# tonyzyl/ladcast

Hardware: AMD Instinct MI355X
Metric: ensemble-member-steps/sec (higher is better)
Workload: dtype f32

## Files before the change

### include/ladcast_hip.h

```cpp
#ifndef LADCAST_HIP_H
#define LADCAST_HIP_H

#ifdef __cplusplus
extern "C" {
#endif

#define LDC_ABI_VERSION 5

#define LDC_OK 0
#define LDC_ERR_ARG (-1)
#define LDC_ERR_ALIGN (-2)
#define LDC_ERR_UNSUPPORTED (-3)

enum ldc_act { LDC_ACT_NONE = 0, LDC_ACT_SILU = 1, LDC_ACT_GELU_TANH = 2, LDC_ACT_RELU = 3 };
#define LDC_ACT_IN_TIMESTEP_SINCOS 16

int ldc_abi_version(void);
const char* ldc_build_arch(void);

typedef struct ldc_gemm_desc {
  int M, N, K, batch;
  int lda, ldw, ldc, ldr;
  long long a_bs, c_bs, r_bs;
  int gate_bs;
  int act;
  int flags;
  int reserved;
} ldc_gemm_desc;
#define LDC_GEMM_A_SPLIT 1
#define LDC_GEMM_C_SPLIT 2
#define LDC_GEMM_BF16_1TERM 4
#define LDC_GEMM_F32_REGSTAGE 8
#define LDC_FMT_F32 0
#define LDC_FMT_SPLIT 1
#define LDC_FMT_BF16 2
int ldc_sizeof_gemm_desc(void);
int ldc_gemm_bias_act(const float* A, const float* W, const float* bias, const float* gate,
                      const float* R, float* C, const ldc_gemm_desc* d, void* stream);

#define LDC_GEMM_MAX_PROBLEMS 4
typedef struct ldc_gemm_problem {
  const float* A;
  const float* W;
  const float* bias;
  const float* gate;
  const float* R;
  float* C;
  ldc_gemm_desc d;
} ldc_gemm_problem;
int ldc_sizeof_gemm_problem(void);
long long ldc_gemm_grouped_workspace_bytes(void);
int ldc_gemm_grouped_workspace_init(void* workspace, long long workspace_bytes, void* stream);
int ldc_gemm_grouped(const ldc_gemm_problem* problems, int n, void* workspace, long long workspace_bytes,
                     void* stream);

int ldc_gemm_grouped_bf16x3(const ldc_gemm_problem* problems, int n, void* workspace, long long workspace_bytes,
                            void* stream);
int ldc_pack_weight_bf16x2(const float* W, void* out, int N, int K, int ldw, void* stream);
int ldc_pack_weight_bf16(const float* W, void* out, int N, int K, int ldw, void* stream);

int ldc_linear_small(const float* x, int x_rows, const float* W, const float* bias,
                     const float* add, int add_rows, float* y, int rows, int N, int K,
                     int act_in, int act_out, void* stream);

int ldc_linear_small_mod(const float* x, int x_rows, const float* W, const float* bias, const float* add, int add_rows,
                         const float* mod, int mod_rows, float* y, int rows, int N, int K, int act_in, int act_out,
                         void* stream);

#define LDC_LINEAR_SMALL_MAX_GROUPED 4
typedef struct ldc_linear_small_problem {
  const float* x;
  const float* W;
  const float* bias;
  const float* add;
  float* y;
  int x_rows, add_rows, rows, N, K, act_in, act_out, reserved;
} ldc_linear_small_problem;
int ldc_linear_small_grouped(const ldc_linear_small_problem* problems, int n, void* stream);

int ldc_attn_fwd(const float* Q, const float* K, const float* V, float* O, int B, int S, int H,
                 int ld_qkv, long long qkv_bs, int ldo, long long o_bs, const float* key_bias, void* stream);
long long ldc_attn_fwd_workspace_bytes(void);
int ldc_attn_fwd_ws(const float* Q, const float* K, const float* V, float* O, int B, int S, int H, int ld_qkv, long long qkv_bs,
                    int ldo, long long o_bs, const float* key_bias, void* workspace, long long workspace_bytes, void* stream);
int ldc_attn_fwd_qrows(const float* Q, const float* K, const float* V, float* O, int B, int S, int Sq, int H, int ld_qkv,
                       long long qkv_bs, int ldo, long long o_bs, const float* key_bias, void* stream);
int ldc_attn_fwd_ws_qrows(const float* Q, const float* K, const float* V, float* O, int B, int S, int Sq, int H, int ld_qkv,
                          long long qkv_bs, int ldo, long long o_bs, const float* key_bias, void* workspace, long long workspace_bytes,
                          void* stream);

#define LDC_ATTN_OUT_SPLIT 1
#define LDC_ATTN_BF16_1TERM 2
#define LDC_ATTN_OUT_BF16 4

typedef struct ldc_qkv_epilogue {
  const float* wq;
  const float* wk;
  const float* rope;
  const float* reserved;
  float eps, qscale;
  int heads, rope_row0;
} ldc_qkv_epilogue;
int ldc_sizeof_qkv_epilogue(void);
int ldc_gemm_grouped_bf16x3_qkv(const ldc_gemm_problem* problems, const ldc_qkv_epilogue* epi, int n, void* workspace,
                                long long workspace_bytes, void* stream);
int ldc_gemm_grouped_qkv_f32(const ldc_gemm_problem* problems, const ldc_qkv_epilogue* epi, int n, void* workspace,
                             long long workspace_bytes, void* stream);
int ldc_attn_qkv_prepare_split(float* Q, float* K, float* V, int B, int S, int H, int ld_qkv, long long qkv_bs, int split_row,
                               const float* wq0, const float* wk0, const float* cos0, const float* sin0, const float* wq1,
                               const float* wk1, const float* cos1, const float* sin1, float eps, void* stream);
long long ldc_attn_fwd_split_workspace_bytes(int B, int S, int H);
long long ldc_attn_fwd_split_workspace_max_bytes(void);
int ldc_attn_fwd_split(const float* Q, const float* K, const float* V, float* O, int B, int S, int H, int ld_qkv,
                       long long qkv_bs, int ldo, long long o_bs, const float* key_bias, int flags, void* workspace,
                       long long workspace_bytes, void* stream);
long long ldc_attn_fwd_split_qrows_workspace_bytes(int B, int S, int Sq, int H);
int ldc_attn_fwd_split_qrows(const float* Q, const float* K, const float* V, float* O, int B, int S, int Sq, int H, int ld_qkv,
                             long long qkv_bs, int ldo, long long o_bs, const float* key_bias, int flags, void* workspace,
                             long long workspace_bytes, void* stream);

int ldc_qk_rmsnorm_rope(float* q, float* k, int B, int row0, int rows, int H, int ld, long long bs,
                        const float* wq, const float* wk, float eps, const float* cos_tab,
                        const float* sin_tab, void* stream);

int ldc_layernorm_mod(const float* x, float* y, int B, int rows, int D, int ldx, long long x_bs,
                      int ldy, long long y_bs, const float* scale, const float* shift, int mod_bs,
                      int mode, float eps, int out_split, void* stream);
int ldc_layernorm_mod2(const float* x, float* y, int B, int rows, int D, int ldx, long long x_bs,
                       int ldy, long long y_bs, const float* scale, const float* shift, int split_row,
                       const float* scale2, const float* shift2, int mod_bs, int mode, float eps,
                       int out_split, void* stream);

int ldc_mean_rows(const float* x, float* y, int B, int rows, int D, int ldx, long long x_bs, void* stream);
int ldc_mean_rows_split(const float* x, float* y, float* x_split, int B, int rows, int D, int ldx,
                        long long x_bs, int lds, long long s_bs, int fmt , void* stream);

int ldc_gate_residual(const float* resid, const float* y, const float* gate, float* out, int B,
                      int rows, int D, int ld_res, long long res_bs, int ld_y, long long y_bs,
                      int gate_bs, void* stream);
int ldc_gate_residual_layernorm(float* resid, const float* y, const float* gate, float* out, int B, int rows, int D, int ld_res,
                                long long res_bs, int ld_y, long long y_bs, int gate_bs, int ld_out, long long out_bs,
                                const float* weight, const float* bias, float eps, int out_split, void* stream);

int ldc_chan_to_token(const float* in, float* out, int B, int C, int N, int ldo, int fill_cols, void* stream);
int ldc_chan_to_token_split(const float* in, float* out, int B, int C, int N, int ldo, int fill_cols,
                            int out_split, void* stream);
int ldc_token_to_chan(const float* in, float* out, int B, int C, int N, int ldi, void* stream);

int ldc_timestep_embedding(const float* t, float* out, int n, void* stream);

int ldc_temb_modulate(float* temb, const float* te, int B, int D, int te_rows, void* stream);

int ldc_chan_affine(const float* x, float* y, const float* mean, const float* std_, float target_std,
                    long long outer, int C, long long inner, int inverse, void* stream);

int ldc_edm_scale_f64_to_f32(const double* x, double c_in, float* out, long long n, void* stream);
int ldc_edm_init_state(const float* noise, double sigma0, double* x, long long n, void* stream);
int ldc_edm_churn(const double* x_cur, const double* noise, double coef, double* x_hat, long long n, void* stream);
int ldc_edm_euler(const double* x_hat, const float* F, double c_skip, double c_out, double t_hat,
                  double dt, double* x_next, double* d_cur, long long n, void* stream);
int ldc_edm_heun(const double* x_hat, double* x_next, const float* F, const double* d_cur,
                 double c_skip, double c_out, double t_next, double dt, long long n, void* stream);
int ldc_f64_to_f32(const double* x, float* y, long long n, void* stream);
int ldc_dpm_step(const float* sample, const float* F, const float* m1, float* x0, float* prev,
                 float c_skip, float c_out, float a, float b, float inv_r0, int order, long long n,
                 void* stream);
int ldc_ddim_step(const float* sample, const float* F, const float* noise, float* x0, float* prev, float sqrt_alpha_t,
                  float sqrt_beta_t, float sqrt_alpha_prev, float dir_coef, float std_dev, float clip_range,
                  int prediction_type, int use_clipped_model_output, long long n, void* stream);
int ldc_ddpm_step(const float* sample, const float* F, const float* noise, float* x0, float* prev, float sqrt_alpha_t,
                  float sqrt_beta_t, float x0_coef, float sample_coef, float std_dev, float clip_range, int prediction_type,
                  long long n, void* stream);
int ldc_scale_f32(const float* x, float s, float* y, long long n, void* stream);
int ldc_axpby_f32(const float* x, float a, const float* y, float b, float* out, long long n, void* stream);

int ldc_edm_noise_inputs(const float* clean, const float* noise, const float* sigma, const float* c_in, float* noisy,
                         float* x_in, int B, long long n_per_sample, void* stream);
int ldc_edm_denoise(const float* noisy, const float* F, const float* c_skip, const float* c_out, float* denoised, int B,
                    int C, int T, int plane, int noisy_frames, int f_frames, int denoised_frames, void* stream);
int ldc_edm_denoise_loss(const float* noisy, const float* F, const float* target, const float* c_skip, const float* c_out,
                         const float* weight, const float* lat_weight, float* table, float* denoised, int B, int C, int T,
                         int H, int W, void* stream);

int ldc_sphere_conv_nhwc(const float* X, const float* Wt, const float* bias, const float* R, float* Y, int B,
                         int H, int W, int cin, int ldx, int cout, int ldy, int ldr, int ksize, int act,
                         void* stream);
int ldc_sphere_dwconv_nhwc(const float* x, const float* wt, const float* bias, float* y, int B, int H, int W,
                           int C, int ldx, int ldy, int ksize, int glu, void* stream);
int ldc_grouped_conv1x1_nhwc(const float* x, const float* wt, float* y, long long M, int groups, int ldx, int ldy,
                             void* stream);
int ldc_relu_linear_attn_nhwc(const float* qkv, float* y, int B, int P, int groups, int ldq, int ldy, float eps,
                              void* workspace, long long workspace_bytes, void* stream);
long long ldc_relu_linear_attn_workspace_bytes(int B, int P, int groups);
int ldc_rmsnorm_rows(const float* x, const float* w, const float* b, const float* resid, float* y, long long rows,
                     int C, int ldx, int ldr, int ldy, float eps, int act, void* stream);
int ldc_pixel_unshuffle_shortcut(const float* cv, const float* x, float* y, int B, int H2, int W2, int cout, int cin,
                                 void* stream);
int ldc_pixel_shuffle_shortcut(const float* cv, const float* x, float* y, int B, int H, int W, int cout, int cin,
                               void* stream);
int ldc_chan_regroup(const float* x, float* y, long long M, int cin, int cout, void* stream);

int ldc_sphere_conv_nhwc_split(const float* X, const void* Wp, const float* bias, const float* R, float* Y, int B, int H, int W,
                               int cin, int ldx, int cout, int ldy, int ldr, int ksize, int act, int in_fmt, int out_fmt,
                               void* workspace, long long workspace_bytes, void* stream);
int ldc_sphere_conv_plan(int B, int H, int W, int cin, int cout, int ksize, int in_fmt, int* tile_rows, int* tile_w);
int ldc_rmsnorm_rows_split(const float* x, const float* w, const float* b, const float* resid, float* y, float* ys, long long rows,
                           int C, int ldx, int ldr, int ldy, int lds, int fmt, float eps, int act, void* stream);
int ldc_pixel_unshuffle_shortcut_split(const float* cv, const float* x, float* y, float* ys, int B, int H2, int W2, int cout,
                                       int cin, int lds, int fmt, void* stream);
int ldc_pixel_shuffle_shortcut_split(const float* cv, const float* x, float* y, float* ys, int B, int H, int W, int cout, int cin,
                                     int lds, int fmt, void* stream);
int ldc_upsample_nearest2x_rows(const float* x, float* y, float* ys, int B, int H, int W, int C, int ldx, int ldy, int lds, int fmt, void* stream);
int ldc_pixel_shuffle_to_chan(const float* cv, float* out, int B, int H, int W, int cout, int keep, void* stream);
int ldc_split_rows(const float* x, float* ys, long long rows, int C, int ldx, int lds, int fmt, void* stream);
int ldc_sphere_dwconv_nhwc_fmt(const float* x, const float* wt, const float* bias, float* y, int B, int H, int W, int C, int ldx,
                               int ldy, int ksize, int glu, int out_fmt, void* stream);
int ldc_relu_linear_attn_nhwc_fmt(const float* qkv, float* y, int B, int P, int groups, int ldq, int ldy, float eps, int out_fmt,
                                  void* workspace, long long workspace_bytes, void* stream);

long long ldc_ensemble_scores_workspace_bytes(int C, int H, int W);
int ldc_ensemble_scores(const float* forecast, long long member_stride, long long channel_stride,
                        const float* truth, long long truth_channel_stride, const float* clim,
                        long long clim_channel_stride, const float* lat_weight, int M, int C, int H, int W,
                        int nan_channel, float* out, float* skill_map, float* spread_map, void* workspace,
                        long long workspace_bytes, void* stream);
long long ldc_rollout_scores_workspace_bytes(int C, int L, int H, int W);
int ldc_rollout_scores(const float* forecast, long long member_stride, long long lead_stride, long long channel_stride,
                       const float* mean, const float* std_, float target_std, const float* truth, long long truth_slot_stride,
                       long long truth_channel_stride, const int* truth_slot, const float* clim, long long clim_slot_stride,
                       long long clim_channel_stride, const int* clim_slot, const float* lat_weight, int M, int C, int L, int H,
                       int W, int nan_channel, float* out, int L_total, int l_off, void* workspace, long long workspace_bytes,
                       void* stream);
long long ldc_validation_scores_workspace_bytes(int C, int L, int H, int W);
int ldc_validation_scores(const float* forecast, long long member_stride, long long lead_stride, long long channel_stride,
                          const float* mean, const float* std_, float target_std, const float* truth, long long truth_slot_stride,
                          long long truth_channel_stride, const int* truth_slot, const float* lat_weight, int M, int C, int L, int H,
                          int W, float* out, int L_total, int l_off, void* workspace, long long workspace_bytes, void* stream);
long long ldc_rollout_reliability_workspace_bytes(int M, int C, int L, int H, int W);
int ldc_rollout_reliability(const float* forecast, long long member_stride, long long lead_stride, long long channel_stride,
                            const float* mean, const float* std_, float target_std, const float* truth, long long truth_slot_stride,
                            long long truth_channel_stride, const int* truth_slot, const float* lat_weight, int M, int C, int L, int H,
                            int W, int nan_channel, float* out, int* hist_count, float* hist_weight, int* n_invalid, int L_total,
                            int l_off, void* workspace, long long workspace_bytes, void* stream);
long long ldc_rollout_spectrum_workspace_bytes(int M, int C, int L, int H, int W);
int ldc_rollout_spectrum(const float* forecast, long long member_stride, long long lead_stride, long long channel_stride,
                         const float* mean, const float* std_, float target_std, const float* truth, long long truth_slot_stride,
                         long long truth_channel_stride, const int* truth_slot, const float* row_weight, int M, int C, int L, int H,
                         int W, float* out, int* n_invalid, int L_total, int l_off, void* workspace, long long workspace_bytes,
                         void* stream);
#define LDC_PRODUCTS_MAX_QUANTILES 16
#define LDC_PRODUCTS_MAX_THRESHOLDS 8
typedef struct ldc_products_desc {
  int n_quant;
  int n_thr;
  int q_lo[LDC_PRODUCTS_MAX_QUANTILES];
  float q_t[LDC_PRODUCTS_MAX_QUANTILES];
  int thr_dir[LDC_PRODUCTS_MAX_THRESHOLDS];
} ldc_products_desc;
int ldc_sizeof_products_desc(void);
int ldc_rollout_products(const float* forecast, long long member_stride, long long lead_stride, long long channel_stride,
                         const float* mean, const float* std_, float target_std, const int* channels, int M, int C, int Cs, int L, int H,
                         int W, const ldc_products_desc* desc, const float* thr, float* stats, float* quant, float* exceed, int L_total,
                         int l_off, void* stream);

#define LDC_TRACK_MAX_CHANNELS 8
#define LDC_TRACK_MAX_BOXES 8
#define LDC_TRACK_MAX_INNER 30
#define LDC_TRACK_MAX_GRID 1024
int ldc_track_gather(const float* x, long long sb, long long st, long long sc, int B, int T, long long HW, const int* channels,
                     int n_ch, const float* mean, const float* std_, float target_std, float* out, int T_total, int t_off,
                     void* stream);
int ldc_track_nanmean(const float* x, long long member_stride, int E, long long n, float* out, void* stream);
int ldc_track_storms(const float* fields, long long track_stride, long long frame_stride, long long mslp_off, long long z_off,
                     const float* lsm, const double* lat, int H, const double* lon, int W, const double* lat0,
                     const double* lon0, int n_tracks, int n_steps, const int* inner_box_sizes, int n_boxes, int enforce_msl,
                     double* out_lat, double* out_lon, int* out_code, void* stream);
int ldc_track_local_min(const float* fields, long long field_stride, const int* field_idx, const double* lat, int H,
                        const double* lon, int W, const double* lat0, const double* lon0, const int* inner, int n_queries,
                        int* found, double* out_lat, double* out_lon, float* out_val, void* stream);

int ldc_recon_preprocess(const float* x, long long batch_stride, long long channel_stride, long long row_stride, int B, int C,
                         int H, int W, const float* mean, const float* std_, int sst_channel, float* out,
                         unsigned char* nan_mask, void* stream);
long long ldc_recon_scores_workspace_bytes(int B, int Cp, int H, int W);
int ldc_recon_scores(const float* pred, const float* target, const float* static_, long long static_batch_stride,
                     const unsigned char* nan_mask, const float* lat_weight, const float* mean, const float* std_, int B, int C,
                     int S, int H, int W, int sst_channel, float* rel, float* abs_norm, float* lw_mse, void* workspace,
                     long long workspace_bytes, void* stream);

long long ldc_field_moments_workspace_bytes(int B, int C, int H, int W);
int ldc_field_moments(const float* x, long long batch_stride, long long channel_stride, long long row_stride, int B, int C, int H,
                      int W, double* state, int accumulate, void* workspace, long long workspace_bytes, void* stream);

#ifdef __cplusplus
}
#endif
#endif
```

### ladcast_amd/csrc/rowops.hip

```cpp
#include "common.h"

namespace {

constexpr int LN_MAX_V4 = 8;

__global__ __launch_bounds__(256) void layernorm_mod_kernel(float* __restrict__ x, float* __restrict__ y,
                                                            int rows, int D, int ldx, long long x_bs, int ldy,
                                                            long long y_bs, const float* __restrict__ scale,
                                                            const float* __restrict__ shift, int split_row,
                                                            const float* __restrict__ scale2,
                                                            const float* __restrict__ shift2, int mod_bs, int mode,
                                                            float eps, int out_split, const float* __restrict__ pre_y,
                                                            const float* __restrict__ pre_gate, int ld_prey,
                                                            long long prey_bs, int gate_bs) {
  const int lane = threadIdx.x & 63;
  const int row = blockIdx.x * 4 + (threadIdx.x >> 6);
  const int b = blockIdx.y;
  if (row >= rows) return;
  if (row >= split_row) {
    scale = scale2;
    shift = shift2;
  }
  float* xr = x + b * x_bs + static_cast<long long>(row) * ldx;
  float* yr = y + b * y_bs + static_cast<long long>(row) * ldy;
  const int nv4 = D >> 2;
  float4 v[LN_MAX_V4];
  float sum = 0.f;
#pragma unroll
  for (int i = 0; i < LN_MAX_V4; ++i) {
    const int c = lane + 64 * i;
    if (c < nv4) {
      v[i] = reinterpret_cast<const float4*>(xr)[c];
      if (pre_y) {
        const float4 yv = reinterpret_cast<const float4*>(pre_y + b * prey_bs + static_cast<long long>(row) * ld_prey)[c];
        const float4 g = reinterpret_cast<const float4*>(pre_gate + static_cast<long long>(b) * gate_bs)[c];
        v[i] = make_float4(fmaf(yv.x, g.x, v[i].x), fmaf(yv.y, g.y, v[i].y), fmaf(yv.z, g.z, v[i].z), fmaf(yv.w, g.w, v[i].w));
        reinterpret_cast<float4*>(xr)[c] = v[i];
      }
      sum += (v[i].x + v[i].y) + (v[i].z + v[i].w);
    } else {
      v[i] = make_float4(0.f, 0.f, 0.f, 0.f);
    }
  }
  const float mean = wave_sum(sum) / static_cast<float>(D);
  float sq = 0.f;
#pragma unroll
  for (int i = 0; i < LN_MAX_V4; ++i) {
    const int c = lane + 64 * i;
    if (c < nv4) {
      const float a = v[i].x - mean, bq = v[i].y - mean, cq = v[i].z - mean, dq = v[i].w - mean;
      sq += (a * a + bq * bq) + (cq * cq + dq * dq);
    }
  }
  const float rstd = rsqrtf(wave_sum(sq) / static_cast<float>(D) + eps);
  const float* sc = scale ? scale + (mode == 0 ? static_cast<long long>(b) * mod_bs : 0) : nullptr;
  const float* sh = shift ? shift + (mode == 0 ? static_cast<long long>(b) * mod_bs : 0) : nullptr;
  const float one = (mode == 0) ? 1.f : 0.f;
#pragma unroll
  for (int i = 0; i < LN_MAX_V4; ++i) {
    const int c = lane + 64 * i;
    if (c < nv4) {
      float4 m = sc ? reinterpret_cast<const float4*>(sc)[c] : make_float4(1.f - one, 1.f - one, 1.f - one, 1.f - one);
      float4 a = sh ? reinterpret_cast<const float4*>(sh)[c] : make_float4(0.f, 0.f, 0.f, 0.f);
      float4 o;
      o.x = (v[i].x - mean) * rstd * (one + m.x) + a.x;
      o.y = (v[i].y - mean) * rstd * (one + m.y) + a.y;
      o.z = (v[i].z - mean) * rstd * (one + m.z) + a.z;
      o.w = (v[i].w - mean) * rstd * (one + m.w) + a.w;
      if (out_split == LDC_FMT_BF16) {
        *reinterpret_cast<uint2*>(reinterpret_cast<unsigned char*>(yr) + 8 * c) = make_uint2(ldc_pack_pair(o.x, o.y), ldc_pack_pair(o.z, o.w));
      } else if (out_split) {
        float r0, r1, r2, r3;
        uint2 hi, lo;
        hi.x = ldc_split_pair(o.x, o.y, r0, r1);
        hi.y = ldc_split_pair(o.z, o.w, r2, r3);
        lo.x = ldc_pack_pair(r0, r1);
        lo.y = ldc_pack_pair(r2, r3);
        unsigned char* grp = reinterpret_cast<unsigned char*>(yr + 8 * (c >> 1)) + 8 * (c & 1);
        *reinterpret_cast<uint2*>(grp) = hi;
        *reinterpret_cast<uint2*>(grp + 16) = lo;
      } else {
        reinterpret_cast<float4*>(yr)[c] = o;
      }
    }
  }
}

__global__ __launch_bounds__(256) void qk_rmsnorm_rope_kernel(float* __restrict__ q, float* __restrict__ k, int row0,
                                                              int rows, int H, int ld, long long bs,
                                                              const float* __restrict__ wq,
                                                              const float* __restrict__ wk, float eps,
                                                              const float* __restrict__ cos_tab,
                                                              const float* __restrict__ sin_tab) {
  const int lane = threadIdx.x & 63;
  const long long item = static_cast<long long>(blockIdx.x) * 4 + (threadIdx.x >> 6);
  const int b = blockIdx.y;
  const long long n_items = static_cast<long long>(rows) * H * 2;
  if (item >= n_items) return;
  const int which = static_cast<int>(item & 1);
  const int head = static_cast<int>((item >> 1) % H);
  const int row = static_cast<int>((item >> 1) / H);
  float* base = (which ? k : q) + b * bs + static_cast<long long>(row0 + row) * ld + head * 128;
  const float* w = which ? wk : wq;
  float2 v = reinterpret_cast<float2*>(base)[lane];
  const float ss = wave_sum(v.x * v.x + v.y * v.y);
  const float r = rsqrtf(ss * (1.0f / 128.0f) + eps);
  const float2 wv = reinterpret_cast<const float2*>(w)[lane];
  v.x = v.x * r * wv.x;
  v.y = v.y * r * wv.y;
  if (cos_tab) {
    const float2 c = reinterpret_cast<const float2*>(cos_tab + static_cast<long long>(row) * 128)[lane];
    const float2 s = reinterpret_cast<const float2*>(sin_tab + static_cast<long long>(row) * 128)[lane];
    const float ox = v.x * c.x + (-v.y) * s.x;
    const float oy = v.y * c.y + v.x * s.y;
    v.x = ox;
    v.y = oy;
  }
  reinterpret_cast<float2*>(base)[lane] = v;
}

__global__ __launch_bounds__(1024) void mean_rows_kernel(const float* __restrict__ x, float* __restrict__ y, int rows,
                                                         int D, int ldx, long long x_bs) {
  __shared__ float part[16][64];
  const int c = threadIdx.x & 63;
  const int col = blockIdx.x * 64 + c;
  const int g = threadIdx.x >> 6;
  const int b = blockIdx.y;
  float s0 = 0.f, s1 = 0.f, s2 = 0.f, s3 = 0.f;
  if (col < D) {
    const float* xb = x + b * x_bs + col;
    int r = g;
    for (; r + 48 < rows; r += 64) {
      s0 += xb[static_cast<long long>(r) * ldx];
      s1 += xb[static_cast<long long>(r + 16) * ldx];
      s2 += xb[static_cast<long long>(r + 32) * ldx];
      s3 += xb[static_cast<long long>(r + 48) * ldx];
    }
    for (; r < rows; r += 16) s0 += xb[static_cast<long long>(r) * ldx];
  }
  part[g][c] = (s0 + s1) + (s2 + s3);
  __syncthreads();
  if (g == 0 && col < D) {
    float t = 0.f;
#pragma unroll
    for (int i = 0; i < 16; ++i) t += part[i][c];
    y[static_cast<long long>(b) * D + col] = t / static_cast<float>(rows);
  }
}

__global__ __launch_bounds__(1024) void mean_rows_split_kernel(const float* __restrict__ x, float* __restrict__ y,
                                                               float* __restrict__ xs, int rows, int D, int ldx,
                                                               long long x_bs, int lds, long long s_bs, int fmt) {
  __shared__ float2 part[16][64];
  const int c = threadIdx.x & 63;
  const int col = (blockIdx.x * 64 + c) * 2;
  const int g = threadIdx.x >> 6;
  const int b = blockIdx.y;
  float2 s0 = make_float2(0.f, 0.f), s1 = s0, s2 = s0, s3 = s0;
  if (col < D) {
    const float* xb = x + b * x_bs + col;
    unsigned char* sb = fmt == LDC_FMT_BF16 ? reinterpret_cast<unsigned char*>(xs + b * s_bs) + 2 * col
                                            : reinterpret_cast<unsigned char*>(xs + b * s_bs + (col & ~7)) + 2 * (col & 7);
    auto take = [&](int r, float2& acc) {
      const float2 v = *reinterpret_cast<const float2*>(xb + static_cast<long long>(r) * ldx);
      acc.x += v.x;
      acc.y += v.y;
      float r0, r1;
      const unsigned hi = ldc_split_pair(v.x, v.y, r0, r1);
      unsigned char* d = sb + static_cast<long long>(r) * lds * 4;
      *reinterpret_cast<unsigned*>(d) = hi;
      if (fmt != LDC_FMT_BF16) *reinterpret_cast<unsigned*>(d + 16) = ldc_pack_pair(r0, r1);
    };
    int r = g;
    for (; r + 48 < rows; r += 64) {
      take(r, s0);
      take(r + 16, s1);
      take(r + 32, s2);
      take(r + 48, s3);
    }
    for (; r < rows; r += 16) take(r, s0);
  }
  part[g][c] = make_float2((s0.x + s1.x) + (s2.x + s3.x), (s0.y + s1.y) + (s2.y + s3.y));
  __syncthreads();
  if (g == 0 && col < D) {
    float2 t = make_float2(0.f, 0.f);
#pragma unroll
    for (int i = 0; i < 16; ++i) {
      t.x += part[i][c].x;
      t.y += part[i][c].y;
    }
    y[static_cast<long long>(b) * D + col] = t.x / static_cast<float>(rows);
    y[static_cast<long long>(b) * D + col + 1] = t.y / static_cast<float>(rows);
  }
}

__global__ __launch_bounds__(256) void gate_residual_kernel(const float* __restrict__ resid, const float* __restrict__ y,
                                                            const float* __restrict__ gate, float* __restrict__ out,
                                                            int rows, int D, int ld_res, long long res_bs, int ld_y,
                                                            long long y_bs, int gate_bs) {
  const int b = blockIdx.z;
  const int row = blockIdx.y;
  const int c = blockIdx.x * 256 + threadIdx.x;
  if (c * 4 >= D) return;
  const float4 r = reinterpret_cast<const float4*>(resid + b * res_bs + static_cast<long long>(row) * ld_res)[c];
  const float4 v = reinterpret_cast<const float4*>(y + b * y_bs + static_cast<long long>(row) * ld_y)[c];
  const float4 g = reinterpret_cast<const float4*>(gate + static_cast<long long>(b) * gate_bs)[c];
  float4 o = make_float4(fmaf(v.x, g.x, r.x), fmaf(v.y, g.y, r.y), fmaf(v.z, g.z, r.z), fmaf(v.w, g.w, r.w));
  reinterpret_cast<float4*>(out + b * res_bs + static_cast<long long>(row) * ld_res)[c] = o;
}

constexpr int LS_ROWS = 8;
constexpr int LS_CPW_MAX = 4;
constexpr int LS_KC = 2048;

__device__ __forceinline__ float modulate_nocontract(float v, float scale, float shift) {
#pragma clang fp contract(off)
  const float f = 1.f + scale;
  const float p = v * f;
  return p + shift;
}

__device__ __forceinline__ void ls_first_read(float4& v) {
#if !(defined(LDC_AB_BUILD) && defined(LDC_LS_NO_FIRST_READ))
  float t0, t1;
  asm volatile("s_waitcnt lgkmcnt(0)\n\tv_mov_b32 %0, %2\n\tv_mov_b32 %1, %3" : "=&v"(t0), "=&v"(t1), "+v"(v.y), "+v"(v.w));
#endif
}

template <int LS_CPW, bool FULL = true>
__device__ __forceinline__ void linear_small_body(const float* __restrict__ x, int x_rows, const float* __restrict__ W,
                                                  const float* __restrict__ bias, const float* __restrict__ add,
                                                  int add_rows, float* __restrict__ y, int rows, int N, int K, int kc,
                                                  int act_in, int act_out, int iters, const float* __restrict__ mod = nullptr,
                                                  int mod_rows = 1) {
  extern __shared__ __attribute__((aligned(16))) float xs[];
  const int lane = threadIdx.x & 63;
  const int wave = threadIdx.x >> 6;
  const int r_base = blockIdx.y * LS_ROWS;
  const int rows_here = rows - r_base < LS_ROWS ? rows - r_base : LS_ROWS;
  for (int it = 0; it < iters; ++it) {
    const int n0 = ((blockIdx.x * iters + it) * 4 + wave) * LS_CPW;
    const float* wr[LS_CPW];
#pragma unroll
    for (int j = 0; j < LS_CPW; ++j) {
      const int n = n0 + j < N ? n0 + j : N - 1;
      wr[j] = W + static_cast<long long>(n) * K;
    }
    float acc[LS_CPW][LS_ROWS];
#pragma unroll
    for (int j = 0; j < LS_CPW; ++j)
#pragma unroll
      for (int i = 0; i < LS_ROWS; ++i) acc[j][i] = 0.f;

    for (int k0 = 0; k0 < K; k0 += kc) {
      const int kn = K - k0 < kc ? K - k0 : kc;
      const int nv4 = kn >> 2;
      if (it == 0) {
        if (k0) __syncthreads();
        for (int idx = threadIdx.x; idx < rows_here * nv4; idx += 256) {
          const int i = idx / nv4, c = idx - i * nv4;
          float4 xv;
          if (FULL && act_in == LDC_ACT_IN_TIMESTEP_SINCOS) {
            const float t = x[(r_base + i) % x_rows];
            float e[4];
#pragma unroll
            for (int j = 0; j < 4; ++j) {
              const int k = k0 + 4 * c + j;
              const float f = expf(-9.210340371976184f * static_cast<float>(k & 127) / 128.0f);
              const float a = t * f;
              e[j] = k < 128 ? cosf(a) : sinf(a);
            }
            xv = make_float4(e[0], e[1], e[2], e[3]);
          } else {
            xv = reinterpret_cast<const float4*>(x + static_cast<long long>((r_base + i) % x_rows) * K + k0)[c];
          }
          if (act_in != LDC_ACT_NONE && !(FULL && act_in == LDC_ACT_IN_TIMESTEP_SINCOS)) {
            xv.x = ldc_apply_act(xv.x, act_in);
            xv.y = ldc_apply_act(xv.y, act_in);
            xv.z = ldc_apply_act(xv.z, act_in);
            xv.w = ldc_apply_act(xv.w, act_in);
          }
          reinterpret_cast<float4*>(xs + i * kc)[c] = xv;
        }
        __syncthreads();
      }
      if (n0 < N) {
        for (int c = lane; c < nv4; c += 64) {
          float4 w[LS_CPW];
#pragma unroll
          for (int j = 0; j < LS_CPW; ++j) {
            typedef float ls_f32x4 __attribute__((ext_vector_type(4)));
            const ls_f32x4 t = __builtin_nontemporal_load(reinterpret_cast<const ls_f32x4*>(wr[j] + k0) + c);
            w[j] = make_float4(t.x, t.y, t.z, t.w);
          }
#pragma unroll
          for (int i = 0; i < LS_ROWS; ++i) {
            if (i < rows_here) {
              float4 xv = reinterpret_cast<const float4*>(xs + i * kc)[c];
              ls_first_read(xv);
#pragma unroll
              for (int j = 0; j < LS_CPW; ++j) acc[j][i] += (w[j].x * xv.x + w[j].y * xv.y) + (w[j].z * xv.z + w[j].w * xv.w);
            }
          }
        }
      }
    }
    if (n0 >= N) continue;
#pragma unroll
    for (int j = 0; j < LS_CPW; ++j) {
      const int n = n0 + j;
#pragma unroll
      for (int i = 0; i < LS_ROWS; ++i) {
        const float sum = wave_sum(acc[j][i]);
        const int r = r_base + i;
        if (lane == 0 && i < rows_here && n < N) {
          float v = sum + (bias ? bias[n] : 0.f);
          v = ldc_apply_act(v, act_out);
          if (add) v += add[static_cast<long long>(r % add_rows) * N + n];
          if (FULL && mod) {
            const float* mr = mod + static_cast<long long>(r % mod_rows) * 2 * N;
            v = modulate_nocontract(v, mr[n], mr[N + n]);
          }
          y[static_cast<long long>(r) * N + n] = v;
        }
      }
    }
  }
}

constexpr int LM_KC = 512;
constexpr int LM_LD = LM_KC + 4;
typedef float lm_f32x4 __attribute__((ext_vector_type(4)));
template <int RT, int U>
__device__ __forceinline__ void lm_steps(const lm_f32x4* __restrict__ wp, const float* __restrict__ xa, lm_f32x4 (&acc)[RT]) {
  lm_f32x4 w[U];
#pragma unroll
  for (int u = 0; u < U; ++u) w[u] = __builtin_nontemporal_load(wp + 4 * u);
#pragma unroll
  for (int u = 0; u < U; ++u)
#pragma unroll
    for (int rt = 0; rt < RT; ++rt) {
      const float4 a = *reinterpret_cast<const float4*>(xa + rt * 16 * LM_LD + 16 * u);
      acc[rt] = __builtin_amdgcn_mfma_f32_16x16x4f32(a.x, w[u].x, acc[rt], 0, 0, 0);
      acc[rt] = __builtin_amdgcn_mfma_f32_16x16x4f32(a.y, w[u].y, acc[rt], 0, 0, 0);
      acc[rt] = __builtin_amdgcn_mfma_f32_16x16x4f32(a.z, w[u].z, acc[rt], 0, 0, 0);
      acc[rt] = __builtin_amdgcn_mfma_f32_16x16x4f32(a.w, w[u].w, acc[rt], 0, 0, 0);
    }
}

template <int RT, int IT>
__global__ __launch_bounds__(256) void linear_rows_mfma_kernel(const float* __restrict__ x, int x_rows, const float* __restrict__ W,
                                                               const float* __restrict__ bias, const float* __restrict__ add, int add_rows,
                                                               float* __restrict__ y, int rows, int N, int K, int act_in, int act_out) {
  extern __shared__ __attribute__((aligned(16))) float xs[];
  const int lane = threadIdx.x & 63, wave = threadIdx.x >> 6;
  const int col = lane & 15, kq = lane >> 4;
  const int r_base = blockIdx.y * 16 * RT;
  const int rows_here = rows - r_base < 16 * RT ? rows - r_base : 16 * RT;
  lm_f32x4 acc[IT][RT];
#pragma unroll
  for (int it = 0; it < IT; ++it)
#pragma unroll
    for (int rt = 0; rt < RT; ++rt) acc[it][rt] = lm_f32x4{0.f, 0.f, 0.f, 0.f};
  for (int k0 = 0; k0 < K; k0 += LM_KC) {
    const int kn = K - k0 < LM_KC ? K - k0 : LM_KC;
    const int nv4 = kn >> 2;
    if (k0) __syncthreads();
    for (int idx = threadIdx.x; idx < 16 * RT * nv4; idx += 256) {
      const int i = idx / nv4, c = idx - i * nv4;
      float4 xv = make_float4(0.f, 0.f, 0.f, 0.f);
      if (i < rows_here) {
        xv = reinterpret_cast<const float4*>(x + static_cast<long long>((r_base + i) % x_rows) * K + k0)[c];
        if (act_in != LDC_ACT_NONE) {
          xv.x = ldc_apply_act(xv.x, act_in);
          xv.y = ldc_apply_act(xv.y, act_in);
          xv.z = ldc_apply_act(xv.z, act_in);
          xv.w = ldc_apply_act(xv.w, act_in);
        }
      }
      reinterpret_cast<float4*>(xs + i * LM_LD)[c] = xv;
    }
    __syncthreads();
#pragma unroll
    for (int it = 0; it < IT; ++it) {
      const int n0 = ((blockIdx.x * IT + it) * 4 + wave) * 16;
      if (n0 < N) {
        const int n = n0 + col < N ? n0 + col : N - 1;
        const lm_f32x4* wp = reinterpret_cast<const lm_f32x4*>(W + static_cast<long long>(n) * K + k0) + kq;
        const float* xa = xs + col * LM_LD + 4 * kq;
        const int ns = kn >> 4;
        int s0 = 0;
        for (; s0 + 8 <= ns; s0 += 8) lm_steps<RT, 8>(wp + 4 * s0, xa + 16 * s0, acc[it]);
        if (s0 < ns) lm_steps<RT, 4>(wp + 4 * s0, xa + 16 * s0, acc[it]);
      }
    }
  }
#pragma unroll
  for (int it = 0; it < IT; ++it) {
    const int n = ((blockIdx.x * IT + it) * 4 + wave) * 16 + col;
    if (n >= N) continue;
    const float bv = bias ? bias[n] : 0.f;
#pragma unroll
    for (int rt = 0; rt < RT; ++rt)
#pragma unroll
      for (int i = 0; i < 4; ++i) {
        const int rl = 16 * rt + 4 * kq + i;
        if (rl >= rows_here) continue;
        const int r = r_base + rl;
        float v = acc[it][rt][i] + bv;
        v = ldc_apply_act(v, act_out);
        if (add) v += add[static_cast<long long>(r % add_rows) * N + n];
        y[static_cast<long long>(r) * N + n] = v;
      }
  }
}

template <int LS_CPW>
__global__ __launch_bounds__(256) void linear_small_kernel(const float* __restrict__ x, int x_rows,
                                                           const float* __restrict__ W, const float* __restrict__ bias,
                                                           const float* __restrict__ add, int add_rows,
                                                           float* __restrict__ y, int rows, int N, int K, int kc, int act_in,
                                                           int act_out, int iters, const float* __restrict__ mod, int mod_rows) {
  linear_small_body<LS_CPW, LS_CPW == 1>(x, x_rows, W, bias, add, add_rows, y, rows, N, K, kc, act_in, act_out, iters, mod, mod_rows);
}

struct LSGroup {
  ldc_linear_small_problem p[LDC_LINEAR_SMALL_MAX_GROUPED];
};

__global__ __launch_bounds__(256) void linear_small_grouped_kernel(LSGroup g) {
  const ldc_linear_small_problem& q = g.p[blockIdx.z];
  if (static_cast<int>(blockIdx.x) * 4 >= q.N || static_cast<int>(blockIdx.y) * LS_ROWS >= q.rows) return;
  const int kc = q.K < LS_KC ? q.K : LS_KC;
  linear_small_body<1>(q.x, q.x_rows, q.W, q.bias, q.add, q.add_rows, q.y, q.rows, q.N, q.K, kc, q.act_in, q.act_out, 1);
}

}

extern "C" int ldc_layernorm_mod2(const float* x, float* y, int B, int rows, int D, int ldx, long long x_bs, int ldy,
                                  long long y_bs, const float* scale, const float* shift, int split_row,
                                  const float* scale2, const float* shift2, int mod_bs, int mode, float eps,
                                  int out_split, void* stream) {
  LDC_CHECK_PTR(x);
  LDC_CHECK_PTR(y);
  if (B <= 0 || rows <= 0 || D <= 0 || split_row < 0) return LDC_ERR_ARG;
  if ((D & 3) || D > 64 * 4 * LN_MAX_V4) return LDC_ERR_UNSUPPORTED;
  if ((ldx & 3) || (ldy & 3) || (x_bs & 3) || (y_bs & 3) || (mod_bs & 3)) return LDC_ERR_ALIGN;
  LDC_CHECK_ALIGN16(x);
  LDC_CHECK_ALIGN16(y);
  if (scale) LDC_CHECK_ALIGN16(scale);
  if (shift) LDC_CHECK_ALIGN16(shift);
  if (scale2) LDC_CHECK_ALIGN16(scale2);
  if (shift2) LDC_CHECK_ALIGN16(shift2);
  if (mode != 0 && mode != 1) return LDC_ERR_UNSUPPORTED;
  if (out_split && ((D & 7) || (ldy & 7) || (y_bs & 7) || (reinterpret_cast<unsigned long long>(y) & 31ull))) return LDC_ERR_ALIGN;
  dim3 grid(ldc_cdiv(rows, 4), B);
  hipLaunchKernelGGL(layernorm_mod_kernel, grid, dim3(256), 0, static_cast<hipStream_t>(stream), const_cast<float*>(x), y, rows, D,
                     ldx, x_bs, ldy, y_bs, scale, shift, split_row, scale2, shift2, mod_bs, mode, eps, out_split,
                     static_cast<const float*>(nullptr), static_cast<const float*>(nullptr), 0, 0LL, 0);
  return ldc_launch_status();
}

extern "C" int ldc_gate_residual_layernorm(float* resid, const float* yv, const float* gate, float* out, int B, int rows, int D,
                                           int ld_res, long long res_bs, int ld_y, long long y_bs, int gate_bs, int ld_out,
                                           long long out_bs, const float* weight, const float* bias, float eps, int out_split,
                                           void* stream) {
  LDC_CHECK_PTR(resid);
  LDC_CHECK_PTR(yv);
  LDC_CHECK_PTR(gate);
  LDC_CHECK_PTR(out);
  if (B <= 0 || rows <= 0 || D <= 0) return LDC_ERR_ARG;
  if ((D & 3) || D > 64 * 4 * LN_MAX_V4) return LDC_ERR_UNSUPPORTED;
  if ((ld_res & 3) || (ld_y & 3) || (ld_out & 3) || (res_bs & 3) || (y_bs & 3) || (out_bs & 3) || (gate_bs & 3)) return LDC_ERR_ALIGN;
  LDC_CHECK_ALIGN16(resid);
  LDC_CHECK_ALIGN16(yv);
  LDC_CHECK_ALIGN16(gate);
  LDC_CHECK_ALIGN16(out);
  if (weight) LDC_CHECK_ALIGN16(weight);
  if (bias) LDC_CHECK_ALIGN16(bias);
  if (out_split && ((D & 7) || (ld_out & 7) || (out_bs & 7) || (reinterpret_cast<unsigned long long>(out) & 31ull))) return LDC_ERR_ALIGN;
  dim3 grid(ldc_cdiv(rows, 4), B);
  hipLaunchKernelGGL(layernorm_mod_kernel, grid, dim3(256), 0, static_cast<hipStream_t>(stream), resid, out, rows, D, ld_res, res_bs,
                     ld_out, out_bs, weight, bias, rows, static_cast<const float*>(nullptr), static_cast<const float*>(nullptr), 0, 1,
                     eps, out_split, yv, gate, ld_y, y_bs, gate_bs);
  return ldc_launch_status();
}

extern "C" int ldc_layernorm_mod(const float* x, float* y, int B, int rows, int D, int ldx, long long x_bs, int ldy,
                                 long long y_bs, const float* scale, const float* shift, int mod_bs, int mode,
                                 float eps, int out_split, void* stream) {
  return ldc_layernorm_mod2(x, y, B, rows, D, ldx, x_bs, ldy, y_bs, scale, shift, rows, nullptr, nullptr, mod_bs, mode, eps,
                            out_split, stream);
}

extern "C" int ldc_qk_rmsnorm_rope(float* q, float* k, int B, int row0, int rows, int H, int ld, long long bs,
                                   const float* wq, const float* wk, float eps, const float* cos_tab,
                                   const float* sin_tab, void* stream) {
  LDC_CHECK_PTR(q);
  LDC_CHECK_PTR(k);
  LDC_CHECK_PTR(wq);
  LDC_CHECK_PTR(wk);
  if (B <= 0 || rows <= 0 || H <= 0 || row0 < 0) return LDC_ERR_ARG;
  if ((cos_tab == nullptr) != (sin_tab == nullptr)) return LDC_ERR_ARG;
  if ((ld & 1) || (bs & 1)) return LDC_ERR_ALIGN;
  const long long items = static_cast<long long>(rows) * H * 2;
  dim3 grid(ldc_cdiv(items, 4), B);
  hipLaunchKernelGGL(qk_rmsnorm_rope_kernel, grid, dim3(256), 0, static_cast<hipStream_t>(stream), q, k, row0, rows, H,
                     ld, bs, wq, wk, eps, cos_tab, sin_tab);
  return ldc_launch_status();
}

extern "C" int ldc_mean_rows(const float* x, float* y, int B, int rows, int D, int ldx, long long x_bs, void* stream) {
  LDC_CHECK_PTR(x);
  LDC_CHECK_PTR(y);
  if (B <= 0 || rows <= 0 || D <= 0) return LDC_ERR_ARG;
  dim3 grid(ldc_cdiv(D, 64), B);
  hipLaunchKernelGGL(mean_rows_kernel, grid, dim3(1024), 0, static_cast<hipStream_t>(stream), x, y, rows, D, ldx, x_bs);
  return ldc_launch_status();
}

extern "C" int ldc_mean_rows_split(const float* x, float* y, float* x_split, int B, int rows, int D, int ldx,
                                   long long x_bs, int lds, long long s_bs, int fmt, void* stream) {
  LDC_CHECK_PTR(x);
  LDC_CHECK_PTR(y);
  LDC_CHECK_PTR(x_split);
  if (B <= 0 || rows <= 0 || D <= 0) return LDC_ERR_ARG;
  if ((D & 7) || (ldx & 1) || (x_bs & 1) || (lds & 7) || (s_bs & 7) || (reinterpret_cast<unsigned long long>(x) & 7ull) ||
      (reinterpret_cast<unsigned long long>(x_split) & 31ull))
    return LDC_ERR_ALIGN;
  if (x == x_split) return LDC_ERR_ARG;
  if (fmt != LDC_FMT_SPLIT && fmt != LDC_FMT_BF16) return LDC_ERR_ARG;
  dim3 grid(ldc_cdiv(D, 128), B);
  hipLaunchKernelGGL(mean_rows_split_kernel, grid, dim3(1024), 0, static_cast<hipStream_t>(stream), x, y, x_split, rows, D,
                     ldx, x_bs, lds, s_bs, fmt);
  return ldc_launch_status();
}

extern "C" int ldc_gate_residual(const float* resid, const float* y, const float* gate, float* out, int B, int rows,
                                 int D, int ld_res, long long res_bs, int ld_y, long long y_bs, int gate_bs,
                                 void* stream) {
  LDC_CHECK_PTR(resid);
  LDC_CHECK_PTR(y);
  LDC_CHECK_PTR(gate);
  LDC_CHECK_PTR(out);
  if (B <= 0 || rows <= 0 || D <= 0) return LDC_ERR_ARG;
  if ((D & 3) || (ld_res & 3) || (ld_y & 3) || (res_bs & 3) || (y_bs & 3) || (gate_bs & 3)) return LDC_ERR_ALIGN;
  if (rows > 65535 || B > 65535) return LDC_ERR_UNSUPPORTED;
  dim3 grid(ldc_cdiv(D / 4, 256), rows, B);
  hipLaunchKernelGGL(gate_residual_kernel, grid, dim3(256), 0, static_cast<hipStream_t>(stream), resid, y, gate, out,
                     rows, D, ld_res, res_bs, ld_y, y_bs, gate_bs);
  return ldc_launch_status();
}

static int linear_small_impl(const float* x, int x_rows, const float* W, const float* bias, const float* add, int add_rows,
                             const float* mod, int mod_rows, float* y, int rows, int N, int K, int act_in, int act_out,
                             void* stream) {
  LDC_CHECK_PTR(x);
  LDC_CHECK_PTR(W);
  LDC_CHECK_PTR(y);
  if (rows <= 0 || N <= 0 || K <= 0 || x_rows <= 0) return LDC_ERR_ARG;
  if (add && add_rows <= 0) return LDC_ERR_ARG;
  if (mod && mod_rows <= 0) return LDC_ERR_ARG;
  if (K & 3) return LDC_ERR_ALIGN;
  if (act_in == LDC_ACT_IN_TIMESTEP_SINCOS) {
    if (K != 256) return LDC_ERR_ARG;
  } else {
    LDC_CHECK_ALIGN16(x);
  }
  LDC_CHECK_ALIGN16(W);
  const int kc = K < LS_KC ? K : LS_KC;
  const int rows_max = rows < LS_ROWS ? rows : LS_ROWS;
  const size_t lds = static_cast<size_t>(rows_max) * kc * sizeof(float);
  static const bool attr_set = [&] {
    (void)hipFuncSetAttribute(reinterpret_cast<const void*>(linear_small_kernel<1>), hipFuncAttributeMaxDynamicSharedMemorySize,
                              LS_ROWS * LS_KC * static_cast<int>(sizeof(float)));
    (void)hipFuncSetAttribute(reinterpret_cast<const void*>(linear_small_kernel<LS_CPW_MAX>),
                              hipFuncAttributeMaxDynamicSharedMemorySize, LS_ROWS * LS_KC * static_cast<int>(sizeof(float)));
    return true;
  }();
  (void)attr_set;
  const bool plain = mod == nullptr && act_in != LDC_ACT_IN_TIMESTEP_SINCOS;
  if (plain && rows > LS_ROWS && N >= 4096 && (K & 63) == 0) {
    const int rt = rows <= 16 ? 1 : 2;
    const int col_groups = ldc_cdiv(N, 64);
    const int row_groups_lm = ldc_cdiv(rows, 16 * rt);
    const long long slots = (rt == 2 ? 2 : 4) * 256LL;
    int iters = 1;
    long long best_cost = -1;
    for (int c = 1; c <= 4; ++c) {
      const long long wgs = static_cast<long long>(ldc_cdiv(col_groups, c)) * row_groups_lm;
      const long long cost = ((wgs + slots - 1) / slots) * c;
      if (best_cost < 0 || cost <= best_cost) { best_cost = cost; iters = c; }
    }
    static const char* const force_lm_iters = LDC_AB_GETENV("LDC_LINEAR_MFMA_ITERS");
    if (force_lm_iters && atoi(force_lm_iters) >= 1 && atoi(force_lm_iters) <= 4) iters = atoi(force_lm_iters);
    dim3 grid(ldc_cdiv(col_groups, iters), row_groups_lm);
    const int lm_lds = 16 * rt * LM_LD * static_cast<int>(sizeof(float));
    static const bool lm_attr_set = [] {
      const int b1 = 16 * LM_LD * static_cast<int>(sizeof(float)), b2 = 2 * b1;
      const auto set = [](auto kern, int bytes) { (void)hipFuncSetAttribute(reinterpret_cast<const void*>(kern), hipFuncAttributeMaxDynamicSharedMemorySize, bytes); };
      set(linear_rows_mfma_kernel<1, 1>, b1); set(linear_rows_mfma_kernel<1, 2>, b1); set(linear_rows_mfma_kernel<1, 3>, b1); set(linear_rows_mfma_kernel<1, 4>, b1);
      set(linear_rows_mfma_kernel<2, 1>, b2); set(linear_rows_mfma_kernel<2, 2>, b2); set(linear_rows_mfma_kernel<2, 3>, b2); set(linear_rows_mfma_kernel<2, 4>, b2);
      return true;
    }();
    (void)lm_attr_set;
    auto launch = [&](auto kern) {
      hipLaunchKernelGGL(kern, grid, dim3(256), lm_lds, static_cast<hipStream_t>(stream), x, x_rows, W, bias, add, add_rows, y, rows, N, K,
                         act_in, act_out);
    };
    if (rt == 1) {
      if (iters == 4) launch(linear_rows_mfma_kernel<1, 4>);
      else if (iters == 3) launch(linear_rows_mfma_kernel<1, 3>);
      else if (iters == 2) launch(linear_rows_mfma_kernel<1, 2>);
      else launch(linear_rows_mfma_kernel<1, 1>);
    } else {
      if (iters == 4) launch(linear_rows_mfma_kernel<2, 4>);
      else if (iters == 3) launch(linear_rows_mfma_kernel<2, 3>);
      else if (iters == 2) launch(linear_rows_mfma_kernel<2, 2>);
      else launch(linear_rows_mfma_kernel<2, 1>);
    }
    return ldc_launch_status();
  }
  const int row_groups = ldc_cdiv(rows, LS_ROWS);
  if (plain && static_cast<long long>(ldc_cdiv(N, 4 * LS_CPW_MAX)) * row_groups >= 1024) {
    int iters = 1;
    if (K <= LS_KC) {
      const long long groups = static_cast<long long>(ldc_cdiv(N, 4 * LS_CPW_MAX)) * row_groups;
      iters = groups >= 2048 ? 4 : 1;
      static const char* const force_iters = LDC_AB_GETENV("LDC_LINEAR_SMALL_ITERS");
      if (force_iters && atoi(force_iters) > 0) iters = atoi(force_iters);
    }
    dim3 grid(ldc_cdiv(ldc_cdiv(N, 4 * LS_CPW_MAX), iters), row_groups);
    hipLaunchKernelGGL(linear_small_kernel<LS_CPW_MAX>, grid, dim3(256), lds, static_cast<hipStream_t>(stream), x, x_rows, W,
                       bias, add, add_rows, y, rows, N, K, kc, act_in, act_out, iters, mod, mod_rows);
  } else {
    dim3 grid(ldc_cdiv(N, 4), row_groups);
    hipLaunchKernelGGL(linear_small_kernel<1>, grid, dim3(256), lds, static_cast<hipStream_t>(stream), x, x_rows, W, bias, add,
                       add_rows, y, rows, N, K, kc, act_in, act_out, 1, mod, mod_rows);
  }
  return ldc_launch_status();
}

extern "C" int ldc_linear_small(const float* x, int x_rows, const float* W, const float* bias, const float* add,
                                int add_rows, float* y, int rows, int N, int K, int act_in, int act_out,
                                void* stream) {
  return linear_small_impl(x, x_rows, W, bias, add, add_rows, nullptr, 1, y, rows, N, K, act_in, act_out, stream);
}

extern "C" int ldc_linear_small_mod(const float* x, int x_rows, const float* W, const float* bias, const float* add,
                                    int add_rows, const float* mod, int mod_rows, float* y, int rows, int N, int K, int act_in,
                                    int act_out, void* stream) {
  LDC_CHECK_PTR(mod);
  return linear_small_impl(x, x_rows, W, bias, add, add_rows, mod, mod_rows, y, rows, N, K, act_in, act_out, stream);
}

extern "C" int ldc_linear_small_grouped(const ldc_linear_small_problem* problems, int n, void* stream) {
  LDC_CHECK_PTR(problems);
  if (n < 1 || n > LDC_LINEAR_SMALL_MAX_GROUPED) return LDC_ERR_ARG;
  LSGroup g{};
  int gx = 0, gy = 0, kc_max = 0, rows_max = 0;
  for (int i = 0; i < n; ++i) {
    const ldc_linear_small_problem& q = problems[i];
    LDC_CHECK_PTR(q.x);
    LDC_CHECK_PTR(q.W);
    LDC_CHECK_PTR(q.y);
    if (q.rows <= 0 || q.N <= 0 || q.K <= 0 || q.x_rows <= 0) return LDC_ERR_ARG;
    if (q.add && q.add_rows <= 0) return LDC_ERR_ARG;
    if (q.K & 3) return LDC_ERR_ALIGN;
    if (q.act_in == LDC_ACT_IN_TIMESTEP_SINCOS) {
      if (q.K != 256) return LDC_ERR_ARG;
    } else {
      LDC_CHECK_ALIGN16(q.x);
    }
    LDC_CHECK_ALIGN16(q.W);
    for (int j = 0; j < i; ++j)
      if (problems[j].y == q.x || problems[j].y == q.add || q.y == problems[j].x || q.y == problems[j].add || q.y == problems[j].y)
        return LDC_ERR_ARG;
    g.p[i] = q;
    const int bx = ldc_cdiv(q.N, 4), by = ldc_cdiv(q.rows, LS_ROWS);
    gx = bx > gx ? bx : gx;
    gy = by > gy ? by : gy;
    const int kc = q.K < LS_KC ? q.K : LS_KC;
    kc_max = kc > kc_max ? kc : kc_max;
    const int r = q.rows < LS_ROWS ? q.rows : LS_ROWS;
    rows_max = r > rows_max ? r : rows_max;
  }
  static const bool attr_set = [&] {
    (void)hipFuncSetAttribute(reinterpret_cast<const void*>(linear_small_grouped_kernel), hipFuncAttributeMaxDynamicSharedMemorySize,
                              LS_ROWS * LS_KC * static_cast<int>(sizeof(float)));
    return true;
  }();
  (void)attr_set;
  const size_t lds = static_cast<size_t>(rows_max) * kc_max * sizeof(float);
  hipLaunchKernelGGL(linear_small_grouped_kernel, dim3(gx, gy, n), dim3(256), lds, static_cast<hipStream_t>(stream), g);
  return ldc_launch_status();
}
```

### ladcast_amd/hip.py

```python
from __future__ import annotations

import ctypes
import os
from ctypes import POINTER, Structure, c_char_p, c_double, c_float, c_int, c_longlong, c_void_p

import torch

_HERE = os.path.dirname(os.path.abspath(__file__))
LIB_PATH = os.environ.get("LDC_LIB_PATH") or os.path.join(_HERE, "libladcast_hip.so")

ACT_NONE, ACT_SILU, ACT_GELU_TANH, ACT_RELU = 0, 1, 2, 3
ACT_IN_TIMESTEP_SINCOS = 16
GEMM_A_SPLIT, GEMM_C_SPLIT, GEMM_BF16_1TERM = 1, 2, 4
GEMM_F32_REGSTAGE = 8
ATTN_OUT_SPLIT, ATTN_BF16_1TERM, ATTN_OUT_BF16 = 1, 2, 4
ABI_VERSION = 5
FMT_F32, FMT_SPLIT, FMT_BF16 = 0, 1, 2


class GemmDesc(Structure):
    _fields_ = [
        ("M", c_int), ("N", c_int), ("K", c_int), ("batch", c_int),
        ("lda", c_int), ("ldw", c_int), ("ldc", c_int), ("ldr", c_int),
        ("a_bs", c_longlong), ("c_bs", c_longlong), ("r_bs", c_longlong),
        ("gate_bs", c_int), ("act", c_int), ("flags", c_int), ("reserved", c_int),
    ]


class GemmProblem(Structure):
    _fields_ = [("A", c_void_p), ("W", c_void_p), ("bias", c_void_p), ("gate", c_void_p), ("R", c_void_p), ("C", c_void_p), ("d", GemmDesc)]


MAX_GROUPED = 4


class QkvEpilogue(Structure):
    _fields_ = [("wq", c_void_p), ("wk", c_void_p), ("rope", c_void_p), ("reserved", c_void_p), ("eps", c_float), ("qscale", c_float),
                ("heads", c_int), ("rope_row0", c_int)]


class LinearSmallProblem(Structure):
    _fields_ = [("x", c_void_p), ("W", c_void_p), ("bias", c_void_p), ("add", c_void_p), ("y", c_void_p), ("x_rows", c_int), ("add_rows", c_int),
                ("rows", c_int), ("N", c_int), ("K", c_int), ("act_in", c_int), ("act_out", c_int), ("reserved", c_int)]


PRODUCTS_MAX_QUANTILES, PRODUCTS_MAX_THRESHOLDS, PRODUCTS_MAX_MEMBERS, PRODUCTS_MAX_SORT_MEMBERS = 16, 8, 1024, 64


class ProductsDesc(Structure):
    _fields_ = [("n_quant", c_int), ("n_thr", c_int), ("q_lo", c_int * PRODUCTS_MAX_QUANTILES), ("q_t", c_float * PRODUCTS_MAX_QUANTILES),
                ("thr_dir", c_int * PRODUCTS_MAX_THRESHOLDS)]


def _load():
    if not os.path.exists(LIB_PATH):
        raise RuntimeError(
            f"{LIB_PATH} is missing: build it with `python -c 'import __graft_entry__ as g; g.build()'` "
            "(or `make -C ladcast_amd/csrc`).  ladcast_amd has no CPU fallback."
        )
    lib = ctypes.CDLL(LIB_PATH)
    P, I, L, F, D = c_void_p, c_int, c_longlong, c_float, c_double
    sig = {
        "ldc_abi_version": (I, []),
        "ldc_build_arch": (c_char_p, []),
        "ldc_sizeof_gemm_desc": (I, []),
        "ldc_gemm_bias_act": (I, [P, P, P, P, P, P, POINTER(GemmDesc), P]),
        "ldc_sizeof_gemm_problem": (I, []),
        "ldc_gemm_grouped_workspace_bytes": (L, []),
        "ldc_gemm_grouped_workspace_init": (I, [P, L, P]),
        "ldc_gemm_grouped": (I, [POINTER(GemmProblem), I, P, L, P]),
        "ldc_gemm_grouped_bf16x3": (I, [POINTER(GemmProblem), I, P, L, P]),
        "ldc_sizeof_qkv_epilogue": (I, []),
        "ldc_gemm_grouped_bf16x3_qkv": (I, [POINTER(GemmProblem), POINTER(QkvEpilogue), I, P, L, P]),
        "ldc_gemm_grouped_qkv_f32": (I, [POINTER(GemmProblem), POINTER(QkvEpilogue), I, P, L, P]),
        "ldc_attn_qkv_prepare_split": (I, [P, P, P, I, I, I, I, L, I, P, P, P, P, P, P, P, P, F, P]),
        "ldc_attn_fwd_split_workspace_bytes": (L, [I, I, I]),
        "ldc_attn_fwd_split_workspace_max_bytes": (L, []),
        "ldc_attn_fwd_split": (I, [P, P, P, P, I, I, I, I, L, I, L, P, I, P, L, P]),
        "ldc_attn_fwd_split_qrows_workspace_bytes": (L, [I, I, I, I]),
        "ldc_attn_fwd_split_qrows": (I, [P, P, P, P, I, I, I, I, I, L, I, L, P, I, P, L, P]),
        "ldc_pack_weight_bf16x2": (I, [P, P, I, I, I, P]),
        "ldc_pack_weight_bf16": (I, [P, P, I, I, I, P]),
        "ldc_linear_small": (I, [P, I, P, P, P, I, P, I, I, I, I, I, P]),
        "ldc_linear_small_grouped": (I, [POINTER(LinearSmallProblem), I, P]),
        "ldc_linear_small_mod": (I, [P, I, P, P, P, I, P, I, P, I, I, I, I, I, P]),
        "ldc_gate_residual_layernorm": (I, [P, P, P, P, I, I, I, I, L, I, L, I, I, L, P, P, F, I, P]),
        "ldc_attn_fwd": (I, [P, P, P, P, I, I, I, I, L, I, L, P, P]),
        "ldc_attn_fwd_ws": (I, [P, P, P, P, I, I, I, I, L, I, L, P, P, L, P]),
        "ldc_attn_fwd_qrows": (I, [P, P, P, P, I, I, I, I, I, L, I, L, P, P]),
        "ldc_attn_fwd_ws_qrows": (I, [P, P, P, P, I, I, I, I, I, L, I, L, P, P, L, P]),
        "ldc_attn_fwd_workspace_bytes": (L, []),
        "ldc_qk_rmsnorm_rope": (I, [P, P, I, I, I, I, I, L, P, P, F, P, P, P]),
        "ldc_sphere_conv_nhwc_split": (I, [P, P, P, P, P, I, I, I, I, I, I, I, I, I, I, I, I, P, L, P]),
        "ldc_sphere_conv_plan": (I, [I, I, I, I, I, I, I, P, P]),
        "ldc_rmsnorm_rows_split": (I, [P, P, P, P, P, P, L, I, I, I, I, I, I, F, I, P]),
        "ldc_pixel_unshuffle_shortcut_split": (I, [P, P, P, P, I, I, I, I, I, I, I, P]),
        "ldc_pixel_shuffle_shortcut_split": (I, [P, P, P, P, I, I, I, I, I, I, I, P]),
        "ldc_pixel_shuffle_to_chan": (I, [P, P, I, I, I, I, I, P]),
        "ldc_split_rows": (I, [P, P, L, I, I, I, I, P]),
        "ldc_upsample_nearest2x_rows": (I, [P, P, P, I, I, I, I, I, I, I, I, P]),
        "ldc_sphere_dwconv_nhwc_fmt": (I, [P, P, P, P, I, I, I, I, I, I, I, I, I, P]),
        "ldc_relu_linear_attn_nhwc_fmt": (I, [P, P, I, I, I, I, I, F, I, P, L, P]),
        "ldc_ensemble_scores_workspace_bytes": (L, [I, I, I]),
        "ldc_ensemble_scores": (I, [P, L, L, P, L, P, L, P, I, I, I, I, I, P, P, P, P, L, P]),
        "ldc_rollout_scores_workspace_bytes": (L, [I, I, I, I]),
        "ldc_rollout_scores": (I, [P, L, L, L, P, P, F, P, L, L, P, P, L, L, P, P, I, I, I, I, I, I, P, I, I, P, L, P]),
        "ldc_validation_scores_workspace_bytes": (L, [I, I, I, I]),
        "ldc_validation_scores": (I, [P, L, L, L, P, P, F, P, L, L, P, P, I, I, I, I, I, P, I, I, P, L, P]),
        "ldc_rollout_reliability_workspace_bytes": (L, [I, I, I, I, I]),
        "ldc_rollout_reliability": (I, [P, L, L, L, P, P, F, P, L, L, P, P, I, I, I, I, I, I, P, P, P, P, I, I, P, L, P]),
        "ldc_rollout_spectrum_workspace_bytes": (L, [I, I, I, I, I]),
        "ldc_rollout_spectrum": (I, [P, L, L, L, P, P, F, P, L, L, P, P, I, I, I, I, I, P, P, I, I, P, L, P]),
        "ldc_sizeof_products_desc": (I, []),
        "ldc_rollout_products": (I, [P, L, L, L, P, P, F, P, I, I, I, I, I, I, POINTER(ProductsDesc), P, P, P, P, I, I, P]),
        "ldc_layernorm_mod": (I, [P, P, I, I, I, I, L, I, L, P, P, I, I, F, I, P]),
        "ldc_layernorm_mod2": (I, [P, P, I, I, I, I, L, I, L, P, P, I, P, P, I, I, F, I, P]),
        "ldc_mean_rows": (I, [P, P, I, I, I, I, L, P]),
        "ldc_mean_rows_split": (I, [P, P, P, I, I, I, I, L, I, L, I, P]),
        "ldc_chan_to_token_split": (I, [P, P, I, I, I, I, I, I, P]),
        "ldc_gate_residual": (I, [P, P, P, P, I, I, I, I, L, I, L, I, P]),
        "ldc_chan_to_token": (I, [P, P, I, I, I, I, I, P]),
        "ldc_token_to_chan": (I, [P, P, I, I, I, I, P]),
        "ldc_timestep_embedding": (I, [P, P, I, P]),
        "ldc_temb_modulate": (I, [P, P, I, I, I, P]),
        "ldc_chan_affine": (I, [P, P, P, P, F, L, I, L, I, P]),
        "ldc_edm_scale_f64_to_f32": (I, [P, D, P, L, P]),
        "ldc_edm_init_state": (I, [P, D, P, L, P]),
        "ldc_edm_euler": (I, [P, P, D, D, D, D, P, P, L, P]),
        "ldc_edm_churn": (I, [P, P, c_double, P, L, P]),
        "ldc_edm_heun": (I, [P, P, P, P, D, D, D, D, L, P]),
        "ldc_f64_to_f32": (I, [P, P, L, P]),
        "ldc_dpm_step": (I, [P, P, P, P, P, F, F, F, F, F, I, L, P]),
        "ldc_ddim_step": (I, [P, P, P, P, P, F, F, F, F, F, F, I, I, L, P]),
        "ldc_ddpm_step": (I, [P, P, P, P, P, F, F, F, F, F, F, I, L, P]),
        "ldc_scale_f32": (I, [P, F, P, L, P]),
        "ldc_axpby_f32": (I, [P, F, P, F, P, L, P]),
        "ldc_edm_noise_inputs": (I, [P, P, P, P, P, P, I, L, P]),
        "ldc_edm_denoise": (I, [P, P, P, P, P, I, I, I, I, I, I, I, P]),
        "ldc_edm_denoise_loss": (I, [P, P, P, P, P, P, P, P, P, I, I, I, I, I, P]),
        "ldc_sphere_conv_nhwc": (I, [P, P, P, P, P, I, I, I, I, I, I, I, I, I, I, P]),
        "ldc_sphere_dwconv_nhwc": (I, [P, P, P, P, I, I, I, I, I, I, I, I, P]),
        "ldc_grouped_conv1x1_nhwc": (I, [P, P, P, L, I, I, I, P]),
        "ldc_relu_linear_attn_nhwc": (I, [P, P, I, I, I, I, I, F, P, L, P]),
        "ldc_relu_linear_attn_workspace_bytes": (L, [I, I, I]),
        "ldc_rmsnorm_rows": (I, [P, P, P, P, P, L, I, I, I, I, F, I, P]),
        "ldc_pixel_unshuffle_shortcut": (I, [P, P, P, I, I, I, I, I, P]),
        "ldc_pixel_shuffle_shortcut": (I, [P, P, P, I, I, I, I, I, P]),
        "ldc_chan_regroup": (I, [P, P, L, I, I, P]),
        "ldc_track_gather": (I, [P, L, L, L, I, I, L, POINTER(c_int), I, P, P, F, P, I, I, P]),
        "ldc_track_nanmean": (I, [P, L, I, L, P, P]),
        "ldc_track_storms": (I, [P, L, L, L, L, P, P, I, P, I, P, P, I, I, POINTER(c_int), I, I, P, P, P, P]),
        "ldc_track_local_min": (I, [P, L, P, P, I, P, I, P, P, P, I, P, P, P, P, P]),
        "ldc_recon_preprocess": (I, [P, L, L, L, I, I, I, I, P, P, I, P, P, P]),
        "ldc_recon_scores_workspace_bytes": (L, [I, I, I, I]),
        "ldc_recon_scores": (I, [P, P, P, L, P, P, P, P, I, I, I, I, I, I, P, P, P, P, L, P]),
        "ldc_field_moments_workspace_bytes": (L, [I, I, I, I]),
        "ldc_field_moments": (I, [P, L, L, L, I, I, I, I, P, I, P, L, P]),
    }
    for name, (res, args) in sig.items():
        fn = getattr(lib, name)
        fn.restype = res
        fn.argtypes = args
    if lib.ldc_abi_version() != ABI_VERSION:
        raise RuntimeError("libladcast_hip.so ABI version mismatch")
    if lib.ldc_sizeof_gemm_desc() != ctypes.sizeof(GemmDesc) or lib.ldc_sizeof_gemm_problem() != ctypes.sizeof(GemmProblem):
        raise RuntimeError("ldc_gemm_desc / ldc_gemm_problem layout mismatch between header and binding")
    if lib.ldc_sizeof_qkv_epilogue() != ctypes.sizeof(QkvEpilogue):
        raise RuntimeError("ldc_qkv_epilogue layout mismatch between header and binding")
    if lib.ldc_sizeof_products_desc() != ctypes.sizeof(ProductsDesc):
        raise RuntimeError("ldc_products_desc layout mismatch between header and binding")
    return lib, sig


lib, SIGNATURES = _load()


def _check(status: int, what: str):
    if status != 0:
        raise RuntimeError(f"{what} failed with status {status}")


def upload_nonblocking(t, device):
    device = torch.device(device)
    if device.type != "cuda" or t.device.type != "cpu":
        return t.to(device)
    return (t if t.is_pinned() else t.pin_memory()).to(device, non_blocking=True)


def _p(t):
    return None if t is None else c_void_p(t.data_ptr())


def _stream():
    return c_void_p(torch.cuda.current_stream().cuda_stream)


def _dev(*ts):
    for t in ts:
        if t is not None and not t.is_cuda:
            raise RuntimeError("ladcast_amd kernels need device tensors (no CPU fallback)")


def gemm(A, W, C, *, M, N, K, batch=1, lda=None, ldw=None, ldc=None, a_bs=0, c_bs=0, bias=None, gate=None,
         gate_bs=0, R=None, ldr=0, r_bs=0, act=ACT_NONE):
    _dev(A, W, C, bias, gate, R)
    d = GemmDesc(M, N, K, batch, lda if lda is not None else K, ldw if ldw is not None else K,
                 ldc if ldc is not None else N, ldr, a_bs, c_bs, r_bs, gate_bs, act, 0, 0)
    _check(lib.ldc_gemm_bias_act(_p(A), _p(W), _p(bias), _p(gate), _p(R), _p(C), ctypes.byref(d), _stream()), "ldc_gemm_bias_act")


_workspaces = {}
_outgrown = []


def _workspace(name, device, nbytes, init=None, grow=False):
    key = (name, str(device), torch.cuda.current_stream(device).cuda_stream)
    ws = _workspaces.get(key)
    if ws is None or (grow and ws.numel() * 4 < nbytes):
        if not grow and torch.cuda.is_current_stream_capturing():
            raise RuntimeError(f"{name}: the first call on a stream must be made outside a graph capture (run one warm-up forward)")
        if ws is not None:
            _outgrown.append(ws)
        ws = torch.empty((nbytes + 3) // 4, device=device, dtype=torch.float32)
        if init == "zero":
            ws.zero_()
        elif init == "grouped":
            _check(lib.ldc_gemm_grouped_workspace_init(c_void_p(ws.data_ptr()), ws.numel() * 4, _stream()), "ldc_gemm_grouped_workspace_init")
        _workspaces[key] = ws
    return ws


def _grouped_workspace(device):
    return _workspace("gemm_grouped", device, lib.ldc_gemm_grouped_workspace_bytes(), init="grouped")


def gemm_problem(A, W, C, *, M, N, K, batch=1, lda=None, ldw=None, ldc=None, a_bs=0, c_bs=0, bias=None, gate=None, gate_bs=0, R=None,
                 ldr=0, r_bs=0, act=ACT_NONE, flags=0):
    _dev(A, W, C, bias, gate, R)
    d = GemmDesc(M, N, K, batch, lda if lda is not None else K, ldw if ldw is not None else K, ldc if ldc is not None else N, ldr,
                 a_bs, c_bs, r_bs, gate_bs, act, flags, 0)
    pv = lambda t: None if t is None else t.data_ptr()
    return GemmProblem(pv(A), pv(W), pv(bias), pv(gate), pv(R), pv(C), d), (A, W, C, bias, gate, R)


def gemm_grouped(problems, split_bf16=False):
    n = len(problems)
    if not 1 <= n <= MAX_GROUPED:
        raise ValueError(f"gemm_grouped takes 1..{MAX_GROUPED} problems")
    arr = (GemmProblem * n)(*[p[0] for p in problems])
    ws = _grouped_workspace(problems[0][1][2].device)
    fn = lib.ldc_gemm_grouped_bf16x3 if split_bf16 else lib.ldc_gemm_grouped
    _check(fn(arr, n, c_void_p(ws.data_ptr()), ws.numel() * 4, _stream()), "ldc_gemm_grouped" + ("_bf16x3" if split_bf16 else ""))


def gemm_sk(A, W, C, split_bf16=False, **kw):
    gemm_grouped([gemm_problem(A, W, C, **kw)], split_bf16=split_bf16)


def pack_weight_bf16x2(W):
    _dev(W)
    W = W.contiguous()
    N, K = W.shape
    out = torch.empty(N * K, device=W.device, dtype=torch.int32)
    _check(lib.ldc_pack_weight_bf16x2(_p(W), _p(out), N, K, K, _stream()), "ldc_pack_weight_bf16x2")
    return out


def pack_weight_bf16(W):
    _dev(W)
    W = W.contiguous()
    N, K = W.shape
    out = torch.empty(N * K, device=W.device, dtype=torch.bfloat16)
    _check(lib.ldc_pack_weight_bf16(_p(W), _p(out), N, K, K, _stream()), "ldc_pack_weight_bf16")
    return out


def linear_small(x, W, y, *, rows, N, K, x_rows=None, bias=None, add=None, add_rows=1, act_in=ACT_NONE, act_out=ACT_NONE, mod=None, mod_rows=1):
    _dev(x, W, y, bias, add, mod)
    xr = x_rows if x_rows is not None else rows
    if mod is not None:
        _check(lib.ldc_linear_small_mod(_p(x), xr, _p(W), _p(bias), _p(add), add_rows, _p(mod), mod_rows, _p(y), rows, N, K, act_in, act_out, _stream()),
               "ldc_linear_small_mod")
        return
    _check(lib.ldc_linear_small(_p(x), xr, _p(W), _p(bias), _p(add), add_rows, _p(y), rows, N, K, act_in, act_out, _stream()), "ldc_linear_small")


def gate_residual_layernorm(resid, y, gate, out, *, B, rows, D, ld_res, res_bs, ld_y, y_bs, gate_bs, ld_out, out_bs, weight, bias, eps, out_split=False):
    _dev(resid, y, gate, out, weight, bias)
    _check(lib.ldc_gate_residual_layernorm(_p(resid), _p(y), _p(gate), _p(out), B, rows, D, ld_res, res_bs, ld_y, y_bs, gate_bs, ld_out, out_bs,
                                           _p(weight), _p(bias), eps, int(out_split), _stream()), "ldc_gate_residual_layernorm")


LINEAR_SMALL_MAX_GROUPED = 4


def linear_small_problem(x, W, y, *, rows, N, K, x_rows=None, bias=None, add=None, add_rows=1, act_in=ACT_NONE, act_out=ACT_NONE):
    _dev(x, W, y, bias, add)
    q = LinearSmallProblem(_p(x), _p(W), _p(bias), _p(add), _p(y), x_rows if x_rows is not None else rows, add_rows, rows, N, K, act_in, act_out, 0)
    return q, (x, W, y, bias, add)


def linear_small_grouped(problems):
    n = len(problems)
    if not 1 <= n <= LINEAR_SMALL_MAX_GROUPED:
        raise ValueError(f"linear_small_grouped takes 1..{LINEAR_SMALL_MAX_GROUPED} problems")
    arr = (LinearSmallProblem * n)(*[p[0] for p in problems])
    _check(lib.ldc_linear_small_grouped(arr, n, _stream()), "ldc_linear_small_grouped")


def _attn_f32_workspace(device):
    return _workspace("attn_fwd", device, lib.ldc_attn_fwd_workspace_bytes(), init="zero")


def attn_fwd(Q, K, V, O, *, B, S, H, ld_qkv, qkv_bs, ldo, o_bs, key_bias=None, use_workspace=True, Sq=None):
    _dev(Q, K, V, O, key_bias)
    if key_bias is not None and key_bias.numel() < S:
        raise ValueError("key_bias must hold one value per key")
    if not use_workspace:
        if Sq is None:
            _check(lib.ldc_attn_fwd(_p(Q), _p(K), _p(V), _p(O), B, S, H, ld_qkv, qkv_bs, ldo, o_bs, _p(key_bias), _stream()), "ldc_attn_fwd")
        else:
            _check(lib.ldc_attn_fwd_qrows(_p(Q), _p(K), _p(V), _p(O), B, S, Sq, H, ld_qkv, qkv_bs, ldo, o_bs, _p(key_bias), _stream()), "ldc_attn_fwd_qrows")
        return
    ws = _attn_f32_workspace(Q.device)
    if Sq is None:
        st = lib.ldc_attn_fwd_ws(_p(Q), _p(K), _p(V), _p(O), B, S, H, ld_qkv, qkv_bs, ldo, o_bs, _p(key_bias), _p(ws), ws.numel() * 4, _stream())
    else:
        st = lib.ldc_attn_fwd_ws_qrows(_p(Q), _p(K), _p(V), _p(O), B, S, Sq, H, ld_qkv, qkv_bs, ldo, o_bs, _p(key_bias), _p(ws), ws.numel() * 4, _stream())
    if st != 0 and not torch.cuda.is_current_stream_capturing():
        ws.zero_()
    _check(st, "ldc_attn_fwd_ws" if Sq is None else "ldc_attn_fwd_ws_qrows")


def rearm_attention_workspaces(device=None):
    want = None if device is None else torch.device(device).index
    for key, ws in _workspaces.items():
        if key[0] == "attn_fwd" and (want is None or ws.device.index == want):
            ws.zero_()


def ensemble_scores(forecast, truth, clim, lat_weight, out, *, M, C, H, W, member_stride, channel_stride, truth_channel_stride,
                    clim_channel_stride=0, nan_channel=-1, skill_map=None, spread_map=None):
    _dev(forecast, truth, clim, lat_weight, out, skill_map, spread_map)
    ws = _workspace("ensemble_scores", forecast.device, int(lib.ldc_ensemble_scores_workspace_bytes(C, H, W)), grow=True)
    _check(lib.ldc_ensemble_scores(_p(forecast), member_stride, channel_stride, _p(truth), truth_channel_stride, _p(clim),
                                   clim_channel_stride, _p(lat_weight), M, C, H, W, nan_channel, _p(out), _p(skill_map), _p(spread_map),
                                   _p(ws), ws.numel() * 4, _stream()), "ldc_ensemble_scores")


def rollout_scores(forecast, truth, truth_slot, clim, clim_slot, lat_weight, out, *, M, C, L, H, W, member_stride, lead_stride, channel_stride,
                   truth_slot_stride, truth_channel_stride, clim_slot_stride=0, clim_channel_stride=0, mean=None, std=None, target_std=1.0,
                   nan_channel=-1, L_total, l_off=0):
    _dev(forecast, truth, truth_slot, clim, clim_slot, lat_weight, out, mean, std)
    ws = _workspace("rollout_scores", forecast.device, int(lib.ldc_rollout_scores_workspace_bytes(C, L, H, W)), grow=True)
    _check(lib.ldc_rollout_scores(_p(forecast), member_stride, lead_stride, channel_stride, _p(mean), _p(std), float(target_std), _p(truth),
                                  truth_slot_stride, truth_channel_stride, _p(truth_slot), _p(clim), clim_slot_stride, clim_channel_stride,
                                  _p(clim_slot), _p(lat_weight), M, C, L, H, W, nan_channel, _p(out), L_total, l_off, _p(ws), ws.numel() * 4,
                                  _stream()), "ldc_rollout_scores")


def validation_scores(forecast, truth, truth_slot, lat_weight, out, *, M, C, L, H, W, member_stride, lead_stride, channel_stride,
                      truth_slot_stride, truth_channel_stride, mean=None, std=None, target_std=1.0, L_total, l_off=0):
    _dev(forecast, truth, truth_slot, lat_weight, out, mean, std)
    ws = _workspace("validation_scores", forecast.device, int(lib.ldc_validation_scores_workspace_bytes(C, L, H, W)), grow=True)
    _check(lib.ldc_validation_scores(_p(forecast), member_stride, lead_stride, channel_stride, _p(mean), _p(std), float(target_std), _p(truth),
                                     truth_slot_stride, truth_channel_stride, _p(truth_slot), _p(lat_weight), M, C, L, H, W, _p(out), L_total,
                                     l_off, _p(ws), ws.numel() * 4, _stream()), "ldc_validation_scores")


def rollout_reliability(forecast, truth, truth_slot, lat_weight, out, hist_count, hist_weight, n_invalid, *, M, C, L, H, W, member_stride,
                        lead_stride, channel_stride, truth_slot_stride, truth_channel_stride, mean=None, std=None, target_std=1.0,
                        nan_channel=-1, L_total, l_off=0):
    _dev(forecast, truth, truth_slot, lat_weight, out, hist_count, hist_weight, n_invalid, mean, std)
    nbytes = int(lib.ldc_rollout_reliability_workspace_bytes(M, C, L, H, W))
    ws = _workspace("rollout_reliability", forecast.device, max(nbytes, 4), grow=True)
    _check(lib.ldc_rollout_reliability(_p(forecast), member_stride, lead_stride, channel_stride, _p(mean), _p(std), float(target_std), _p(truth),
                                       truth_slot_stride, truth_channel_stride, _p(truth_slot), _p(lat_weight), M, C, L, H, W, nan_channel,
                                       _p(out), _p(hist_count), _p(hist_weight), _p(n_invalid), L_total, l_off, _p(ws), ws.numel() * 4,
                                       _stream()), "ldc_rollout_reliability")


def rollout_spectrum(forecast, truth, truth_slot, row_weight, out, n_invalid, *, M, C, L, H, W, member_stride, lead_stride, channel_stride,
                     truth_slot_stride, truth_channel_stride, mean=None, std=None, target_std=1.0, L_total, l_off=0):
    _dev(forecast, truth, truth_slot, row_weight, out, n_invalid, mean, std)
    nbytes = int(lib.ldc_rollout_spectrum_workspace_bytes(M, C, L, H, W))
    ws = _workspace("rollout_spectrum", forecast.device, max(nbytes, 4), grow=True)
    _check(lib.ldc_rollout_spectrum(_p(forecast), member_stride, lead_stride, channel_stride, _p(mean), _p(std), float(target_std), _p(truth),
                                    truth_slot_stride, truth_channel_stride, _p(truth_slot), _p(row_weight), M, C, L, H, W, _p(out),
                                    _p(n_invalid), L_total, l_off, _p(ws), ws.numel() * 4, _stream()), "ldc_rollout_spectrum")


def products_desc(quantiles, M, threshold_dirs=()):
    import math

    qs, dirs = [float(q) for q in quantiles], [int(d) for d in threshold_dirs]
    if len(qs) > PRODUCTS_MAX_QUANTILES or len(dirs) > PRODUCTS_MAX_THRESHOLDS:
        raise ValueError(f"at most {PRODUCTS_MAX_QUANTILES} quantiles and {PRODUCTS_MAX_THRESHOLDS} thresholds per call")
    if any(not 0.0 <= q <= 1.0 for q in qs):
        raise ValueError(f"quantiles must lie in [0, 1], got {qs}")
    if any(d not in (1, -1) for d in dirs):
        raise ValueError(f"a threshold direction is +1 (above) or -1 (below), got {dirs}")
    if M < 1:
        raise ValueError("at least one member")
    d = ProductsDesc()
    d.n_quant, d.n_thr = len(qs), len(dirs)
    for k, q in enumerate(qs):
        pos = q * (M - 1)
        lo = min(int(math.floor(pos)), M - 1)
        d.q_lo[k], d.q_t[k] = lo, pos - lo
    for k, v in enumerate(dirs):
        d.thr_dir[k] = v
    return d


def rollout_products(forecast, desc, *, M, C, L, H, W, member_stride, lead_stride, channel_stride, channels=None, Cs=None, thr=None, stats=None,
                     quant=None, exceed=None, mean=None, std=None, target_std=1.0, L_total, l_off=0):
    _dev(forecast, channels, thr, stats, quant, exceed, mean, std)
    _check(lib.ldc_rollout_products(_p(forecast), member_stride, lead_stride, channel_stride, _p(mean), _p(std), float(target_std), _p(channels),
                                    M, C, C if Cs is None else Cs, L, H, W, ctypes.byref(desc), _p(thr), _p(stats), _p(quant), _p(exceed),
                                    L_total, l_off, _stream()), "ldc_rollout_products")


def recon_preprocess(x, mean, std, out, nan_mask=None, *, B, C, H, W, batch_stride, channel_stride, row_stride, sst_channel=-1):
    _dev(x, mean, std, out, nan_mask)
    _check(lib.ldc_recon_preprocess(_p(x), batch_stride, channel_stride, row_stride, B, C, H, W, _p(mean), _p(std), sst_channel, _p(out),
                                    _p(nan_mask), _stream()), "ldc_recon_preprocess")


def recon_scores(pred, target, static, nan_mask, lat_weight, mean, std, rel, lw_mse, *, B, C, S, H, W, static_batch_stride=0, sst_channel=-1,
                 abs_norm=None):
    _dev(pred, target, static, nan_mask, lat_weight, mean, std, rel, lw_mse, abs_norm)
    ws = _workspace("recon_scores", pred.device, int(lib.ldc_recon_scores_workspace_bytes(B, C + S, H, W)), grow=True)
    _check(lib.ldc_recon_scores(_p(pred), _p(target), _p(static), static_batch_stride, _p(nan_mask), _p(lat_weight), _p(mean), _p(std), B, C, S,
                                H, W, sst_channel, _p(rel), _p(abs_norm), _p(lw_mse), _p(ws), ws.numel() * 4, _stream()), "ldc_recon_scores")


def field_moments(x, state, *, B, C, H, W, batch_stride, channel_stride, row_stride, accumulate):
    _dev(x, state)
    nbytes = int(lib.ldc_field_moments_workspace_bytes(B, C, H, W))
    ws = _workspace("field_moments", x.device, max(nbytes, 16), grow=True)
    _check(lib.ldc_field_moments(_p(x), batch_stride, channel_stride, row_stride, B, C, H, W, _p(state), 1 if accumulate else 0, _p(ws),
                                 ws.numel() * 4, _stream()), "ldc_field_moments")


def compact_rope_table(cos, sin):
    if not (torch.equal(cos[:, 0::2], cos[:, 1::2]) and torch.equal(sin[:, 0::2], sin[:, 1::2])):
        raise ValueError("rotary tables must hold every (cos, sin) value twice (adjacent-pair RoPE)")
    return torch.stack([cos[:, 0::2], sin[:, 0::2]], dim=-1).reshape(cos.shape[0], cos.shape[1]).contiguous()


def qkv_epilogue(wq=None, wk=None, rope=None, *, eps=1e-7, heads, rope_row0=0, qscale=0.0):
    _dev(wq, wk, rope)
    pv = lambda t: None if t is None else t.data_ptr()
    return QkvEpilogue(pv(wq), pv(wk), pv(rope), None, eps, qscale, heads, rope_row0), (wq, wk, rope)


ERR_UNSUPPORTED = -3
_DEFAULT_QSCALE = ctypes.c_float(0.08838834764831845 * 1.4426950408889634).value


def gemm_grouped_qkv_f32(problems, epilogues):
    n = len(problems)
    if not 1 <= n <= MAX_GROUPED or len(epilogues) != n:
        raise ValueError(f"gemm_grouped_qkv_f32 takes 1..{MAX_GROUPED} problems and one epilogue (or None) per problem")
    arr = (GemmProblem * n)(*[p[0] for p in problems])
    epi = (QkvEpilogue * n)(*[(e[0] if e is not None else QkvEpilogue()) for e in epilogues])
    ws = _grouped_workspace(problems[0][1][2].device)
    st = lib.ldc_gemm_grouped_qkv_f32(arr, epi, n, c_void_p(ws.data_ptr()), ws.numel() * 4, _stream())
    if st == ERR_UNSUPPORTED:
        return False
    _check(st, "ldc_gemm_grouped_qkv_f32")
    return True


def gemm_grouped_qkv(problems, epilogues, force_fallback=False):
    n = len(problems)
    if not 1 <= n <= MAX_GROUPED or len(epilogues) != n:
        raise ValueError(f"gemm_grouped_qkv takes 1..{MAX_GROUPED} problems and one epilogue (or None) per problem")
    arr = (GemmProblem * n)(*[p[0] for p in problems])
    epi = (QkvEpilogue * n)(*[(e[0] if e is not None else QkvEpilogue()) for e in epilogues])
    ws = _grouped_workspace(problems[0][1][2].device)
    st = ERR_UNSUPPORTED if force_fallback else lib.ldc_gemm_grouped_bf16x3_qkv(arr, epi, n, c_void_p(ws.data_ptr()), ws.numel() * 4, _stream())
    if st != ERR_UNSUPPORTED:
        _check(st, "ldc_gemm_grouped_bf16x3_qkv")
        return
    if any(p[0].d.flags & GEMM_BF16_1TERM for p in problems):
        raise RuntimeError("ldc_gemm_grouped_bf16x3_qkv: shape not served by the fused kernel, and the plain-GEMM + ldc_attn_qkv_prepare_split "
                           "route only writes split-bf16 operand rows (status -3 in the single-term bf16 mode)")
    _check(lib.ldc_gemm_grouped_bf16x3(arr, n, c_void_p(ws.data_ptr()), ws.numel() * 4, _stream()), "ldc_gemm_grouped_bf16x3 (QKV fallback)")
    for (p, keep), e in zip(problems, epilogues):
        if e is None:
            continue
        q, (wq, wk, rope) = e
        if q.qscale not in (0.0, _DEFAULT_QSCALE):
            raise RuntimeError("ldc_gemm_grouped_bf16x3_qkv: shape not served by the fused kernel, and the plain-GEMM + ldc_attn_qkv_prepare_split "
                               f"route applies the default q scale log2(e)/sqrt(128), not qscale={q.qscale!r}")
        d, C = p.d, keep[2]
        D, S = q.heads * 128, d.M
        if d.N != 3 * D:
            raise RuntimeError("ldc_gemm_grouped_bf16x3_qkv failed with status -1")
        cos = sin = None
        if rope is not None:
            t = rope.reshape(-1, 64, 2)[q.rope_row0 : q.rope_row0 + S]
            cos, sin = t[..., 0].repeat_interleave(2, dim=1).contiguous(), t[..., 1].repeat_interleave(2, dim=1).contiguous()
        base = C.data_ptr()
        _check(lib.ldc_attn_qkv_prepare_split(c_void_p(base), c_void_p(base + 4 * D), c_void_p(base + 8 * D), d.batch, S, q.heads, d.ldc, d.c_bs, S,
                                              _p(wq), _p(wk), _p(cos), _p(sin), None, None, None, None, q.eps, _stream()), "ldc_attn_qkv_prepare_split")


def attn_qkv_prepare_split(Q, K, V, *, B, S, H, ld_qkv, qkv_bs, split_row, seg0=(None, None, None, None), seg1=(None, None, None, None), eps=1e-7):
    _dev(Q, K, V, *seg0, *seg1)
    _check(lib.ldc_attn_qkv_prepare_split(_p(Q), _p(K), _p(V), B, S, H, ld_qkv, qkv_bs, split_row, _p(seg0[0]), _p(seg0[1]), _p(seg0[2]), _p(seg0[3]),
                                          _p(seg1[0]), _p(seg1[1]), _p(seg1[2]), _p(seg1[3]), eps, _stream()), "ldc_attn_qkv_prepare_split")


def _attn_workspace(device, nbytes):
    ws = _workspace("attn_fwd_split", device, lib.ldc_attn_fwd_split_workspace_max_bytes())
    if ws.numel() * 4 < nbytes:
        raise RuntimeError(f"attn_fwd_split: call shape asks for {nbytes} workspace bytes, more than ldc_attn_fwd_split_workspace_max_bytes")
    return ws


def attn_fwd_split(Q, K, V, O, *, B, S, H, ld_qkv, qkv_bs, ldo, o_bs, out_split=False, one_term=False, key_bias=None, use_workspace=True, Sq=None):
    _dev(Q, K, V, O, key_bias)
    if Sq is None:
        nbytes = lib.ldc_attn_fwd_split_workspace_bytes(B, S, H) if use_workspace else 0
    else:
        nbytes = lib.ldc_attn_fwd_split_qrows_workspace_bytes(B, S, Sq, H) if use_workspace else 0
    ws = _attn_workspace(Q.device, nbytes) if nbytes > 0 else None
    if key_bias is not None and key_bias.numel() < 32 * ((S + 31) // 32):
        raise ValueError("key_bias must be padded to a multiple of 32 keys (hip.pad_key_bias)")
    flags = (ATTN_OUT_BF16 if int(out_split) == FMT_BF16 else ATTN_OUT_SPLIT if out_split else 0) | (ATTN_BF16_1TERM if one_term else 0)
    if Sq is None:
        _check(lib.ldc_attn_fwd_split(_p(Q), _p(K), _p(V), _p(O), B, S, H, ld_qkv, qkv_bs, ldo, o_bs, _p(key_bias), flags, _p(ws), 0 if ws is None else ws.numel() * 4,
                                      _stream()), "ldc_attn_fwd_split")
    else:
        _check(lib.ldc_attn_fwd_split_qrows(_p(Q), _p(K), _p(V), _p(O), B, S, Sq, H, ld_qkv, qkv_bs, ldo, o_bs, _p(key_bias), flags, _p(ws),
                                            0 if ws is None else ws.numel() * 4, _stream()), "ldc_attn_fwd_split_qrows")


def pad_key_bias(bias):
    S = bias.numel()
    out = torch.zeros(32 * ((S + 31) // 32), device=bias.device, dtype=torch.float32)
    out[:S] = bias.reshape(-1)
    return out


def qk_rmsnorm_rope(q, k, *, B, row0, rows, H, ld, bs, wq, wk, eps, cos=None, sin=None):
    _dev(q, k, wq, wk, cos, sin)
    _check(lib.ldc_qk_rmsnorm_rope(_p(q), _p(k), B, row0, rows, H, ld, bs, _p(wq), _p(wk), eps, _p(cos), _p(sin), _stream()),
           "ldc_qk_rmsnorm_rope")


def layernorm_mod(x, y, *, B, rows, D, ldx, x_bs, ldy, y_bs, scale=None, shift=None, mod_bs=0, mode=0, eps=1e-6, out_split=False,
                  split_row=None, scale2=None, shift2=None):
    _dev(x, y, scale, shift, scale2, shift2)
    if split_row is None:
        _check(lib.ldc_layernorm_mod(_p(x), _p(y), B, rows, D, ldx, x_bs, ldy, y_bs, _p(scale), _p(shift), mod_bs, mode, eps,
                                     int(out_split), _stream()),
               "ldc_layernorm_mod")
    else:
        _check(lib.ldc_layernorm_mod2(_p(x), _p(y), B, rows, D, ldx, x_bs, ldy, y_bs, _p(scale), _p(shift), split_row, _p(scale2), _p(shift2),
                                      mod_bs, mode, eps, int(out_split), _stream()),
               "ldc_layernorm_mod2")


def mean_rows(x, y, *, B, rows, D, ldx, x_bs, x_split=None, lds=None, s_bs=None, fmt=FMT_SPLIT):
    _dev(x, y, x_split)
    if x_split is None:
        _check(lib.ldc_mean_rows(_p(x), _p(y), B, rows, D, ldx, x_bs, _stream()), "ldc_mean_rows")
    else:
        _check(lib.ldc_mean_rows_split(_p(x), _p(y), _p(x_split), B, rows, D, ldx, x_bs, lds if lds is not None else ldx,
                                       s_bs if s_bs is not None else x_bs, int(fmt), _stream()), "ldc_mean_rows_split")


def gate_residual(resid, y, gate, out, *, B, rows, D, ld_res, res_bs, ld_y, y_bs, gate_bs):
    _dev(resid, y, gate, out)
    _check(lib.ldc_gate_residual(_p(resid), _p(y), _p(gate), _p(out), B, rows, D, ld_res, res_bs, ld_y, y_bs, gate_bs, _stream()),
           "ldc_gate_residual")


def chan_to_token(x, out, *, B, C, N, ldo, fill_cols=None, out_split=False):
    _dev(x, out)
    _check(lib.ldc_chan_to_token_split(_p(x), _p(out), B, C, N, ldo, ldo if fill_cols is None else fill_cols, int(out_split), _stream()),
           "ldc_chan_to_token")


def token_to_chan(x, out, *, B, C, N, ldi):
    _dev(x, out)
    _check(lib.ldc_token_to_chan(_p(x), _p(out), B, C, N, ldi, _stream()), "ldc_token_to_chan")


def timestep_embedding(t, out, n):
    _dev(t, out)
    _check(lib.ldc_timestep_embedding(_p(t), _p(out), n, _stream()), "ldc_timestep_embedding")


def temb_modulate(temb, te, *, B, D, te_rows):
    _dev(temb, te)
    _check(lib.ldc_temb_modulate(_p(temb), _p(te), B, D, te_rows, _stream()), "ldc_temb_modulate")


def chan_affine(x, y, mean, std, target_std, *, outer, C, inner, inverse):
    _dev(x, y, mean, std)
    _check(lib.ldc_chan_affine(_p(x), _p(y), _p(mean), _p(std), target_std, outer, C, inner, int(inverse), _stream()), "ldc_chan_affine")


TRACK_MAX_CHANNELS, TRACK_MAX_BOXES, TRACK_MAX_INNER, TRACK_MAX_GRID = 8, 8, 30, 1024


def _int_array(values):
    return (c_int * len(values))(*[int(v) for v in values])


def track_gather(x, out, channels, mean, std, *, sb, st, sc, B, T, HW, T_total, t_off, target_std=1.0):
    _dev(x, out, mean, std)
    _check(lib.ldc_track_gather(_p(x), sb, st, sc, B, T, HW, _int_array(channels), len(channels), _p(mean), _p(std), float(target_std),
                                _p(out), T_total, t_off, _stream()), "ldc_track_gather")


def track_nanmean(x, out, *, member_stride, E, n):
    _dev(x, out)
    _check(lib.ldc_track_nanmean(_p(x), member_stride, E, n, _p(out), _stream()), "ldc_track_nanmean")


def track_storms(fields, lat, lon, lat0, lon0, out_lat, out_lon, out_code, *, track_stride, frame_stride, mslp_off, z_off, lsm, H, W,
                 n_tracks, n_steps, inner_box_sizes, enforce_msl):
    _dev(fields, lat, lon, lat0, lon0, out_lat, out_lon, out_code, lsm)
    _check(lib.ldc_track_storms(_p(fields), track_stride, frame_stride, mslp_off, z_off, _p(lsm), _p(lat), H, _p(lon), W, _p(lat0), _p(lon0),
                                n_tracks, n_steps, _int_array(inner_box_sizes), len(inner_box_sizes), int(bool(enforce_msl)), _p(out_lat),
                                _p(out_lon), _p(out_code), _stream()), "ldc_track_storms")


def track_local_min(fields, field_idx, lat, lon, lat0, lon0, inner, found, out_lat, out_lon, out_val, *, field_stride, H, W, n_queries):
    _dev(fields, field_idx, lat, lon, lat0, lon0, inner, found, out_lat, out_lon, out_val)
    _check(lib.ldc_track_local_min(_p(fields), field_stride, _p(field_idx), _p(lat), H, _p(lon), W, _p(lat0), _p(lon0), _p(inner), n_queries,
                                   _p(found), _p(out_lat), _p(out_lon), _p(out_val), _stream()), "ldc_track_local_min")


def edm_scale_f64_to_f32(x, c_in, out):
    _dev(x, out)
    _check(lib.ldc_edm_scale_f64_to_f32(_p(x), c_in, _p(out), x.numel(), _stream()), "ldc_edm_scale_f64_to_f32")


def edm_init_state(noise, sigma0, x):
    _dev(noise, x)
    _check(lib.ldc_edm_init_state(_p(noise), sigma0, _p(x), x.numel(), _stream()), "ldc_edm_init_state")


def edm_churn(x_cur, noise, coef, x_hat):
    _dev(x_cur, noise, x_hat)
    if noise.dtype != torch.float64 or x_cur.dtype != torch.float64:
        raise TypeError("edm_churn works on the fp64 sampler state")
    _check(lib.ldc_edm_churn(_p(x_cur), _p(noise), coef, _p(x_hat), x_cur.numel(), _stream()), "ldc_edm_churn")


def edm_euler(x_hat, F, c_skip, c_out, t_hat, dt, x_next, d_cur):
    _dev(x_hat, F, x_next, d_cur)
    _check(lib.ldc_edm_euler(_p(x_hat), _p(F), c_skip, c_out, t_hat, dt, _p(x_next), _p(d_cur), x_hat.numel(), _stream()), "ldc_edm_euler")


def edm_heun(x_hat, x_next, F, d_cur, c_skip, c_out, t_next, dt):
    _dev(x_hat, x_next, F, d_cur)
    _check(lib.ldc_edm_heun(_p(x_hat), _p(x_next), _p(F), _p(d_cur), c_skip, c_out, t_next, dt, x_hat.numel(), _stream()), "ldc_edm_heun")


def f64_to_f32(x, y):
    _dev(x, y)
    _check(lib.ldc_f64_to_f32(_p(x), _p(y), x.numel(), _stream()), "ldc_f64_to_f32")


def dpm_step(sample, F, m1, x0, prev, c_skip, c_out, a, b, inv_r0, order):
    _dev(sample, F, m1, x0, prev)
    _check(lib.ldc_dpm_step(_p(sample), _p(F), _p(m1), _p(x0), _p(prev), c_skip, c_out, a, b, inv_r0, order, sample.numel(), _stream()),
           "ldc_dpm_step")


def ddim_step(sample, F, noise, x0, prev, sqrt_alpha_t, sqrt_beta_t, sqrt_alpha_prev, dir_coef, std_dev, clip_range, prediction_type, reclip):
    _dev(sample, F, noise, x0, prev)
    _check(lib.ldc_ddim_step(_p(sample), _p(F), _p(noise), _p(x0), _p(prev), sqrt_alpha_t, sqrt_beta_t, sqrt_alpha_prev, dir_coef, std_dev,
                             clip_range, prediction_type, int(bool(reclip)), sample.numel(), _stream()), "ldc_ddim_step")


def ddpm_step(sample, F, noise, x0, prev, sqrt_alpha_t, sqrt_beta_t, x0_coef, sample_coef, std_dev, clip_range, prediction_type):
    _dev(sample, F, noise, x0, prev)
    _check(lib.ldc_ddpm_step(_p(sample), _p(F), _p(noise), _p(x0), _p(prev), sqrt_alpha_t, sqrt_beta_t, x0_coef, sample_coef, std_dev, clip_range,
                             prediction_type, sample.numel(), _stream()), "ldc_ddpm_step")


def scale_f32(x, s, y):
    _dev(x, y)
    _check(lib.ldc_scale_f32(_p(x), s, _p(y), x.numel(), _stream()), "ldc_scale_f32")


def axpby_f32(x, a, y, b, out):
    _dev(x, y, out)
    _check(lib.ldc_axpby_f32(_p(x), a, _p(y), b, _p(out), x.numel(), _stream()), "ldc_axpby_f32")


def _f32c(what, *ts):
    for t in ts:
        if t is not None and not (t.dtype == torch.float32 and t.is_contiguous()):
            raise TypeError(f"{what}: contiguous fp32 tensors only")


def _per_sample(what, B, *vs):
    for v in vs:
        if v is not None and not (v.is_cuda and v.dtype == torch.float32 and v.is_contiguous() and v.numel() == B):
            raise ValueError(f"{what}: per-sample coefficients are contiguous fp32 device vectors with one entry per sample ({B})")


def edm_noise_inputs(clean, noise, sigma, c_in, noisy, x_in):
    _dev(clean, noise, sigma, c_in, noisy, x_in)
    _f32c("edm_noise_inputs", clean, noise, noisy, x_in)
    B = clean.shape[0]
    _per_sample("edm_noise_inputs", B, sigma, c_in)
    for t in (noise, noisy, x_in):
        if t is not None and t.shape != clean.shape:
            raise ValueError("edm_noise_inputs: all tensors have the shape of `clean`")
    _check(lib.ldc_edm_noise_inputs(_p(clean), _p(noise), _p(sigma), _p(c_in), _p(noisy), _p(x_in), B, clean.numel() // max(B, 1), _stream()),
           "ldc_edm_noise_inputs")


def _t_slice_frames(what, t, shape):
    B, C, T, H, W = shape
    if tuple(t.shape) != tuple(shape) or t.dtype != torch.float32:
        raise ValueError(f"{what}: fp32 tensors of one shape (B, C, T, H, W)")
    plane = H * W
    sb, sc, st, sh, sw = t.stride()
    ok = (sw == 1 or W == 1) and (sh == W or H == 1) and (st == plane or T == 1)
    frames = sc // plane if C > 1 else (sb // (C * plane) if B > 1 else T)
    ok = ok and frames >= T and (C == 1 or sc == frames * plane) and (B == 1 or sb == C * frames * plane)
    if not ok:
        raise ValueError(f"{what}: tensors must be contiguous or slices along T of contiguous tensors (strides {t.stride()})")
    return frames


def edm_denoise(noisy, F, c_skip, c_out, denoised):
    _dev(noisy, F, c_skip, c_out, denoised)
    B, C, T, H, W = noisy.shape
    _per_sample("edm_denoise", B, c_skip, c_out)
    fr = [_t_slice_frames("edm_denoise", t, noisy.shape) for t in (noisy, F, denoised)]
    _check(lib.ldc_edm_denoise(_p(noisy), _p(F), _p(c_skip), _p(c_out), _p(denoised), B, C, T, H * W, fr[0], fr[1], fr[2], _stream()),
           "ldc_edm_denoise")


def edm_denoise_loss(noisy, F, target, c_skip, c_out, weight, table, lat_weight=None, denoised=None):
    _dev(noisy, F, target, c_skip, c_out, weight, table, lat_weight, denoised)
    _f32c("edm_denoise_loss", noisy, F, target, table, lat_weight, denoised)
    B, C, T, H, W = noisy.shape
    _per_sample("edm_denoise_loss", B, c_skip, c_out, weight)
    for t in (F, target, denoised):
        if t is not None and t.shape != noisy.shape:
            raise ValueError("edm_denoise_loss: noisy, F, target and denoised have one shape (B, C, T, H, W)")
    if table.numel() != B * C * T or (lat_weight is not None and lat_weight.numel() != H):
        raise ValueError("edm_denoise_loss: table holds B * C * T values, lat_weight H")
    _check(lib.ldc_edm_denoise_loss(_p(noisy), _p(F), _p(target), _p(c_skip), _p(c_out), _p(weight), _p(lat_weight), _p(table), _p(denoised),
                                    B, C, T, H, W, _stream()), "ldc_edm_denoise_loss")


def sphere_conv_nhwc(X, Wt, Y, *, B, H, W, cin, cout, ldx=None, ldy=None, bias=None, R=None, ldr=0, ksize=3, act=ACT_NONE):
    _dev(X, Wt, Y, bias, R)
    _check(lib.ldc_sphere_conv_nhwc(_p(X), _p(Wt), _p(bias), _p(R), _p(Y), B, H, W, cin, ldx if ldx is not None else cin, cout,
                                    ldy if ldy is not None else cout, ldr, ksize, act, _stream()), "ldc_sphere_conv_nhwc")


def conv_cin_padded(cin, cpk=32):
    kt = -(-cin // cpk)
    p2 = 1
    while p2 < kt:
        p2 *= 2
    return cpk * p2


def sphere_conv_nhwc_split(X, Wp, Y, *, B, H, W, cin, cout, ldx, ldy=None, bias=None, R=None, ldr=0, ksize=3, act=ACT_NONE, in_fmt=FMT_SPLIT,
                           out_fmt=FMT_F32):
    _dev(X, Wp, Y, bias, R)
    ws = _grouped_workspace(X.device)
    _check(lib.ldc_sphere_conv_nhwc_split(_p(X), _p(Wp), _p(bias), _p(R), _p(Y), B, H, W, cin, ldx, cout, ldy if ldy is not None else cout,
                                          ldr, ksize, act, int(in_fmt), int(out_fmt), _p(ws), ws.numel() * 4, _stream()), "ldc_sphere_conv_nhwc_split")


def sphere_conv_plan(B, H, W, cin, cout, ksize=3, in_fmt=FMT_SPLIT):
    bm, tw = c_int(0), c_int(0)
    halo = lib.ldc_sphere_conv_plan(B, H, W, cin, cout, ksize, int(in_fmt), ctypes.byref(bm), ctypes.byref(tw))
    return bool(halo), bm.value, tw.value


def split_rows(x, ys, *, rows, C, ldx=None, lds=None, fmt=FMT_SPLIT):
    _dev(x, ys)
    _check(lib.ldc_split_rows(_p(x), _p(ys), rows, C, ldx if ldx is not None else C, lds if lds is not None else -(-C // 8) * 8, int(fmt), _stream()),
           "ldc_split_rows")


def sphere_dwconv_nhwc(x, wt, y, *, B, H, W, C, ldx=None, ldy=None, bias=None, ksize=3, glu=False, out_fmt=FMT_F32):
    _dev(x, wt, y, bias)
    cy = C // 2 if glu else C
    _check(lib.ldc_sphere_dwconv_nhwc_fmt(_p(x), _p(wt), _p(bias), _p(y), B, H, W, C, ldx if ldx is not None else C,
                                          ldy if ldy is not None else cy, ksize, int(glu), int(out_fmt), _stream()), "ldc_sphere_dwconv_nhwc_fmt")


def grouped_conv1x1_nhwc(x, wt, y, *, M, groups, ldx, ldy):
    _dev(x, wt, y)
    _check(lib.ldc_grouped_conv1x1_nhwc(_p(x), _p(wt), _p(y), M, groups, ldx, ldy, _stream()), "ldc_grouped_conv1x1_nhwc")


def relu_linear_attn_nhwc(qkv, y, *, B, P, groups, ldq, ldy, eps, out_fmt=FMT_F32, sliced=True):
    _dev(qkv, y)
    ws, nbytes = None, 0
    if sliced:
        nbytes = lib.ldc_relu_linear_attn_workspace_bytes(B, P, groups)
        ws = torch.empty(nbytes // 4, device=qkv.device, dtype=torch.float32) if nbytes else None
    _check(lib.ldc_relu_linear_attn_nhwc_fmt(_p(qkv), _p(y), B, P, groups, ldq, ldy, eps, int(out_fmt), _p(ws), nbytes,
                                             _stream()),
           "ldc_relu_linear_attn_nhwc_fmt")


def rmsnorm_rows(x, w, y, *, rows, C, eps, b=None, resid=None, ldx=None, ldr=None, ldy=None, act=ACT_NONE, ys=None, lds=None, fmt=FMT_SPLIT):
    _dev(x, w, b, resid, y, ys)
    _check(lib.ldc_rmsnorm_rows_split(_p(x), _p(w), _p(b), _p(resid), _p(y), _p(ys), rows, C, ldx if ldx is not None else C,
                                      ldr if ldr is not None else C, ldy if ldy is not None else C,
                                      (lds if lds is not None else -(-C // 8) * 8) if ys is not None else 0, int(fmt), eps, act, _stream()),
           "ldc_rmsnorm_rows_split")


def pixel_unshuffle_shortcut(cv, x, y, *, B, H2, W2, cout, cin, ys=None, lds=None, fmt=FMT_SPLIT):
    _dev(cv, x, y, ys)
    _check(lib.ldc_pixel_unshuffle_shortcut_split(_p(cv), _p(x), _p(y), _p(ys), B, H2, W2, cout, cin,
                                                  (lds if lds is not None else -(-cout // 8) * 8) if ys is not None else 0, int(fmt), _stream()),
           "ldc_pixel_unshuffle_shortcut_split")


def pixel_shuffle_to_chan(cv, out, *, B, H, W, cout, keep):
    _dev(cv, out)
    _check(lib.ldc_pixel_shuffle_to_chan(_p(cv), _p(out), B, H, W, cout, keep, _stream()), "ldc_pixel_shuffle_to_chan")


def pixel_shuffle_shortcut(cv, x, y, *, B, H, W, cout, cin, ys=None, lds=None, fmt=FMT_SPLIT):
    _dev(cv, x, y, ys)
    _check(lib.ldc_pixel_shuffle_shortcut_split(_p(cv), _p(x), _p(y), _p(ys), B, H, W, cout, cin,
                                                (lds if lds is not None else -(-cout // 8) * 8) if ys is not None else 0, int(fmt), _stream()),
           "ldc_pixel_shuffle_shortcut_split")


def upsample_nearest2x_rows(x, y, *, B, H, W, C, ldx=None, ldy=None, ys=None, lds=None, fmt=FMT_SPLIT):
    _dev(x, y, ys)
    _check(lib.ldc_upsample_nearest2x_rows(_p(x), _p(y), _p(ys), B, H, W, C, ldx if ldx is not None else C, ldy if ldy is not None else C,
                                           (lds if lds is not None else (ys.shape[1] if ys is not None else 0)), int(fmt), _stream()), "ldc_upsample_nearest2x_rows")


def chan_regroup(x, y, *, M, cin, cout):
    _dev(x, y)
    _check(lib.ldc_chan_regroup(_p(x), _p(y), M, cin, cout, _stream()), "ldc_chan_regroup")
```

### ladcast_amd/models/LaDCast_3D_model.py

```python
from __future__ import annotations

from types import SimpleNamespace
from typing import Optional, Tuple

import numpy as np
import torch
import torch.nn as nn

from .. import graphs, hip
from .embeddings import get_year_sincos_embedding, rope_tables_from_grid, rotary_1d
from .modeling_utils import ModelMixin


class _RMSNormP(nn.Module):
    def __init__(self, dim, eps):
        super().__init__()
        self.eps = eps
        self.weight = nn.Parameter(torch.ones(dim))

    def forward(self, x):
        var = x.to(torch.float32).pow(2).mean(-1, keepdim=True)
        return x * torch.rsqrt(var + self.eps) * self.weight


class LaDCastAttnProcessor2_0:

    def __call__(self, *a, **k):
        raise RuntimeError("the built-in processor is fused into the HIP forward and is not callable on its own; "
                           "use the C ABI (ldc_gemm_grouped_bf16x3_qkv + ldc_attn_fwd_split, or ldc_qk_rmsnorm_rope + ldc_attn_fwd)")


class _TimestepEmbeddingP(nn.Module):
    def __init__(self, in_channels, dim):
        super().__init__()
        self.linear_1 = nn.Linear(in_channels, dim)
        self.linear_2 = nn.Linear(dim, dim)


class _CombinedTimestepTextProjP(nn.Module):
    def __init__(self, dim, pooled_dim):
        super().__init__()
        self.timestep_embedder = _TimestepEmbeddingP(256, dim)
        self.text_embedder = _TimestepEmbeddingP(pooled_dim, dim)


class _AdaLinearP(nn.Module):
    def __init__(self, dim_in, dim_out):
        super().__init__()
        self.linear = nn.Linear(dim_in, dim_out)


class _ActProjP(nn.Module):
    def __init__(self, a, b):
        super().__init__()
        self.proj = nn.Linear(a, b)


class _FeedForwardP(nn.Module):
    def __init__(self, dim, mult):
        super().__init__()
        inner = int(dim * mult)
        self.net = nn.ModuleList([_ActProjP(dim, inner), nn.Identity(), nn.Linear(inner, dim)])


class _AttentionP(nn.Module):
    def __init__(self, dim, heads, head_dim, eps=1e-7, added=False, pre_only=False):
        super().__init__()
        inner = heads * head_dim
        self.heads = heads
        self.to_q = nn.Linear(dim, inner)
        self.to_k = nn.Linear(dim, inner)
        self.to_v = nn.Linear(dim, inner)
        self.norm_q = _RMSNormP(head_dim, eps)
        self.norm_k = _RMSNormP(head_dim, eps)
        if added:
            self.add_k_proj = nn.Linear(dim, inner)
            self.add_v_proj = nn.Linear(dim, inner)
            self.add_q_proj = nn.Linear(dim, inner)
            self.norm_added_q = _RMSNormP(head_dim, eps)
            self.norm_added_k = _RMSNormP(head_dim, eps)
            self.to_add_out = nn.Linear(inner, dim)
        else:
            self.add_q_proj = self.add_k_proj = self.add_v_proj = None
            self.norm_added_q = self.norm_added_k = None
            self.to_add_out = None
        if not pre_only:
            self.to_out = nn.ModuleList([nn.Linear(inner, dim), nn.Identity()])
        else:
            self.to_out = None
        self.processor = LaDCastAttnProcessor2_0()

    def set_processor(self, processor):
        self.processor = processor

    def get_processor(self):
        return self.processor

    @property
    def foreign_processor(self):
        p = self.processor
        return None if p is None or isinstance(p, LaDCastAttnProcessor2_0) else p


class _PatchEmbedP(nn.Module):

    def __init__(self, in_chans, dim, patch=(1, 1, 1)):
        super().__init__()
        self.proj = nn.Conv3d(in_chans, dim, kernel_size=tuple(patch), stride=tuple(patch))


class _RefinerBlockP(nn.Module):
    def __init__(self, heads, head_dim, mlp_width_ratio=4.0):
        super().__init__()
        d = heads * head_dim
        self.norm1 = nn.LayerNorm(d, elementwise_affine=True, eps=1e-7)
        self.attn = _AttentionP(d, heads, head_dim, pre_only=True)
        self.norm2 = nn.LayerNorm(d, elementwise_affine=True, eps=1e-7)
        self.ff = _FeedForwardP(d, mlp_width_ratio)
        self.norm_out = _AdaLinearP(d, 2 * d)


class _IndividualTokenRefinerP(nn.Module):
    def __init__(self, heads, head_dim, n):
        super().__init__()
        self.refiner_blocks = nn.ModuleList([_RefinerBlockP(heads, head_dim) for _ in range(n)])


class _TokenRefinerP(nn.Module):
    def __init__(self, in_channels, heads, head_dim, n):
        super().__init__()
        d = heads * head_dim
        self.time_text_embed = _CombinedTimestepTextProjP(d, in_channels)
        self.proj_in = nn.Linear(in_channels, d)
        self.token_refiner = _IndividualTokenRefinerP(heads, head_dim, n)


class _SingleBlockP(nn.Module):
    def __init__(self, heads, head_dim, mlp_ratio):
        super().__init__()
        d = heads * head_dim
        mlp = int(d * mlp_ratio)
        self.attn = _AttentionP(d, heads, head_dim, pre_only=True)
        self.norm = _AdaLinearP(d, 3 * d)
        self.proj_mlp = nn.Linear(d, mlp)
        self.proj_out = nn.Linear(d + mlp, d)


class _DualBlockP(nn.Module):
    def __init__(self, heads, head_dim, mlp_ratio):
        super().__init__()
        d = heads * head_dim
        self.norm1 = _AdaLinearP(d, 6 * d)
        self.norm1_context = _AdaLinearP(d, 6 * d)
        self.attn = _AttentionP(d, heads, head_dim, added=True)
        self.ff = _FeedForwardP(d, mlp_ratio)
        self.ff_context = _FeedForwardP(d, mlp_ratio)


class _Workspace:

    def __init__(self, dev, B, Bt, Nx, Nc, D, C_in, C_out, n_mod):
        f = dict(device=dev, dtype=torch.float32)
        self.mods = torch.empty(B, n_mod, **f)
        S = Nx + Nc
        self.h = torch.empty(B, S, D, **f)
        self.nh = torch.empty(B, S, D, **f)
        self.qkv = torch.empty(B, S, 3 * D, **f)
        self.att = torch.empty(B, S, D, **f)
        self.cat = torch.empty(B, S, 5 * D, **f)
        self.xtok = torch.empty(B, Nx, C_in, **f)
        self.ctok = torch.empty(B, Nc, C_in, **f)
        self.ctx0 = torch.empty(B, Nc, D, **f)
        self.otok = torch.empty(B, Nx, C_out, **f)
        self.tsin = torch.empty(Bt, 256, **f)
        self.t1 = torch.empty(Bt, D, **f)
        self.t2 = torch.empty(Bt, D, **f)
        self.t1m = torch.empty(Bt, D, **f)
        self.t2m = torch.empty(Bt, D, **f)
        self.pooled = torch.empty(B, D, **f)
        self.p1 = torch.empty(B, D, **f)
        self.temb_r = torch.empty(B, D, **f)
        self.temb = torch.empty(B, D, **f)
        self.mod_a = torch.empty(B, 6 * D, **f)
        self.mod_b = torch.empty(B, 6 * D, **f)


class LaDCastTransformer3DModel(ModelMixin):
    _supports_gradient_checkpointing = False

    def __init__(
        self,
        in_channels: int = 16,
        out_channels: int = 16,
        num_attention_heads: int = 24,
        attention_head_dim: int = 128,
        num_layers: int = 20,
        num_single_layers: int = 40,
        num_refiner_layers: int = 2,
        mlp_ratio: float = 4.0,
        patch_size: int = 1,
        patch_size_t: int = 1,
        qk_norm: str = "rms_norm",
        rope_theta: float = 256.0,
        rope_axes_dim: Tuple[int, ...] = (16, 56, 56),
        rope_spatial_grid_start_pos=0,
        rope_spatial_grid_end_pos=None,
        spatial_deg2rad: bool = False,
        conditioning_tensor_in_channels: int = None,
        conditioning_tensor_intermediate_proj_dim: Optional[int] = None,
        conditioning_tensor_rope_axes_dim: Tuple[int, ...] = (16, 56, 56),
        incl_time_elapsed: bool = False,
        nope: bool = False,
        scale_attn_by_lat: bool = False,
    ) -> None:
        super().__init__()
        self.register_to_config(**{k: v for k, v in locals().items() if k not in ("self", "__class__")})
        if scale_attn_by_lat and patch_size != 1:
            raise NotImplementedError("scale_attn_by_lat hard-wires the 15 x 30 token grid (models/LaDCast_3D_model.py:684-693): patch size 1 only")
        if attention_head_dim != 128 or qk_norm != "rms_norm":
            raise NotImplementedError("the attention kernel is built for head_dim 128 + rms_norm q/k")
        if in_channels % 4 or (conditioning_tensor_in_channels or in_channels) % 4:
            raise NotImplementedError("channel counts must be multiples of 4 (16-byte rows)")
        heads, hd = num_attention_heads, attention_head_dim
        d = heads * hd
        out_channels = out_channels or in_channels
        self.inner_dim = d
        ps3 = (patch_size_t, patch_size, patch_size)
        self._patch_vol = patch_size_t * patch_size * patch_size
        if (in_channels * self._patch_vol) % 4 or ((conditioning_tensor_in_channels or in_channels) * self._patch_vol) % 4:
            raise NotImplementedError("channels x patch volume must be a multiple of 4 (16-byte rows)")
        self.x_embedder = _PatchEmbedP(in_channels, d, ps3)
        if conditioning_tensor_intermediate_proj_dim is None:
            conditioning_tensor_intermediate_proj_dim = d
        self.context_embedder = _PatchEmbedP(conditioning_tensor_in_channels, d, ps3)
        self.context_refiner = _TokenRefinerP(conditioning_tensor_intermediate_proj_dim, heads, hd, num_refiner_layers)
        self.time_text_embed = _CombinedTimestepTextProjP(d, d)
        self.time_elapsed_embed = _TimestepEmbeddingP(256, 2 * d) if incl_time_elapsed else None
        if spatial_deg2rad:
            rope_spatial_grid_start_pos = [float(np.deg2rad(v)) for v in rope_spatial_grid_start_pos]
            rope_spatial_grid_end_pos = [float(np.deg2rad(v)) for v in rope_spatial_grid_end_pos]
        self.rope_spatial_grid_start_pos = rope_spatial_grid_start_pos
        self.rope_spatial_grid_end_pos = rope_spatial_grid_end_pos
        assert sum(rope_axes_dim) == hd, "sum(rope_axes_dim) must equal attention_head_dim"
        assert sum(conditioning_tensor_rope_axes_dim) == hd
        self.transformer_blocks = nn.ModuleList([_DualBlockP(heads, hd, mlp_ratio) for _ in range(num_layers)])
        self.single_transformer_blocks = nn.ModuleList([_SingleBlockP(heads, hd, mlp_ratio) for _ in range(num_single_layers)])
        self.norm_out = _AdaLinearP(d, 2 * d)
        self.proj_out = nn.Linear(d, self._patch_vol * out_channels)
        self.requires_grad_(False)
        self.scale_attn_by_lat = bool(scale_attn_by_lat)
        self.attn_lat_weights = None
        if scale_attn_by_lat:
            w = np.cos(np.deg2rad(np.linspace(-83.25, 84.75, 15)))
            w = w / w.mean()
            self.attn_lat_weights = torch.from_numpy(w / w.sum()).float().repeat_interleave(30).view(1, 1, 1, -1)
        self._kbias = {}
        self._plan = None
        self._plan_gen = 0
        self._ws = {}
        self._rope = {}
        self._te_cache = None
        self._te_buf = {}
        self._graphs = {}
        self._capture_stream = None
        self.use_hip_graph = False
        self.gemm_precision = "fp32"

    def enable_hip_graph(self, flag: bool = True):
        if flag and self._foreign_processors():
            raise NotImplementedError("hipGraph capture is for the built-in attention path; a user-supplied attention processor runs eagerly")
        self.use_hip_graph = bool(flag)
        if not flag:
            self._drop_graphs()
        return self

    def _drop_graphs(self):
        self._graphs = {}

    def _drop_plan(self, device_caches=False):
        self._plan = None
        self._drop_graphs()
        if device_caches:
            self._ws, self._rope, self._te_buf, self._kbias = {}, {}, {}, {}
            self._te_cache = None

    def set_attn_lat_weights(self, weights: torch.Tensor):
        self.attn_lat_weights = weights.detach().float().reshape(1, 1, 1, -1).cpu()
        self._kbias = {}
        self._drop_graphs()
        return self

    def _key_bias(self, frames, dev):
        if not self.scale_attn_by_lat:
            return None
        key = (frames, str(dev))
        if key not in self._kbias:
            self._kbias[key] = hip.pad_key_bias(self.attn_lat_weights.reshape(-1).repeat(frames).to(dev))
        return self._kbias[key]

    def set_gemm_precision(self, mode: str):
        if mode not in ("fp32", "bf16x3", "bf16"):
            raise ValueError("gemm precision must be 'fp32', 'bf16x3' or 'bf16'")
        if mode != self.gemm_precision:
            self.gemm_precision = mode
            self._drop_plan()
        return self

    @property
    def attn_processors(self):
        out = {}
        for name, mod in self.named_modules():
            if isinstance(mod, _AttentionP):
                out[f"{name}.processor"] = mod.get_processor()
        return out

    def set_attn_processor(self, processor):
        mods = {f"{n}.processor": m for n, m in self.named_modules() if isinstance(m, _AttentionP)}
        if isinstance(processor, dict):
            if len(processor) != len(mods):
                raise ValueError(
                    f"A dict of processors was passed, but the number of processors {len(processor)} does not match the"
                    f" number of attention layers: {len(mods)}. Please make sure to pass {len(mods)} processor classes."
                )
            for k, m in mods.items():
                m.set_processor(processor[k])
        else:
            for m in mods.values():
                m.set_processor(processor)
        if self._foreign_processors():
            if self.use_hip_graph:
                self.enable_hip_graph(False)
            self._drop_graphs()

    def _foreign_processors(self):
        return [m for m in self.modules() if isinstance(m, _AttentionP) and m.foreign_processor is not None]

    def _call_processor(self, attn, hidden_states, encoder_hidden_states, attention_mask, image_rotary_emb, cond_image_rotary_emb):
        import inspect

        proc = attn.foreign_processor
        kw = dict(encoder_hidden_states=encoder_hidden_states, attention_mask=attention_mask, image_rotary_emb=image_rotary_emb,
                  cond_image_rotary_emb=cond_image_rotary_emb)
        params = inspect.signature(proc.__call__).parameters
        if not any(p.kind is inspect.Parameter.VAR_KEYWORD for p in params.values()):
            kw = {k: v for k, v in kw.items() if k in params}
        out = proc(attn, hidden_states, **kw)
        if not (isinstance(out, tuple) and len(out) == 2):
            raise TypeError("an attention processor must return (hidden_states, encoder_hidden_states) (models/LaDCast_3D_model.py:78-86,221)")
        return out

    def _apply(self, fn, *a, **k):
        self._drop_plan(device_caches=True)
        return super()._apply(fn, *a, **k)

    def load_state_dict(self, *a, **k):
        self._drop_plan()
        return super().load_state_dict(*a, **k)

    @staticmethod
    def _fuse_qkv(q, k, v):
        return (
            torch.cat([q.weight, k.weight, v.weight], dim=0).contiguous(),
            torch.cat([q.bias, k.bias, v.bias], dim=0).contiguous(),
        )

    def _build_plan(self):
        self._upcast_to_fp32()
        if not next(self.parameters()).is_cuda:
            raise RuntimeError("LaDCastTransformer3DModel must live on a HIP device (no CPU fallback)")
        plan = SimpleNamespace(attn={})
        for name, mod in self.named_modules():
            if isinstance(mod, _AttentionP):
                e = SimpleNamespace()
                e.wqkv, e.bqkv = self._fuse_qkv(mod.to_q, mod.to_k, mod.to_v)
                if mod.add_q_proj is not None:
                    e.wqkv_c, e.bqkv_c = self._fuse_qkv(mod.add_q_proj, mod.add_k_proj, mod.add_v_proj)
                plan.attn[id(mod)] = e
        d = self.inner_dim
        plan.wx = self.x_embedder.proj.weight.reshape(d, -1).contiguous()
        plan.wc = self.context_embedder.proj.weight.reshape(d, -1).contiguous()
        kq = 64 if self.gemm_precision == "bf16" else 32
        plan.kx_pad = -(-plan.wx.shape[1] // kq) * kq
        plan.kc_pad = -(-plan.wc.shape[1] // kq) * kq
        mods = []
        for blk in self.transformer_blocks:
            mods += [blk.norm1.linear, blk.norm1_context.linear]
        mods += [blk.norm.linear for blk in self.single_transformer_blocks]
        mods.append(self.norm_out.linear)
        plan.mod_w = torch.cat([m.weight for m in mods], dim=0).contiguous()
        plan.mod_b = torch.cat([m.bias for m in mods], dim=0).contiguous()
        plan.mod_off, off = {}, 0
        for m in mods:
            plan.mod_off[id(m)] = off
            off += m.weight.shape[0]
        plan.split = self.gemm_precision in ("bf16x3", "bf16")
        plan.one_term = self.gemm_precision == "bf16"
        plan.packed = {}
        if plan.split:
            ws = [e.wqkv for e in plan.attn.values()] + [e.wqkv_c for e in plan.attn.values() if hasattr(e, "wqkv_c")]
            ws.append(self.context_refiner.proj_in.weight)
            ws.append(self.proj_out.weight)
            for blk in self.context_refiner.token_refiner.refiner_blocks:
                ws += [blk.ff.net[0].proj.weight, blk.ff.net[2].weight]
            for blk in self.transformer_blocks:
                ws += [blk.attn.to_out[0].weight, blk.attn.to_add_out.weight, blk.ff.net[0].proj.weight, blk.ff.net[2].weight,
                       blk.ff_context.net[0].proj.weight, blk.ff_context.net[2].weight]
            for blk in self.single_transformer_blocks:
                ws += [blk.proj_mlp.weight, blk.proj_out.weight]
            pack = hip.pack_weight_bf16 if plan.one_term else hip.pack_weight_bf16x2
            for w in ws:
                plan.packed[id(w)] = pack(w)
            for w, kp in ((plan.wx, plan.kx_pad), (plan.wc, plan.kc_pad)):
                wp = torch.zeros(w.shape[0], kp, device=w.device, dtype=w.dtype)
                wp[:, : w.shape[1]] = w
                plan.packed[id(w)] = pack(wp)
        self._plan = plan
        self._plan_gen += 1

    def _patches(self, x):
        p, pt = self.config.patch_size, self.config.patch_size_t
        if p == 1 and pt == 1:
            return x
        B, C, T, H, W = x.shape
        if T % pt or H % p or W % p:
            raise ValueError(f"a (T, H, W) = {(T, H, W)} tensor is not a whole number of ({pt}, {p}, {p}) patches")
        return x.reshape(B, C, T // pt, pt, H // p, p, W // p, p).permute(0, 1, 3, 5, 7, 2, 4, 6).reshape(B, C * pt * p * p, T // pt, H // p, W // p).contiguous()

    def _unpatch(self, y, C_out):
        p, pt = self.config.patch_size, self.config.patch_size_t
        if p == 1 and pt == 1:
            return y
        B, _, T, H, W = y.shape
        return y.reshape(B, C_out, pt, p, p, T, H, W).permute(0, 1, 5, 2, 6, 3, 7, 4).reshape(B, C_out, T * pt, H * p, W * p).contiguous()

    def _rope_tables(self, r, t_in, h, w, dev):
        key = (r, t_in, h, w, str(dev))
        if key not in self._rope:
            c = self.config
            cond_t = torch.arange(-t_in + 1, 1, dtype=torch.float32)
            pred_t = torch.arange(1, r + 1, dtype=torch.float32)
            lat = torch.linspace(self.rope_spatial_grid_start_pos[0], self.rope_spatial_grid_end_pos[0], steps=h, dtype=torch.float32)
            lon = torch.linspace(self.rope_spatial_grid_start_pos[1], self.rope_spatial_grid_end_pos[1], steps=w, dtype=torch.float32)
            if getattr(c, "nope", False):
                n = h * w
                pc, ps = (t.repeat_interleave(n, dim=0).contiguous() for t in rotary_1d(c.attention_head_dim, pred_t, c.rope_theta))
                cc, cs = (t.repeat_interleave(n, dim=0).contiguous() for t in rotary_1d(c.attention_head_dim, cond_t, c.rope_theta))
            else:
                pc, ps = rope_tables_from_grid(c.rope_axes_dim, [pred_t, lat, lon], c.rope_theta)
                cc, cs = rope_tables_from_grid(c.conditioning_tensor_rope_axes_dim, [cond_t, lat, lon], c.rope_theta)
            pc, ps, cc, cs = (t.to(dev) for t in (pc, ps, cc, cs))
            pk, ck = hip.compact_rope_table(pc, ps), hip.compact_rope_table(cc, cs)
            jk = torch.cat([pk, ck], dim=0).contiguous()
            self._rope[key] = (pc, ps, cc, cs, pk, ck, jk)
        return self._rope[key]

    def _time_elapsed_embedding(self, time_elapsed, dev):
        key = (time_elapsed.data_ptr(), time_elapsed._version, tuple(time_elapsed.shape), str(time_elapsed.device))
        if self._te_cache is not None and self._te_cache[0] == key:
            return self._te_cache[1]
        stamps = getattr(time_elapsed, "host_values", None)
        if stamps is None or len(stamps) != time_elapsed.numel():
            stamps = time_elapsed.reshape(-1).tolist()
        stamps = [int(v) for v in stamps]
        n, d2 = len(stamps), 2 * self.inner_dim
        emb = get_year_sincos_embedding(stamps, 256)
        emb = hip.upload_nonblocking(emb, dev)
        te = self.time_elapsed_embed
        if n not in self._te_buf:
            self._te_buf[n] = (torch.empty(n, d2, device=dev, dtype=torch.float32), torch.empty(n, d2, device=dev, dtype=torch.float32))
        mid, out = self._te_buf[n]
        hip.linear_small(emb, te.linear_1.weight, mid, rows=n, N=d2, K=256, bias=te.linear_1.bias, act_out=hip.ACT_SILU)
        hip.linear_small(mid, te.linear_2.weight, out, rows=n, N=d2, K=d2, bias=te.linear_2.bias)
        self._te_cache = (key, out, time_elapsed)
        return out

    def _timestep_mlps(self, timestep, Bt, pooled, B, ws):
        D = self.inner_dim
        r, m = self.context_refiner.time_text_embed, self.time_text_embed
        P = hip.linear_small_problem
        TS = hip.ACT_IN_TIMESTEP_SINCOS
        hip.linear_small_grouped([
            P(timestep, r.timestep_embedder.linear_1.weight, ws.t1, rows=Bt, N=D, K=256, bias=r.timestep_embedder.linear_1.bias, act_in=TS, act_out=hip.ACT_SILU),
            P(timestep, m.timestep_embedder.linear_1.weight, ws.t1m, rows=Bt, N=D, K=256, bias=m.timestep_embedder.linear_1.bias, act_in=TS, act_out=hip.ACT_SILU),
            P(pooled, r.text_embedder.linear_1.weight, ws.p1, rows=B, N=D, K=D, bias=r.text_embedder.linear_1.bias, act_out=hip.ACT_SILU),
        ])
        hip.linear_small_grouped([
            P(ws.t1, r.timestep_embedder.linear_2.weight, ws.t2, rows=Bt, N=D, K=D, bias=r.timestep_embedder.linear_2.bias),
            P(ws.t1m, m.timestep_embedder.linear_2.weight, ws.t2m, rows=Bt, N=D, K=D, bias=m.timestep_embedder.linear_2.bias),
        ])
        tx = r.text_embedder
        hip.linear_small(ws.p1, tx.linear_2.weight, ws.temb_r, rows=B, N=D, K=D, bias=tx.linear_2.bias, add=ws.t2, add_rows=Bt)

    def _text_mlp(self, emb, pooled, B, Bt, t2, ws, out, te=None):
        D = self.inner_dim
        tx = emb.text_embedder
        hip.linear_small(pooled, tx.linear_1.weight, ws.p1, rows=B, N=D, K=D, bias=tx.linear_1.bias, act_out=hip.ACT_SILU)
        hip.linear_small(ws.p1, tx.linear_2.weight, out, rows=B, N=D, K=D, bias=tx.linear_2.bias, add=t2, add_rows=Bt, mod=te,
                         mod_rows=1 if te is None else te.shape[0])

    def _attention(self, ws, B, row0, Sx, Sc, out, ldo, o_bs, seg_x, seg_c, out_split=False, key_bias=None, normed=False, Sq=None):
        D, H = self.inner_dim, self.config.num_attention_heads
        qkv = ws.qkv
        full = qkv.shape[1]
        S = Sx + Sc
        q = qkv[:, row0:, 0:D]
        k = qkv[:, row0:, D : 2 * D]
        v = qkv[:, row0:, 2 * D : 3 * D]
        if self.gemm_precision in ("bf16x3", "bf16"):
            hip.attn_fwd_split(q, k, v, out, B=B, S=S, H=H, ld_qkv=3 * D, qkv_bs=full * 3 * D, ldo=ldo, o_bs=o_bs, out_split=out_split,
                               one_term=self.gemm_precision == "bf16", key_bias=key_bias, Sq=Sq)
            return
        segs = [] if normed else [sg for sg in ((Sx, seg_x), (Sc, seg_c)) if sg[0] > 0]
        r0 = row0
        for rows, (nq, nk, c, s_) in segs:
            hip.qk_rmsnorm_rope(qkv[:, :, 0:D], qkv[:, :, D : 2 * D], B=B, row0=r0, rows=rows, H=H, ld=3 * D, bs=full * 3 * D,
                                wq=nq.weight, wk=nk.weight, eps=nq.eps, cos=c, sin=s_)
            r0 += rows
        hip.attn_fwd(q, k, v, out, B=B, S=S, H=H, ld_qkv=3 * D, qkv_bs=full * 3 * D, ldo=ldo, o_bs=o_bs, key_bias=key_bias, Sq=Sq)

    def _qkv_epi(self, norm_q, norm_k, rope):
        if norm_q.eps != norm_k.eps:
            raise NotImplementedError("the fused QKV epilogue takes one RMSNorm eps for q and k")
        return hip.qkv_epilogue(norm_q.weight, norm_k.weight, rope, eps=norm_q.eps, heads=self.config.num_attention_heads,
                                qscale=0.0 if self.gemm_precision in ("bf16x3", "bf16") else 1.0)

    @torch.no_grad()
    def forward(
        self,
        hidden_states: torch.Tensor,
        timestep: torch.Tensor,
        conditioning_tensors: torch.Tensor,
        time_elapsed: Optional[torch.Tensor] = None,
        attention_kwargs=None,
        return_dict: bool = True,
        coords=None,
        conditioning=None,
    ):
        if self._plan is None:
            self._build_plan()
        plan = self._plan
        dev = self.device
        cfg = self.config
        D, H = self.inner_dim, cfg.num_attention_heads
        B, C_in, R, Hh, Ww = hidden_states.shape
        T_in = conditioning_tensors.shape[2]
        Cc = conditioning_tensors.shape[1]
        Nx, Nc = R * Hh * Ww, T_in * Hh * Ww
        S = Nx + Nc
        C_out = cfg.out_channels or cfg.in_channels
        hidden_states = hidden_states.to(device=dev, dtype=torch.float32).contiguous()
        conditioning_tensors = conditioning_tensors.to(device=dev, dtype=torch.float32)
        if conditioning_tensors.shape[0] != B:
            conditioning_tensors = conditioning_tensors.expand(B, -1, -1, -1, -1)
        conditioning_tensors = conditioning_tensors.contiguous()
        timestep = timestep.to(device=dev, dtype=torch.float32).reshape(-1).contiguous()
        Bt = timestep.shape[0]
        if Bt not in (1, B):
            raise ValueError(f"timestep must have 1 or {B} entries, got {Bt}")
        te = None
        if time_elapsed is not None and self.time_elapsed_embed is not None:
            te = self._time_elapsed_embedding(time_elapsed, dev)
            if te.shape[0] not in (1, B):
                raise ValueError("time_elapsed must have 1 or batch entries")

        if conditioning is not None:
            pack, idx = conditioning
            if tuple(pack.shape) != (B,) + tuple(conditioning_tensors.shape[1:]) or not 0 <= idx < pack.levels:
                raise ValueError("`conditioning` was prepared for another batch / conditioning shape")
            out = self._main_device(hidden_states, pack, idx)
            return (out,) if not return_dict else SimpleNamespace(sample=out)
        if self.use_hip_graph:
            gkey = (B, Bt, C_in, R, T_in, Hh, Ww, None if te is None else (te.data_ptr(), te.shape[0]), bool(self.skip_unread_rows))
            inputs = [hidden_states, timestep, conditioning_tensors]
            ent = self._graphs.get(gkey)
            if ent is None:
                ent = self._graphs[gkey] = graphs.capture(lambda x, t, k: self._forward_device(x, t, k, te), inputs, dev, self.capture_stream())
            out = ent.replay(*inputs)
        else:
            out = self._forward_device(hidden_states, timestep, conditioning_tensors, te)
        if not return_dict:
            return (out,)
        return SimpleNamespace(sample=out)

    def time_elapsed_embedding(self, time_elapsed):
        if time_elapsed is None or self.time_elapsed_embed is None:
            return None
        if self._plan is None:
            self._build_plan()
        return self._time_elapsed_embedding(time_elapsed, self.device)

    def plan_identity(self):
        if self._plan is None:
            self._build_plan()
        return self._plan_gen

    def capture_stream(self):
        if self._capture_stream is None:
            self._capture_stream = torch.cuda.Stream(device=self.device)
        return self._capture_stream

    @torch.no_grad()
    def forward_launch_only(self, hidden_states, timestep, conditioning_tensors, te, conditioning=None):
        if self._plan is None:
            self._build_plan()
        if hidden_states.dtype != torch.float32 or not hidden_states.is_cuda or not hidden_states.is_contiguous():
            raise TypeError("forward_launch_only takes a contiguous fp32 device tensor (use forward() for anything else)")
        if conditioning is not None:
            return self._main_device(hidden_states, conditioning[0], conditioning[1])
        return self._forward_device(hidden_states, timestep.reshape(-1), conditioning_tensors, te)

    batch_conditioning = True
    skip_unread_rows = True
    COND_MAX_ROWS = 96

    @torch.no_grad()
    def prepare_conditioning(self, timesteps, conditioning_tensors, te=None):
        if self._plan is None:
            self._build_plan()
        dev = self.device
        timesteps = timesteps.to(device=dev, dtype=torch.float32).reshape(-1)
        conditioning_tensors = conditioning_tensors.to(device=dev, dtype=torch.float32)
        if conditioning_tensors.dim() != 5:
            raise ValueError("conditioning_tensors must be (B, C, T_in, h, w)")
        N, B = timesteps.shape[0], conditioning_tensors.shape[0]
        shape = tuple(conditioning_tensors.shape)
        per = max(1, self.COND_MAX_ROWS // B)
        if per >= N:
            pk = self._conditioning_device(timesteps.repeat_interleave(B).contiguous(),
                                           conditioning_tensors.unsqueeze(0).expand(N, *shape).reshape(N * B, *shape[1:]).contiguous(), te)
            return SimpleNamespace(ctx=pk.ctx, mods=pk.mods, shape=shape, levels=N)
        Nc, D, NM = shape[2] * shape[3] * shape[4] // self._patch_vol, self.inner_dim, self._plan.mod_w.shape[0]
        key = ("pack", N, B, Nc)
        if key not in self._ws:
            self._ws[key] = (torch.empty(N * B, Nc, D, device=dev, dtype=torch.float32), torch.empty(N * B, NM, device=dev, dtype=torch.float32))
        ctx, mods = self._ws[key]
        for n0 in range(0, N, per):
            n = min(per, N - n0)
            pk = self._conditioning_device(timesteps[n0 : n0 + n].repeat_interleave(B).contiguous(),
                                           conditioning_tensors.unsqueeze(0).expand(n, *shape).reshape(n * B, *shape[1:]).contiguous(), te)
            ctx[n0 * B : (n0 + n) * B].copy_(pk.ctx)
            mods[n0 * B : (n0 + n) * B].copy_(pk.mods)
        return SimpleNamespace(ctx=ctx, mods=mods, shape=shape, levels=N)

    @staticmethod
    def _launchers(plan):
        split, packed = plan.split, plan.packed
        AS = (hip.GEMM_A_SPLIT | (hip.GEMM_BF16_1TERM if plan.one_term else 0)) if split else 0
        CS = hip.GEMM_C_SPLIT if split else 0
        fmt = hip.FMT_BF16 if plan.one_term else hip.FMT_SPLIT if split else hip.FMT_F32

        def G(A, W, C, **kw):
            return hip.gemm_problem(A, packed[id(W)] if split else W, C, **kw)

        def run(problems):
            hip.gemm_grouped(problems, split_bf16=split)

        def run1(A, W, C, **kw):
            hip.gemm_grouped([G(A, W, C, **kw)], split_bf16=split)

        def run_qkv(problems, epis):
            if split:
                hip.gemm_grouped_qkv(problems, epis)
                return True
            if hip.gemm_grouped_qkv_f32(problems, epis):
                return True
            hip.gemm_grouped(problems, split_bf16=False)
            return False

        return AS, CS, fmt, G, run, run1, run_qkv

    def _forward_device(self, hidden_states, timestep, conditioning_tensors, te):
        pack = self._conditioning_device(timestep, conditioning_tensors, te)
        return self._main_device(hidden_states, SimpleNamespace(ctx=pack.ctx, mods=pack.mods, shape=tuple(conditioning_tensors.shape), levels=1), 0)

    def _conditioning_device(self, timestep, conditioning_tensors, te):
        plan = self._plan
        dev = self.device
        cfg = self.config
        D, H = self.inner_dim, cfg.num_attention_heads
        conditioning_tensors = self._patches(conditioning_tensors)
        B, Cc, T_in, Hh, Ww = conditioning_tensors.shape
        Nx, Nc = 0, T_in * Hh * Ww
        S = Nc
        Bt = timestep.shape[0]
        kpad = max(plan.kx_pad, plan.kc_pad)
        key = ("cond", B, Bt, Nc, kpad)
        if key not in self._ws:
            self._ws[key] = _Workspace(dev, B, Bt, 0, Nc, D, kpad, 4, plan.mod_w.shape[0])
        ws = self._ws[key]
        _, _, cc, cs, _, ck, _ = self._rope_tables(1, T_in, Hh, Ww, dev)
        SD = S * D
        h_c, nh_c = ws.h, ws.nh
        split = plan.split

        AS, CS, fmt, G, run, run1, run_qkv = self._launchers(plan)

        if split:
            KC = plan.kc_pad
            ctok = ws.ctok.view(-1)[: B * Nc * KC].view(B, Nc, KC)
            hip.chan_to_token(conditioning_tensors, ctok, B=B, C=Cc, N=Nc, ldo=KC, fill_cols=KC, out_split=fmt)
            run1(ctok, plan.wc, ws.ctx0, M=Nc, N=D, K=KC, batch=B, a_bs=Nc * KC, c_bs=Nc * D, bias=self.context_embedder.proj.bias, flags=AS)
        else:
            hip.chan_to_token(conditioning_tensors, ws.ctok.view(-1)[: B * Nc * Cc].view(B, Nc, Cc), B=B, C=Cc, N=Nc, ldo=Cc)
            hip.gemm(ws.ctok, plan.wc, ws.ctx0, M=Nc, N=D, K=Cc, batch=B, a_bs=Nc * Cc, c_bs=Nc * D, bias=self.context_embedder.proj.bias)

        kb_cond = None
        if self.scale_attn_by_lat:
            if Hh * Ww != self.attn_lat_weights.numel():
                raise ValueError("scale_attn_by_lat is hard-wired to the 15 x 30 latent grid (models/LaDCast_3D_model.py:684-692)")
            kb_cond = self._key_bias(T_in, dev)
        foreign = bool(self._foreign_processors())
        m_cond = None
        if foreign:
            if split:
                raise NotImplementedError("a user-supplied attention processor runs on the fp32 path: call set_gemm_precision('fp32') "
                                          "(or change the attention arithmetic through the C ABI, include/ladcast_hip.h)")
            if torch.cuda.is_current_stream_capturing():
                raise NotImplementedError("a user-supplied attention processor cannot be captured into a hipGraph")
            if self.scale_attn_by_lat:
                w = self.attn_lat_weights.to(dev)
                m_cond = w.repeat(1, 1, 1, T_in)

        ref = self.context_refiner
        if split:
            hip.mean_rows(ws.ctx0, ws.pooled, B=B, rows=Nc, D=D, ldx=D, x_bs=Nc * D, x_split=nh_c, lds=D, s_bs=SD, fmt=fmt)
        else:
            hip.mean_rows(ws.ctx0, ws.pooled, B=B, rows=Nc, D=D, ldx=D, x_bs=Nc * D)
        self._timestep_mlps(timestep, Bt, ws.pooled, B, ws)
        if split:
            run1(nh_c, ref.proj_in.weight, h_c, M=Nc, N=D, K=D, batch=B, a_bs=SD, c_bs=SD, bias=ref.proj_in.bias, flags=AS)
        else:
            run1(ws.ctx0, ref.proj_in.weight, h_c, M=Nc, N=D, K=D, batch=B, a_bs=Nc * D, c_bs=SD, bias=ref.proj_in.bias)
        for blk in ref.token_refiner.refiner_blocks:
            pa = plan.attn[id(blk.attn)]
            hip.layernorm_mod(h_c, nh_c, B=B, rows=Nc, D=D, ldx=D, x_bs=SD, ldy=D, y_bs=SD, scale=blk.norm1.weight, shift=blk.norm1.bias, mode=1, eps=blk.norm1.eps, out_split=fmt)
            if blk.attn.foreign_processor is not None:
                a, _ = self._call_processor(blk.attn, nh_c, None, m_cond, (cc, cs), None)
                ws.att.copy_(a)
            else:
                nd = run_qkv([G(nh_c, pa.wqkv, ws.qkv, M=Nc, N=3 * D, K=D, batch=B, a_bs=SD, c_bs=S * 3 * D, bias=pa.bqkv, flags=AS)],
                             [self._qkv_epi(blk.attn.norm_q, blk.attn.norm_k, ck)])
                self._attention(ws, B, Nx, Nc, 0, ws.att, D, SD, (blk.attn.norm_q, blk.attn.norm_k, cc, cs), None, key_bias=kb_cond, normed=nd)
            hip.linear_small(ws.temb_r, blk.norm_out.linear.weight, ws.mod_a, rows=B, N=2 * D, K=D, bias=blk.norm_out.linear.bias, act_in=hip.ACT_SILU)
            hip.gate_residual_layernorm(h_c, ws.att, ws.mod_a, nh_c, B=B, rows=Nc, D=D, ld_res=D, res_bs=SD, ld_y=D, y_bs=SD, gate_bs=2 * D,
                                        ld_out=D, out_bs=SD, weight=blk.norm2.weight, bias=blk.norm2.bias, eps=blk.norm2.eps, out_split=fmt)
            f0, f2 = blk.ff.net[0].proj, blk.ff.net[2]
            F = f0.weight.shape[0]
            run1(nh_c, f0.weight, ws.cat, M=Nc, N=F, K=D, batch=B, a_bs=SD, c_bs=Nc * F, bias=f0.bias, act=hip.ACT_SILU, flags=AS | CS)
            run1(ws.cat, f2.weight, h_c, M=Nc, N=D, K=F, batch=B, a_bs=Nc * F, c_bs=SD, bias=f2.bias,
                        gate=ws.mod_a[:, D:], gate_bs=2 * D, R=h_c, ldr=D, r_bs=SD, flags=AS)

        hip.mean_rows(h_c, ws.pooled, B=B, rows=Nc, D=D, ldx=D, x_bs=SD)
        self._text_mlp(self.time_text_embed, ws.pooled, B, Bt, ws.t2m, ws, ws.temb, te=te)
        NM = plan.mod_w.shape[0]
        hip.linear_small(ws.temb, plan.mod_w, ws.mods, rows=B, N=NM, K=D, bias=plan.mod_b, act_in=hip.ACT_SILU)

        return SimpleNamespace(ctx=ws.h, mods=ws.mods, rows=B, shape=(B, Cc, T_in, Hh, Ww))

    def _main_device(self, hidden_states, pack, idx):
        plan = self._plan
        dev = self.device
        cfg = self.config
        D, H = self.inner_dim, cfg.num_attention_heads
        hidden_states = self._patches(hidden_states)
        B, C_in, R, Hh, Ww = hidden_states.shape
        T_in = pack.shape[2] // cfg.patch_size_t
        Nx, Nc = R * Hh * Ww, T_in * Hh * Ww
        S = Nx + Nc
        C_out = (cfg.out_channels or cfg.in_channels) * self._patch_vol
        kpad = max(plan.kx_pad, plan.kc_pad)
        key = (B, Nx, Nc, kpad)
        if key not in self._ws:
            self._ws[key] = _Workspace(dev, B, 1, Nx, Nc, D, kpad, C_out, 4)
        ws = self._ws[key]
        pc, ps, cc, cs, pk, ck, jk = self._rope_tables(R, T_in, Hh, Ww, dev)
        SD = S * D
        h_x, h_c = ws.h[:, :Nx], ws.h[:, Nx:]
        nh_x, nh_c = ws.nh[:, :Nx], ws.nh[:, Nx:]
        NM = plan.mod_w.shape[0]
        mods = pack.mods[idx * B : (idx + 1) * B]
        split = plan.split

        AS, CS, fmt, G, run, run1, run_qkv = self._launchers(plan)

        if split:
            KX = plan.kx_pad
            xtok = ws.xtok.view(-1)[: B * Nx * KX].view(B, Nx, KX)
            hip.chan_to_token(hidden_states, xtok, B=B, C=C_in, N=Nx, ldo=KX, fill_cols=KX, out_split=fmt)
            run1(xtok, plan.wx, h_x, M=Nx, N=D, K=KX, batch=B, a_bs=Nx * KX, c_bs=SD, bias=self.x_embedder.proj.bias, flags=AS)
        else:
            hip.chan_to_token(hidden_states, ws.xtok.view(-1)[: B * Nx * C_in].view(B, Nx, C_in), B=B, C=C_in, N=Nx, ldo=C_in)
            hip.gemm(ws.xtok, plan.wx, h_x, M=Nx, N=D, K=C_in, batch=B, a_bs=Nx * C_in, c_bs=SD, bias=self.x_embedder.proj.bias)
        h_c.copy_(pack.ctx[idx * B : (idx + 1) * B])

        kb_all = None
        if self.scale_attn_by_lat:
            if Hh * Ww != self.attn_lat_weights.numel():
                raise ValueError("scale_attn_by_lat is hard-wired to the 15 x 30 latent grid (models/LaDCast_3D_model.py:684-692)")
            kb_all = self._key_bias(R + T_in, dev)
        foreign = bool(self._foreign_processors())
        m_all = None
        if foreign:
            if split:
                raise NotImplementedError("a user-supplied attention processor runs on the fp32 path: call set_gemm_precision('fp32') "
                                          "(or change the attention arithmetic through the C ABI, include/ladcast_hip.h)")
            if torch.cuda.is_current_stream_capturing():
                raise NotImplementedError("a user-supplied attention processor cannot be captured into a hipGraph")
            if self.scale_attn_by_lat:
                w = self.attn_lat_weights.to(dev)
                m_all = w.repeat(1, 1, 1, T_in + R)


        def mod_of(linear, width):
            o = plan.mod_off[id(linear)]
            return mods[:, o : o + width]

        for blk in self.transformer_blocks:
            pa = plan.attn[id(blk.attn)]
            mx, mc = mod_of(blk.norm1.linear, 6 * D), mod_of(blk.norm1_context.linear, 6 * D)
            hip.layernorm_mod(ws.h, ws.nh, B=B, rows=S, D=D, ldx=D, x_bs=SD, ldy=D, y_bs=SD, scale=mx[:, D:], shift=mx, split_row=Nx, scale2=mc[:, D:], shift2=mc,
                              mod_bs=NM, mode=0, eps=1e-6, out_split=fmt)
            if blk.attn.foreign_processor is not None:
                a, ca = self._call_processor(blk.attn, nh_x, nh_c, m_all, (pc, ps), (cc, cs))
                a, ca = a.contiguous(), ca.contiguous()
                hip.gate_residual(h_x, a, mx[:, 2 * D :], h_x, B=B, rows=Nx, D=D, ld_res=D, res_bs=SD, ld_y=D, y_bs=Nx * D, gate_bs=NM)
                hip.gate_residual(h_c, ca, mc[:, 2 * D :], h_c, B=B, rows=Nc, D=D, ld_res=D, res_bs=SD, ld_y=D, y_bs=Nc * D, gate_bs=NM)
            else:
                nd = run_qkv([
                    G(nh_x, pa.wqkv, ws.qkv, M=Nx, N=3 * D, K=D, batch=B, a_bs=SD, c_bs=S * 3 * D, bias=pa.bqkv, flags=AS),
                    G(nh_c, pa.wqkv_c, ws.qkv[:, Nx:], M=Nc, N=3 * D, K=D, batch=B, a_bs=SD, c_bs=S * 3 * D, bias=pa.bqkv_c, flags=AS),
                ], [self._qkv_epi(blk.attn.norm_q, blk.attn.norm_k, pk), self._qkv_epi(blk.attn.norm_added_q, blk.attn.norm_added_k, None)])
                self._attention(ws, B, 0, Nx, Nc, ws.att, D, SD, (blk.attn.norm_q, blk.attn.norm_k, pc, ps),
                                (blk.attn.norm_added_q, blk.attn.norm_added_k, None, None), out_split=fmt, key_bias=kb_all, normed=nd)
                o, oc = blk.attn.to_out[0], blk.attn.to_add_out
                run([
                    G(ws.att, o.weight, h_x, M=Nx, N=D, K=D, batch=B, a_bs=SD, c_bs=SD, bias=o.bias, gate=mx[:, 2 * D :], gate_bs=NM, R=h_x, ldr=D, r_bs=SD, flags=AS),
                    G(ws.att[:, Nx:], oc.weight, h_c, M=Nc, N=D, K=D, batch=B, a_bs=SD, c_bs=SD, bias=oc.bias, gate=mc[:, 2 * D :], gate_bs=NM, R=h_c, ldr=D, r_bs=SD, flags=AS),
                ])
            hip.layernorm_mod(ws.h, ws.nh, B=B, rows=S, D=D, ldx=D, x_bs=SD, ldy=D, y_bs=SD, scale=mx[:, 4 * D :], shift=mx[:, 3 * D :], split_row=Nx,
                              scale2=mc[:, 4 * D :], shift2=mc[:, 3 * D :], mod_bs=NM, mode=0, eps=1e-7, out_split=fmt)
            up, down = [], []
            for (hs, nhs, rows, ff, mod, off) in ((h_x, nh_x, Nx, blk.ff, mx, 0), (h_c, nh_c, Nc, blk.ff_context, mc, Nx)):
                f0, f2 = ff.net[0].proj, ff.net[2]
                F = f0.weight.shape[0]
                hid = ws.cat.view(-1)[off * B * F :]
                up.append(G(nhs, f0.weight, hid, M=rows, N=F, K=D, batch=B, a_bs=SD, c_bs=rows * F, bias=f0.bias, act=hip.ACT_GELU_TANH, flags=AS | CS))
                down.append(G(hid, f2.weight, hs, M=rows, N=D, K=F, batch=B, a_bs=rows * F, c_bs=SD, bias=f2.bias,
                              gate=mod[:, 5 * D :], gate_bs=NM, R=hs, ldr=D, r_bs=SD, flags=AS))
            run(up)
            run(down)

        n_single = len(self.single_transformer_blocks)
        for i_blk, blk in enumerate(self.single_transformer_blocks):
            pa = plan.attn[id(blk.attn)]
            Mq = Nx if (self.skip_unread_rows and i_blk == n_single - 1 and blk.attn.foreign_processor is None) else S
            mod = mod_of(blk.norm.linear, 3 * D)
            F = blk.proj_mlp.weight.shape[0]
            W5 = D + F
            cat_mlp = ws.cat.view(torch.bfloat16)[:, :, D:] if plan.one_term else ws.cat[:, :, D:]
            hip.layernorm_mod(ws.h, ws.nh, B=B, rows=S, D=D, ldx=D, x_bs=SD, ldy=D, y_bs=SD, scale=mod[:, D:], shift=mod, mod_bs=NM, mode=0, eps=1e-6, out_split=fmt)
            if blk.attn.foreign_processor is not None:
                run([G(ws.nh, blk.proj_mlp.weight, cat_mlp, M=S, N=F, K=D, batch=B, a_bs=SD, ldc=W5, c_bs=S * W5, bias=blk.proj_mlp.bias,
                       act=hip.ACT_GELU_TANH, flags=AS | CS)])
                a, ca = self._call_processor(blk.attn, ws.nh[:, :Nx], ws.nh[:, Nx:], m_all, (pc, ps), (cc, cs))
                ws.cat[:, :Nx, :D].copy_(a)
                ws.cat[:, Nx:, :D].copy_(ca)
            else:
                nd = run_qkv([
                    G(ws.nh, blk.proj_mlp.weight, cat_mlp, M=Mq, N=F, K=D, batch=B, a_bs=SD, ldc=W5, c_bs=S * W5, bias=blk.proj_mlp.bias, act=hip.ACT_GELU_TANH,
                      flags=AS | CS),
                    G(ws.nh, pa.wqkv, ws.qkv, M=S, N=3 * D, K=D, batch=B, a_bs=SD, c_bs=S * 3 * D, bias=pa.bqkv, flags=AS),
                ], [None, self._qkv_epi(blk.attn.norm_q, blk.attn.norm_k, jk)])
                self._attention(ws, B, 0, Nx, Nc, ws.cat, W5, S * W5, (blk.attn.norm_q, blk.attn.norm_k, pc, ps),
                                (blk.attn.norm_q, blk.attn.norm_k, cc, cs), out_split=fmt, key_bias=kb_all, normed=nd, Sq=None if Mq == S else Mq)
            run1(ws.cat, blk.proj_out.weight, ws.h, M=Mq, N=D, K=W5, batch=B, a_bs=S * W5, c_bs=SD, bias=blk.proj_out.bias,
                        gate=mod[:, 2 * D :], gate_bs=NM, R=ws.h, ldr=D, r_bs=SD, flags=AS)

        mo = mod_of(self.norm_out.linear, 2 * D)
        hip.layernorm_mod(h_x, nh_x, B=B, rows=Nx, D=D, ldx=D, x_bs=SD, ldy=D, y_bs=SD, scale=mo, shift=mo[:, D:], mod_bs=NM, mode=0, eps=1e-7, out_split=fmt)
        run1(nh_x, self.proj_out.weight, ws.otok, M=Nx, N=C_out, K=D, batch=B, a_bs=SD, c_bs=Nx * C_out, bias=self.proj_out.bias, flags=AS)
        out = torch.empty(B, C_out, R, Hh, Ww, device=dev, dtype=torch.float32)
        hip.token_to_chan(ws.otok, out, B=B, C=C_out, N=Nx, ldi=C_out)
        return self._unpatch(out, cfg.out_channels or cfg.in_channels)
```

### ladcast_amd/pipelines/edm_sampler.py

```python
from __future__ import annotations

from typing import List, Optional, Union

import numpy as np
import torch

from .. import graphs, hip
from .torch_utils import randn_tensor


@torch.no_grad()
def edm_AR_sampler(
    net,
    noise_scheduler,
    batch_size=1,
    return_seq_len=1,
    randn_like=torch.randn_like,
    num_inference_steps=18,
    S_churn=0,
    S_min=0,
    S_max=float("inf"),
    S_noise=0,
    deterministic=True,
    known_latents=None,
    timestamps: Optional[torch.LongTensor] = None,
    generator: Optional[Union[torch.Generator, List[torch.Generator]]] = None,
    device="cpu",
):
    if isinstance(generator, list) and len(generator) != batch_size:
        raise ValueError(
            f"You have passed a list of generators of length {len(generator)}, but requested an effective batch"
            f" size of {batch_size}. Make sure the batch size matches the length of the generators."
        )
    assert known_latents is not None, "known_latents must be provided"
    if isinstance(device, str):
        device = torch.device(device)

    shape = (batch_size, net.config.out_channels, return_seq_len, *known_latents.shape[-2:])
    latents = randn_tensor(shape, generator=generator, device=device, dtype=torch.float32).contiguous()
    noise_scheduler.set_timesteps(num_inference_steps, device=device)
    t_steps = noise_scheduler.sigmas
    c_noise_host = noise_scheduler.precondition_noise(t_steps[:-1])
    known = known_latents.to(device=device, dtype=torch.float32)
    if known.shape[0] != batch_size:
        known = known.expand(batch_size, *known.shape[1:])
    known = known.contiguous()

    chunk_graph = bool(getattr(net, "use_hip_graph", False)) and hasattr(net, "forward_launch_only") and hasattr(net, "_graphs")
    batched = bool(getattr(net, "batch_conditioning", False)) and hasattr(net, "prepare_conditioning")
    if not deterministic:
        out = torch.empty(shape, device=device, dtype=torch.float32)
        fwd = lambda x, t, k, te_: net(x, t, k, time_elapsed=timestamps).sample
        _heun_chunk_stochastic(fwd, noise_scheduler, t_steps, latents, known, out, shape, device, num_inference_steps, randn_like, S_churn, S_min,
                               S_max, S_noise)
        return out
    if chunk_graph:
        te = net.time_elapsed_embedding(timestamps)
        plan_id = net.plan_identity()
        key = (tuple(shape), tuple(known.shape), num_inference_steps, tuple(float(v) for v in t_steps.tolist()),
               None if te is None else (te.data_ptr(), tuple(te.shape)), str(device), plan_id, batched,
               bool(getattr(net, "skip_unread_rows", False)))
        prepare = net.prepare_conditioning if batched else None
        key = ("edm_chunk",) + key
        cache = net._graphs
        turn = cache.get(key + ("turn",), 0)
        cache[key + ("turn",)] = turn ^ 1

        def capture():
            st_out, cn = torch.empty(shape, device=device, dtype=torch.float32), c_noise_host.to(device)

            def chunk(lat, kn):
                _heun_chunk(net.forward_launch_only, noise_scheduler, t_steps, cn, lat, kn, te, st_out, shape, device, num_inference_steps, prepare)
                return st_out

            return graphs.capture(chunk, [latents, known], device, net.capture_stream(), keep=cn)

        for inst in (turn, turn ^ 1):
            if cache.get(key + (inst,)) is None:
                cache[key + (inst,)] = capture()
        return cache[key + (turn,)].replay(latents, known)

    out = torch.empty(shape, device=device, dtype=torch.float32)
    c_noise = hip.upload_nonblocking(c_noise_host, device)
    fwd = lambda x, t, k, te_, ci=None: net(x, t, k, time_elapsed=timestamps, **({} if ci is None else {"conditioning": ci})).sample
    prepare = None
    if batched:
        te = net.time_elapsed_embedding(timestamps)
        prepare = lambda cn, kn, te_: net.prepare_conditioning(cn, kn, te)
    _heun_chunk(fwd, noise_scheduler, t_steps, c_noise, latents, known, None, out, shape, device, num_inference_steps, prepare)
    return out


def _heun_chunk(fwd, noise_scheduler, t_steps, c_noise, latents, known, te, out, shape, device, num_inference_steps, prepare=None):
    cond = prepare(c_noise, known, te) if prepare is not None else None
    ci = (lambda i: None) if cond is None else (lambda i: (cond, i))
    x_hat = torch.empty(shape, device=device, dtype=torch.float64)
    x_next = torch.empty_like(x_hat)
    d_cur = torch.empty_like(x_hat)
    x_in = torch.empty(shape, device=device, dtype=torch.float32)
    hip.edm_init_state(latents, float(t_steps[0]), x_next)

    for i in range(num_inference_steps):
        t_cur, t_next = t_steps[i], t_steps[i + 1]
        x_hat, x_next = x_next, x_hat
        c_skip, c_out = noise_scheduler._c_skip_out(t_cur)
        hip.edm_scale_f64_to_f32(x_hat, float(noise_scheduler._c_in(t_cur)), x_in)
        F = fwd(x_in, c_noise[i : i + 1], known, te, ci(i))
        hip.edm_euler(x_hat, F, float(c_skip), float(c_out), float(t_cur), float(t_next - t_cur), x_next, d_cur)
        if i < num_inference_steps - 1:
            c_skip, c_out = noise_scheduler._c_skip_out(t_next)
            hip.edm_scale_f64_to_f32(x_next, float(noise_scheduler._c_in(t_next)), x_in)
            F = fwd(x_in, c_noise[i + 1 : i + 2], known, te, ci(i + 1))
            hip.edm_heun(x_hat, x_next, F, d_cur, float(c_skip), float(c_out), float(t_next), float(t_next - t_cur))
    hip.f64_to_f32(x_next, out)


def _heun_chunk_stochastic(fwd, noise_scheduler, t_steps, latents, known, out, shape, device, num_inference_steps, randn_like, S_churn, S_min,
                           S_max, S_noise):
    x_cur = torch.empty(shape, device=device, dtype=torch.float64)
    x_hat = torch.empty_like(x_cur)
    x_next = torch.empty_like(x_cur)
    d_cur = torch.empty_like(x_cur)
    x_in = torch.empty(shape, device=device, dtype=torch.float32)
    hip.edm_init_state(latents, float(t_steps[0]), x_next)
    for i in range(num_inference_steps):
        t_cur, t_next = t_steps[i], t_steps[i + 1]
        x_cur, x_next = x_next, x_cur
        gamma = min(S_churn / num_inference_steps, np.sqrt(2) - 1) if S_min <= t_cur <= S_max else 0
        t_hat = torch.as_tensor(t_cur + gamma * t_cur)
        noise = randn_like(x_cur)
        if noise.dtype != torch.float64 or noise.device != x_cur.device:
            noise = noise.to(device=x_cur.device, dtype=torch.float64)
        hip.edm_churn(x_cur, noise.contiguous(), float((t_hat**2 - t_cur**2).sqrt() * S_noise), x_hat)
        c_skip, c_out = noise_scheduler._c_skip_out(t_hat)
        hip.edm_scale_f64_to_f32(x_hat, float(noise_scheduler._c_in(t_hat)), x_in)
        F = fwd(x_in, noise_scheduler.precondition_noise(t_hat.reshape(1)).to(device), known, None)
        hip.edm_euler(x_hat, F, float(c_skip), float(c_out), float(t_hat), float(t_next - t_hat), x_next, d_cur)
        if i < num_inference_steps - 1:
            c_skip, c_out = noise_scheduler._c_skip_out(t_next)
            hip.edm_scale_f64_to_f32(x_next, float(noise_scheduler._c_in(t_next)), x_in)
            F = fwd(x_in, noise_scheduler.precondition_noise(t_next.reshape(1)).to(device), known, None)
            hip.edm_heun(x_hat, x_next, F, d_cur, float(c_skip), float(c_out), float(t_next), float(t_next - t_hat))
    hip.f64_to_f32(x_next, out)
```

### ladcast_amd/pipelines/pipeline_AR.py

```python
from __future__ import annotations

from typing import List, Optional, Tuple, Union

import torch

from .. import graphs
from .torch_utils import randn_tensor
from .utils import Fields2DPipelineOutput


class AutoRegressive2DPipeline:
    model_cpu_offload_seq = "unet"

    def __init__(self, ar_model, scheduler, scheduler_step_kwargs: Optional[dict] = None):
        self.register_modules(ar_model=ar_model, scheduler=scheduler)
        self.scheduler_step_kwargs = scheduler_step_kwargs or {}

    def register_modules(self, **mods):
        for k, v in mods.items():
            setattr(self, k, v)

    @property
    def _execution_device(self):
        return self.ar_model.device

    @property
    def device(self):
        return self.ar_model.device

    def to(self, *a, **k):
        self.ar_model.to(*a, **k)
        return self

    def return_trajectory(self, *a, **k):
        raise NotImplementedError("This function is not implemented yet.")

    @torch.no_grad()
    def __call__(
        self,
        batch_size: int = 1,
        return_seq_len: int = 1,
        known_latents: torch.Tensor = None,
        timestamps: Optional[torch.LongTensor] = None,
        generator: Optional[Union[torch.Generator, List[torch.Generator]]] = None,
        num_inference_steps: int = 50,
        return_dict: bool = True,
        do_edm_style: bool = True,
    ) -> Union[Fields2DPipelineOutput, Tuple]:
        if isinstance(generator, list) and len(generator) != batch_size:
            raise ValueError(
                f"You have passed a list of generators of length {len(generator)}, but requested an effective batch"
                f" size of {batch_size}. Make sure the batch size matches the length of the generators."
            )
        assert known_latents is not None, "known_latents must be provided"
        dev = self._execution_device
        shape = (batch_size, self.ar_model.config.out_channels, return_seq_len, *known_latents.shape[-2:])
        image = randn_tensor(shape, generator=generator, device=dev, dtype=torch.float32).contiguous()
        known_latents = known_latents.to(device=dev, dtype=torch.float32)
        if not do_edm_style:
            raise NotImplementedError("Only EDM style is supported for now")
        net, sch = self.ar_model, self.scheduler
        kw_ = self.scheduler_step_kwargs
        graphable = getattr(sch, "launch_only", False) and hasattr(sch, "graph_signature") and not kw_.get("eta") and kw_.get("generator") is None and kw_.get("variance_noise") is None
        if getattr(net, "use_hip_graph", False) and hasattr(net, "forward_launch_only") and hasattr(net, "_graphs") and graphable:
            image = self._graph_loop(net, sch, image, known_latents.contiguous(), timestamps, num_inference_steps, batch_size, dev)
            if not return_dict:
                return (image,)
            return Fields2DPipelineOutput(fields=image)
        self.scheduler.set_timesteps(num_inference_steps)
        pack = None
        if getattr(net, "batch_conditioning", False) and hasattr(net, "prepare_conditioning"):
            kn = known_latents if known_latents.shape[0] == batch_size else known_latents.expand(batch_size, *known_latents.shape[1:])
            pack = net.prepare_conditioning(self.scheduler.timesteps, kn.contiguous(), net.time_elapsed_embedding(timestamps))
        for i, t in enumerate(self.scheduler.timesteps):
            if not do_edm_style:
                raise NotImplementedError("Only EDM style is supported for now")
            x_in = self.scheduler.scale_model_input(image, t)
            t_host = t
            t = t.expand(batch_size).to(dev)
            t.host_value = t_host
            ckw = {} if pack is None else {"conditioning": (pack, i)}
            model_output = self.ar_model(x_in, t, known_latents, time_elapsed=timestamps, return_dict=False, **ckw)[0]
            image = self.scheduler.step(model_output, t, image, **self.scheduler_step_kwargs, return_dict=False)[0]
        if not return_dict:
            return (image,)
        return Fields2DPipelineOutput(fields=image)

    def _graph_loop(self, net, sch, image, known, timestamps, num_inference_steps, batch_size, dev):
        sch.set_timesteps(num_inference_steps)
        te = net.time_elapsed_embedding(timestamps)
        key = (tuple(image.shape), tuple(known.shape), num_inference_steps, sch.graph_signature(),
               tuple(sorted((k, str(v)) for k, v in self.scheduler_step_kwargs.items())), None if te is None else (te.data_ptr(), tuple(te.shape)), str(dev), net.plan_identity(),
               bool(getattr(net, "batch_conditioning", False)), bool(getattr(net, "skip_unread_rows", False)))
        key = ("pipeline_loop",) + key
        cache = net._graphs
        ent = cache.get(key)
        if ent is None:
            ts_dev = sch.timesteps.to(device=dev, dtype=torch.float32).contiguous()
            tsteps = [t.to(device=dev, dtype=torch.float32).expand(batch_size).contiguous() for t in sch.timesteps]

            def loop(img, kn):
                kb = kn if kn.shape[0] == batch_size else kn.expand(batch_size, *kn.shape[1:]).contiguous()
                pack = net.prepare_conditioning(ts_dev, kb, te) if getattr(net, "batch_conditioning", False) else None
                for i, (t, t_dev) in enumerate(zip(sch.timesteps, tsteps)):
                    x_in = sch.scale_model_input(img, t)
                    out = net.forward_launch_only(x_in, t_dev, kb, te, None if pack is None else (pack, i))
                    img = sch.step(out, t, img, **self.scheduler_step_kwargs, return_dict=False)[0]
                return img

            ent = graphs.capture(loop, [image, known], dev, net.capture_stream(), reset=lambda: sch.set_timesteps(num_inference_steps),
                                 keep={"tsteps": tsteps, "ts_dev": ts_dev})
            ent.keep["scheduler_state"] = sch.graph_state()
            cache[key] = ent
        out = ent.replay(image, known)
        sch.set_graph_state(ent.keep["scheduler_state"])
        return out
```

Measured before the change: 3.223.

## Share noise-level-invariant conditioning work across diffusion levels and hoist block0 context QKV

Adds a share_level_invariant mode, on by default. The timestep-independent part of the context refiner's first block (norm, QKV, attention) is computed once per conditioning member instead of once per noise level. A new gate_residual_layernorm_from kernel variant broadcasts that shared input across levels. The first transformer block's context-side layernorm and QKV projection are also precomputed for all levels in prepare_conditioning, and at each step they are copied in instead of recomputed. This removes redundant GEMM and attention work on context tokens, at the cost of extra workspace memory, extra copies, and more code-path complexity.

```diff
diff --git a/include/ladcast_hip.h b/include/ladcast_hip.h
--- a/include/ladcast_hip.h
+++ b/include/ladcast_hip.h
@@ -141,6 +141,10 @@
 int ldc_gate_residual_layernorm(float* resid, const float* y, const float* gate, float* out, int B, int rows, int D, int ld_res,
                                 long long res_bs, int ld_y, long long y_bs, int gate_bs, int ld_out, long long out_bs,
                                 const float* weight, const float* bias, float eps, int out_split, void* stream);
+int ldc_gate_residual_layernorm_from(float* resid, const float* resid_in, const float* y, const float* gate, float* out, int B, int P,
+                                     int rows, int D, int ld_res, long long res_bs, int ld_in, long long in_bs, int ld_y,
+                                     long long y_bs, int gate_bs, int ld_out, long long out_bs, const float* weight,
+                                     const float* bias, float eps, int out_split, void* stream);
 
 int ldc_chan_to_token(const float* in, float* out, int B, int C, int N, int ldo, int fill_cols, void* stream);
 int ldc_chan_to_token_split(const float* in, float* out, int B, int C, int N, int ldo, int fill_cols,
diff --git a/ladcast_amd/csrc/rowops.hip b/ladcast_amd/csrc/rowops.hip
--- a/ladcast_amd/csrc/rowops.hip
+++ b/ladcast_amd/csrc/rowops.hip
@@ -12,17 +12,21 @@
                                                             const float* __restrict__ shift2, int mod_bs, int mode,
                                                             float eps, int out_split, const float* __restrict__ pre_y,
                                                             const float* __restrict__ pre_gate, int ld_prey,
-                                                            long long prey_bs, int gate_bs) {
+                                                            long long prey_bs, int gate_bs,
+                                                            const float* __restrict__ x_in, int ld_in, long long in_bs,
+                                                            int src_period) {
   const int lane = threadIdx.x & 63;
   const int row = blockIdx.x * 4 + (threadIdx.x >> 6);
   const int b = blockIdx.y;
   if (row >= rows) return;
+  const int bsrc = b % src_period;
   if (row >= split_row) {
     scale = scale2;
     shift = shift2;
   }
   float* xr = x + b * x_bs + static_cast<long long>(row) * ldx;
   float* yr = y + b * y_bs + static_cast<long long>(row) * ldy;
+  const float* xs = x_in ? x_in + bsrc * in_bs + static_cast<long long>(row) * ld_in : xr;
   const int nv4 = D >> 2;
   float4 v[LN_MAX_V4];
   float sum = 0.f;
@@ -30,9 +34,9 @@
   for (int i = 0; i < LN_MAX_V4; ++i) {
     const int c = lane + 64 * i;
     if (c < nv4) {
-      v[i] = reinterpret_cast<const float4*>(xr)[c];
+      v[i] = reinterpret_cast<const float4*>(xs)[c];
       if (pre_y) {
-        const float4 yv = reinterpret_cast<const float4*>(pre_y + b * prey_bs + static_cast<long long>(row) * ld_prey)[c];
+        const float4 yv = reinterpret_cast<const float4*>(pre_y + bsrc * prey_bs + static_cast<long long>(row) * ld_prey)[c];
         const float4 g = reinterpret_cast<const float4*>(pre_gate + static_cast<long long>(b) * gate_bs)[c];
         v[i] = make_float4(fmaf(yv.x, g.x, v[i].x), fmaf(yv.y, g.y, v[i].y), fmaf(yv.z, g.z, v[i].z), fmaf(yv.w, g.w, v[i].w));
         reinterpret_cast<float4*>(xr)[c] = v[i];
@@ -457,14 +461,17 @@
   dim3 grid(ldc_cdiv(rows, 4), B);
   hipLaunchKernelGGL(layernorm_mod_kernel, grid, dim3(256), 0, static_cast<hipStream_t>(stream), const_cast<float*>(x), y, rows, D,
                      ldx, x_bs, ldy, y_bs, scale, shift, split_row, scale2, shift2, mod_bs, mode, eps, out_split,
-                     static_cast<const float*>(nullptr), static_cast<const float*>(nullptr), 0, 0LL, 0);
+                     static_cast<const float*>(nullptr), static_cast<const float*>(nullptr), 0, 0LL, 0,
+                     static_cast<const float*>(nullptr), 0, 0LL, B);
   return ldc_launch_status();
 }
 
-extern "C" int ldc_gate_residual_layernorm(float* resid, const float* yv, const float* gate, float* out, int B, int rows, int D,
-                                           int ld_res, long long res_bs, int ld_y, long long y_bs, int gate_bs, int ld_out,
-                                           long long out_bs, const float* weight, const float* bias, float eps, int out_split,
-                                           void* stream) {
+namespace {
+
+int gate_residual_layernorm_launch(float* resid, const float* resid_in, const float* yv, const float* gate, float* out, int B, int P,
+                                   int rows, int D, int ld_res, long long res_bs, int ld_in, long long in_bs, int ld_y, long long y_bs,
+                                   int gate_bs, int ld_out, long long out_bs, const float* weight, const float* bias, float eps,
+                                   int out_split, void* stream) {
   LDC_CHECK_PTR(resid);
   LDC_CHECK_PTR(yv);
   LDC_CHECK_PTR(gate);
@@ -472,7 +479,9 @@
   if (B <= 0 || rows <= 0 || D <= 0) return LDC_ERR_ARG;
   if ((D & 3) || D > 64 * 4 * LN_MAX_V4) return LDC_ERR_UNSUPPORTED;
   if ((ld_res & 3) || (ld_y & 3) || (ld_out & 3) || (res_bs & 3) || (y_bs & 3) || (out_bs & 3) || (gate_bs & 3)) return LDC_ERR_ALIGN;
+  if ((ld_in & 3) || (in_bs & 3)) return LDC_ERR_ALIGN;
   LDC_CHECK_ALIGN16(resid);
+  if (resid_in) LDC_CHECK_ALIGN16(resid_in);
   LDC_CHECK_ALIGN16(yv);
   LDC_CHECK_ALIGN16(gate);
   LDC_CHECK_ALIGN16(out);
@@ -482,8 +491,28 @@
   dim3 grid(ldc_cdiv(rows, 4), B);
   hipLaunchKernelGGL(layernorm_mod_kernel, grid, dim3(256), 0, static_cast<hipStream_t>(stream), resid, out, rows, D, ld_res, res_bs,
                      ld_out, out_bs, weight, bias, rows, static_cast<const float*>(nullptr), static_cast<const float*>(nullptr), 0, 1,
-                     eps, out_split, yv, gate, ld_y, y_bs, gate_bs);
+                     eps, out_split, yv, gate, ld_y, y_bs, gate_bs, resid_in, ld_in, in_bs, P);
   return ldc_launch_status();
+}
+
+}
+
+extern "C" int ldc_gate_residual_layernorm(float* resid, const float* yv, const float* gate, float* out, int B, int rows, int D,
+                                           int ld_res, long long res_bs, int ld_y, long long y_bs, int gate_bs, int ld_out,
+                                           long long out_bs, const float* weight, const float* bias, float eps, int out_split,
+                                           void* stream) {
+  return gate_residual_layernorm_launch(resid, nullptr, yv, gate, out, B, B, rows, D, ld_res, res_bs, 0, 0, ld_y, y_bs, gate_bs, ld_out,
+                                        out_bs, weight, bias, eps, out_split, stream);
+}
+
+extern "C" int ldc_gate_residual_layernorm_from(float* resid, const float* resid_in, const float* yv, const float* gate, float* out,
+                                                int B, int P, int rows, int D, int ld_res, long long res_bs, int ld_in, long long in_bs,
+                                                int ld_y, long long y_bs, int gate_bs, int ld_out, long long out_bs,
+                                                const float* weight, const float* bias, float eps, int out_split, void* stream) {
+  LDC_CHECK_PTR(resid_in);
+  if (P <= 0 || B <= 0 || B % P != 0) return LDC_ERR_ARG;
+  return gate_residual_layernorm_launch(resid, resid_in, yv, gate, out, B, P, rows, D, ld_res, res_bs, ld_in, in_bs, ld_y, y_bs, gate_bs,
+                                        ld_out, out_bs, weight, bias, eps, out_split, stream);
 }
 
 extern "C" int ldc_layernorm_mod(const float* x, float* y, int B, int rows, int D, int ldx, long long x_bs, int ldy,
diff --git a/ladcast_amd/hip.py b/ladcast_amd/hip.py
--- a/ladcast_amd/hip.py
+++ b/ladcast_amd/hip.py
@@ -85,6 +85,7 @@
         "ldc_linear_small_grouped": (I, [POINTER(LinearSmallProblem), I, P]),
         "ldc_linear_small_mod": (I, [P, I, P, P, P, I, P, I, P, I, I, I, I, I, P]),
         "ldc_gate_residual_layernorm": (I, [P, P, P, P, I, I, I, I, L, I, L, I, I, L, P, P, F, I, P]),
+        "ldc_gate_residual_layernorm_from": (I, [P, P, P, P, P, I, I, I, I, I, L, I, L, I, L, I, I, L, P, P, F, I, P]),
         "ldc_attn_fwd": (I, [P, P, P, P, I, I, I, I, L, I, L, P, P]),
         "ldc_attn_fwd_ws": (I, [P, P, P, P, I, I, I, I, L, I, L, P, P, L, P]),
         "ldc_attn_fwd_qrows": (I, [P, P, P, P, I, I, I, I, I, L, I, L, P, P]),
@@ -291,6 +292,14 @@
                                            _p(weight), _p(bias), eps, int(out_split), _stream()), "ldc_gate_residual_layernorm")
 
 
+def gate_residual_layernorm_from(resid, resid_in, y, gate, out, *, B, P, rows, D, ld_res, res_bs, ld_in, in_bs, ld_y, y_bs, gate_bs, ld_out, out_bs,
+                                 weight, bias, eps, out_split=False):
+    _dev(resid, resid_in, y, gate, out, weight, bias)
+    _check(lib.ldc_gate_residual_layernorm_from(_p(resid), _p(resid_in), _p(y), _p(gate), _p(out), B, P, rows, D, ld_res, res_bs, ld_in, in_bs,
+                                                ld_y, y_bs, gate_bs, ld_out, out_bs, _p(weight), _p(bias), eps, int(out_split), _stream()),
+           "ldc_gate_residual_layernorm_from")
+
+
 LINEAR_SMALL_MAX_GROUPED = 4
 
 
diff --git a/ladcast_amd/models/LaDCast_3D_model.py b/ladcast_amd/models/LaDCast_3D_model.py
--- a/ladcast_amd/models/LaDCast_3D_model.py
+++ b/ladcast_amd/models/LaDCast_3D_model.py
@@ -183,6 +183,19 @@
         self.temb = torch.empty(B, D, **f)
         self.mod_a = torch.empty(B, 6 * D, **f)
         self.mod_b = torch.empty(B, 6 * D, **f)
+
+
+class _SharedWorkspace:
+
+    def __init__(self, dev, B, Nc, D, C_in):
+        f = dict(device=dev, dtype=torch.float32)
+        self.ctok = torch.empty(B, Nc, C_in, **f)
+        self.ctx0 = torch.empty(B, Nc, D, **f)
+        self.pooled = torch.empty(B, D, **f)
+        self.h = torch.empty(B, Nc, D, **f)
+        self.nh = torch.empty(B, Nc, D, **f)
+        self.qkv = torch.empty(B, Nc, 3 * D, **f)
+        self.att = torch.empty(B, Nc, D, **f)
 
 
 class LaDCastTransformer3DModel(ModelMixin):
@@ -510,11 +523,13 @@
             hip.attn_fwd_split(q, k, v, out, B=B, S=S, H=H, ld_qkv=3 * D, qkv_bs=full * 3 * D, ldo=ldo, o_bs=o_bs, out_split=out_split,
                                one_term=self.gemm_precision == "bf16", key_bias=key_bias, Sq=Sq)
             return
-        segs = [] if normed else [sg for sg in ((Sx, seg_x), (Sc, seg_c)) if sg[0] > 0]
+        segs = [] if normed else [(Sx, seg_x), (Sc, seg_c)]
         r0 = row0
-        for rows, (nq, nk, c, s_) in segs:
-            hip.qk_rmsnorm_rope(qkv[:, :, 0:D], qkv[:, :, D : 2 * D], B=B, row0=r0, rows=rows, H=H, ld=3 * D, bs=full * 3 * D,
-                                wq=nq.weight, wk=nk.weight, eps=nq.eps, cos=c, sin=s_)
+        for rows, sg in segs:
+            if rows > 0 and sg is not None:
+                nq, nk, c, s_ = sg
+                hip.qk_rmsnorm_rope(qkv[:, :, 0:D], qkv[:, :, D : 2 * D], B=B, row0=r0, rows=rows, H=H, ld=3 * D, bs=full * 3 * D,
+                                    wq=nq.weight, wk=nk.weight, eps=nq.eps, cos=c, sin=s_)
             r0 += rows
         hip.attn_fwd(q, k, v, out, B=B, S=S, H=H, ld_qkv=3 * D, qkv_bs=full * 3 * D, ldo=ldo, o_bs=o_bs, key_bias=key_bias, Sq=Sq)
 
@@ -570,7 +585,8 @@
             out = self._main_device(hidden_states, pack, idx)
             return (out,) if not return_dict else SimpleNamespace(sample=out)
         if self.use_hip_graph:
-            gkey = (B, Bt, C_in, R, T_in, Hh, Ww, None if te is None else (te.data_ptr(), te.shape[0]), bool(self.skip_unread_rows))
+            gkey = (B, Bt, C_in, R, T_in, Hh, Ww, None if te is None else (te.data_ptr(), te.shape[0]), bool(self.skip_unread_rows),
+                    bool(self.share_level_invariant))
             inputs = [hidden_states, timestep, conditioning_tensors]
             ent = self._graphs.get(gkey)
             if ent is None:
@@ -611,6 +627,7 @@
 
     batch_conditioning = True
     skip_unread_rows = True
+    share_level_invariant = True
     COND_MAX_ROWS = 96
 
     @torch.no_grad()
@@ -625,22 +642,55 @@
         N, B = timesteps.shape[0], conditioning_tensors.shape[0]
         shape = tuple(conditioning_tensors.shape)
         per = max(1, self.COND_MAX_ROWS // B)
+        share = self._shares_refiner_head()
+        hoist = bool(self.share_level_invariant) and len(self.transformer_blocks) > 0 and self.transformer_blocks[0].attn.foreign_processor is None
+        head = [None]
+
+        def cond(n0, n):
+            ts = timesteps[n0 : n0 + n].repeat_interleave(B).contiguous()
+            if share:
+                pk = self._conditioning_device(ts, conditioning_tensors.contiguous(), te, levels=n, head=head[0])
+                head[0] = pk.head
+                return pk
+            return self._conditioning_device(ts, conditioning_tensors.unsqueeze(0).expand(n, *shape).reshape(n * B, *shape[1:]).contiguous(), te)
+
         if per >= N:
-            pk = self._conditioning_device(timesteps.repeat_interleave(B).contiguous(),
-                                           conditioning_tensors.unsqueeze(0).expand(N, *shape).reshape(N * B, *shape[1:]).contiguous(), te)
-            return SimpleNamespace(ctx=pk.ctx, mods=pk.mods, shape=shape, levels=N)
+            pk = cond(0, N)
+            qkv0 = pk.ws.qkv if hoist and self._block0_context_qkv(pk.ctx, pk.mods, pk.ws.nh, pk.ws.qkv) else None
+            return SimpleNamespace(ctx=pk.ctx, mods=pk.mods, shape=shape, levels=N, qkv0=qkv0)
         Nc, D, NM = shape[2] * shape[3] * shape[4] // self._patch_vol, self.inner_dim, self._plan.mod_w.shape[0]
-        key = ("pack", N, B, Nc)
+        key = ("pack", N, B, Nc, hoist)
         if key not in self._ws:
-            self._ws[key] = (torch.empty(N * B, Nc, D, device=dev, dtype=torch.float32), torch.empty(N * B, NM, device=dev, dtype=torch.float32))
-        ctx, mods = self._ws[key]
+            self._ws[key] = (torch.empty(N * B, Nc, D, device=dev, dtype=torch.float32), torch.empty(N * B, NM, device=dev, dtype=torch.float32),
+                             torch.empty(N * B, Nc, 3 * D, device=dev, dtype=torch.float32) if hoist else None)
+        ctx, mods, qkv0 = self._ws[key]
         for n0 in range(0, N, per):
             n = min(per, N - n0)
-            pk = self._conditioning_device(timesteps[n0 : n0 + n].repeat_interleave(B).contiguous(),
-                                           conditioning_tensors.unsqueeze(0).expand(n, *shape).reshape(n * B, *shape[1:]).contiguous(), te)
+            pk = cond(n0, n)
             ctx[n0 * B : (n0 + n) * B].copy_(pk.ctx)
             mods[n0 * B : (n0 + n) * B].copy_(pk.mods)
-        return SimpleNamespace(ctx=ctx, mods=mods, shape=shape, levels=N)
+            if hoist and qkv0 is not None and not self._block0_context_qkv(pk.ctx, pk.mods, pk.ws.nh, qkv0[n0 * B : (n0 + n) * B]):
+                qkv0 = None
+        return SimpleNamespace(ctx=ctx, mods=mods, shape=shape, levels=N, qkv0=qkv0)
+
+    def _shares_refiner_head(self):
+        blocks = self.context_refiner.token_refiner.refiner_blocks
+        return bool(self.share_level_invariant) and len(blocks) > 0 and blocks[0].attn.foreign_processor is None
+
+    def _block0_context_qkv(self, ctx, mods, nh, out):
+        plan = self._plan
+        D = self.inner_dim
+        Bc, Nc = ctx.shape[0], ctx.shape[1]
+        NM = plan.mod_w.shape[0]
+        AS, CS, fmt, G, run, run1, run_qkv = self._launchers(plan)
+        blk = self.transformer_blocks[0]
+        pa = plan.attn[id(blk.attn)]
+        o = plan.mod_off[id(blk.norm1_context.linear)]
+        mc = mods[:, o : o + 6 * D]
+        hip.layernorm_mod(ctx, nh, B=Bc, rows=Nc, D=D, ldx=D, x_bs=Nc * D, ldy=D, y_bs=Nc * D, scale=mc[:, D:], shift=mc, mod_bs=NM, mode=0, eps=1e-6,
+                          out_split=fmt)
+        return run_qkv([G(nh, pa.wqkv_c, out, M=Bc * Nc, N=3 * D, K=D, bias=pa.bqkv_c, flags=AS)],
+                       [self._qkv_epi(blk.attn.norm_added_q, blk.attn.norm_added_k, None)])
 
     @staticmethod
     def _launchers(plan):
@@ -670,16 +720,18 @@
         return AS, CS, fmt, G, run, run1, run_qkv
 
     def _forward_device(self, hidden_states, timestep, conditioning_tensors, te):
-        pack = self._conditioning_device(timestep, conditioning_tensors, te)
+        pack = self._conditioning_device(timestep, conditioning_tensors, te, levels=1 if self._shares_refiner_head() else None)
         return self._main_device(hidden_states, SimpleNamespace(ctx=pack.ctx, mods=pack.mods, shape=tuple(conditioning_tensors.shape), levels=1), 0)
 
-    def _conditioning_device(self, timestep, conditioning_tensors, te):
+    def _conditioning_device(self, timestep, conditioning_tensors, te, levels=None, head=None):
         plan = self._plan
         dev = self.device
         cfg = self.config
         D, H = self.inner_dim, cfg.num_attention_heads
         conditioning_tensors = self._patches(conditioning_tensors)
-        B, Cc, T_in, Hh, Ww = conditioning_tensors.shape
+        Bm, Cc, T_in, Hh, Ww = conditioning_tensors.shape
+        shared = levels is not None
+        B = Bm * levels if shared else Bm
         Nx, Nc = 0, T_in * Hh * Ww
         S = Nc
         Bt = timestep.shape[0]
@@ -688,21 +740,32 @@
         if key not in self._ws:
             self._ws[key] = _Workspace(dev, B, Bt, 0, Nc, D, kpad, 4, plan.mod_w.shape[0])
         ws = self._ws[key]
+        hd, Bh = ws, B
+        if shared:
+            key = ("cond_head", Bm, Nc, kpad)
+            if key not in self._ws:
+                self._ws[key] = _SharedWorkspace(dev, Bm, Nc, D, kpad)
+            hd, Bh = self._ws[key], Bm
         _, _, cc, cs, _, ck, _ = self._rope_tables(1, T_in, Hh, Ww, dev)
         SD = S * D
         h_c, nh_c = ws.h, ws.nh
         split = plan.split
 
         AS, CS, fmt, G, run, run1, run_qkv = self._launchers(plan)
-
-        if split:
+        done = shared and head is not None
+        if done and head is not hd:
+            raise ValueError("`head` belongs to another conditioning shape")
+
+        if done:
+            pass
+        elif split:
             KC = plan.kc_pad
-            ctok = ws.ctok.view(-1)[: B * Nc * KC].view(B, Nc, KC)
-            hip.chan_to_token(conditioning_tensors, ctok, B=B, C=Cc, N=Nc, ldo=KC, fill_cols=KC, out_split=fmt)
-            run1(ctok, plan.wc, ws.ctx0, M=Nc, N=D, K=KC, batch=B, a_bs=Nc * KC, c_bs=Nc * D, bias=self.context_embedder.proj.bias, flags=AS)
+            ctok = hd.ctok.view(-1)[: Bh * Nc * KC].view(Bh, Nc, KC)
+            hip.chan_to_token(conditioning_tensors, ctok, B=Bh, C=Cc, N=Nc, ldo=KC, fill_cols=KC, out_split=fmt)
+            run1(ctok, plan.wc, hd.ctx0, M=Nc, N=D, K=KC, batch=Bh, a_bs=Nc * KC, c_bs=Nc * D, bias=self.context_embedder.proj.bias, flags=AS)
         else:
-            hip.chan_to_token(conditioning_tensors, ws.ctok.view(-1)[: B * Nc * Cc].view(B, Nc, Cc), B=B, C=Cc, N=Nc, ldo=Cc)
-            hip.gemm(ws.ctok, plan.wc, ws.ctx0, M=Nc, N=D, K=Cc, batch=B, a_bs=Nc * Cc, c_bs=Nc * D, bias=self.context_embedder.proj.bias)
+            hip.chan_to_token(conditioning_tensors, hd.ctok.view(-1)[: Bh * Nc * Cc].view(Bh, Nc, Cc), B=Bh, C=Cc, N=Nc, ldo=Cc)
+            hip.gemm(hd.ctok, plan.wc, hd.ctx0, M=Nc, N=D, K=Cc, batch=Bh, a_bs=Nc * Cc, c_bs=Nc * D, bias=self.context_embedder.proj.bias)
 
         kb_cond = None
         if self.scale_attn_by_lat:
@@ -722,31 +785,50 @@
                 m_cond = w.repeat(1, 1, 1, T_in)
 
         ref = self.context_refiner
-        if split:
-            hip.mean_rows(ws.ctx0, ws.pooled, B=B, rows=Nc, D=D, ldx=D, x_bs=Nc * D, x_split=nh_c, lds=D, s_bs=SD, fmt=fmt)
+        if done:
+            pass
+        elif split:
+            hip.mean_rows(hd.ctx0, hd.pooled, B=Bh, rows=Nc, D=D, ldx=D, x_bs=Nc * D, x_split=hd.nh, lds=D, s_bs=SD, fmt=fmt)
         else:
-            hip.mean_rows(ws.ctx0, ws.pooled, B=B, rows=Nc, D=D, ldx=D, x_bs=Nc * D)
+            hip.mean_rows(hd.ctx0, hd.pooled, B=Bh, rows=Nc, D=D, ldx=D, x_bs=Nc * D)
+        if shared:
+            ws.pooled.view(levels, Bm, D).copy_(hd.pooled)
         self._timestep_mlps(timestep, Bt, ws.pooled, B, ws)
-        if split:
-            run1(nh_c, ref.proj_in.weight, h_c, M=Nc, N=D, K=D, batch=B, a_bs=SD, c_bs=SD, bias=ref.proj_in.bias, flags=AS)
+        if done:
+            pass
+        elif split:
+            run1(hd.nh, ref.proj_in.weight, hd.h, M=Nc, N=D, K=D, batch=Bh, a_bs=SD, c_bs=SD, bias=ref.proj_in.bias, flags=AS)
         else:
-            run1(ws.ctx0, ref.proj_in.weight, h_c, M=Nc, N=D, K=D, batch=B, a_bs=Nc * D, c_bs=SD, bias=ref.proj_in.bias)
-        for blk in ref.token_refiner.refiner_blocks:
+            run1(hd.ctx0, ref.proj_in.weight, hd.h, M=Nc, N=D, K=D, batch=Bh, a_bs=Nc * D, c_bs=SD, bias=ref.proj_in.bias)
+        flat = shared and levels > 1
+        for i_blk, blk in enumerate(ref.token_refiner.refiner_blocks):
             pa = plan.attn[id(blk.attn)]
-            hip.layernorm_mod(h_c, nh_c, B=B, rows=Nc, D=D, ldx=D, x_bs=SD, ldy=D, y_bs=SD, scale=blk.norm1.weight, shift=blk.norm1.bias, mode=1, eps=blk.norm1.eps, out_split=fmt)
-            if blk.attn.foreign_processor is not None:
+            w, Bw = (hd, Bh) if i_blk == 0 else (ws, B)
+            if i_blk == 0 and done:
+                pass
+            elif blk.attn.foreign_processor is not None:
+                hip.layernorm_mod(h_c, nh_c, B=B, rows=Nc, D=D, ldx=D, x_bs=SD, ldy=D, y_bs=SD, scale=blk.norm1.weight, shift=blk.norm1.bias, mode=1, eps=blk.norm1.eps, out_split=fmt)
                 a, _ = self._call_processor(blk.attn, nh_c, None, m_cond, (cc, cs), None)
                 ws.att.copy_(a)
             else:
-                nd = run_qkv([G(nh_c, pa.wqkv, ws.qkv, M=Nc, N=3 * D, K=D, batch=B, a_bs=SD, c_bs=S * 3 * D, bias=pa.bqkv, flags=AS)],
+                hip.layernorm_mod(w.h, w.nh, B=Bw, rows=Nc, D=D, ldx=D, x_bs=SD, ldy=D, y_bs=SD, scale=blk.norm1.weight, shift=blk.norm1.bias, mode=1, eps=blk.norm1.eps, out_split=fmt)
+                nd = run_qkv([G(w.nh, pa.wqkv, w.qkv, M=Nc, N=3 * D, K=D, batch=Bw, a_bs=SD, c_bs=S * 3 * D, bias=pa.bqkv, flags=AS)],
                              [self._qkv_epi(blk.attn.norm_q, blk.attn.norm_k, ck)])
-                self._attention(ws, B, Nx, Nc, 0, ws.att, D, SD, (blk.attn.norm_q, blk.attn.norm_k, cc, cs), None, key_bias=kb_cond, normed=nd)
+                self._attention(w, Bw, Nx, Nc, 0, w.att, D, SD, (blk.attn.norm_q, blk.attn.norm_k, cc, cs), None, key_bias=kb_cond, normed=nd)
             hip.linear_small(ws.temb_r, blk.norm_out.linear.weight, ws.mod_a, rows=B, N=2 * D, K=D, bias=blk.norm_out.linear.bias, act_in=hip.ACT_SILU)
-            hip.gate_residual_layernorm(h_c, ws.att, ws.mod_a, nh_c, B=B, rows=Nc, D=D, ld_res=D, res_bs=SD, ld_y=D, y_bs=SD, gate_bs=2 * D,
-                                        ld_out=D, out_bs=SD, weight=blk.norm2.weight, bias=blk.norm2.bias, eps=blk.norm2.eps, out_split=fmt)
+            if shared and i_blk == 0:
+                hip.gate_residual_layernorm_from(h_c, hd.h, hd.att, ws.mod_a, nh_c, B=B, P=Bm, rows=Nc, D=D, ld_res=D, res_bs=SD, ld_in=D, in_bs=SD,
+                                                 ld_y=D, y_bs=SD, gate_bs=2 * D, ld_out=D, out_bs=SD, weight=blk.norm2.weight, bias=blk.norm2.bias,
+                                                 eps=blk.norm2.eps, out_split=fmt)
+            else:
+                hip.gate_residual_layernorm(h_c, ws.att, ws.mod_a, nh_c, B=B, rows=Nc, D=D, ld_res=D, res_bs=SD, ld_y=D, y_bs=SD, gate_bs=2 * D,
+                                            ld_out=D, out_bs=SD, weight=blk.norm2.weight, bias=blk.norm2.bias, eps=blk.norm2.eps, out_split=fmt)
             f0, f2 = blk.ff.net[0].proj, blk.ff.net[2]
             F = f0.weight.shape[0]
-            run1(nh_c, f0.weight, ws.cat, M=Nc, N=F, K=D, batch=B, a_bs=SD, c_bs=Nc * F, bias=f0.bias, act=hip.ACT_SILU, flags=AS | CS)
+            if flat:
+                run1(nh_c, f0.weight, ws.cat, M=B * Nc, N=F, K=D, bias=f0.bias, act=hip.ACT_SILU, flags=AS | CS)
+            else:
+                run1(nh_c, f0.weight, ws.cat, M=Nc, N=F, K=D, batch=B, a_bs=SD, c_bs=Nc * F, bias=f0.bias, act=hip.ACT_SILU, flags=AS | CS)
             run1(ws.cat, f2.weight, h_c, M=Nc, N=D, K=F, batch=B, a_bs=Nc * F, c_bs=SD, bias=f2.bias,
                         gate=ws.mod_a[:, D:], gate_bs=2 * D, R=h_c, ldr=D, r_bs=SD, flags=AS)
 
@@ -755,7 +837,7 @@
         NM = plan.mod_w.shape[0]
         hip.linear_small(ws.temb, plan.mod_w, ws.mods, rows=B, N=NM, K=D, bias=plan.mod_b, act_in=hip.ACT_SILU)
 
-        return SimpleNamespace(ctx=ws.h, mods=ws.mods, rows=B, shape=(B, Cc, T_in, Hh, Ww))
+        return SimpleNamespace(ctx=ws.h, mods=ws.mods, rows=B, shape=(B, Cc, T_in, Hh, Ww), ws=ws, head=hd if shared else None)
 
     def _main_device(self, hidden_states, pack, idx):
         plan = self._plan
@@ -815,23 +897,35 @@
             o = plan.mod_off[id(linear)]
             return mods[:, o : o + width]
 
-        for blk in self.transformer_blocks:
+        qkv0 = getattr(pack, "qkv0", None)
+        for i_blk, blk in enumerate(self.transformer_blocks):
             pa = plan.attn[id(blk.attn)]
             mx, mc = mod_of(blk.norm1.linear, 6 * D), mod_of(blk.norm1_context.linear, 6 * D)
-            hip.layernorm_mod(ws.h, ws.nh, B=B, rows=S, D=D, ldx=D, x_bs=SD, ldy=D, y_bs=SD, scale=mx[:, D:], shift=mx, split_row=Nx, scale2=mc[:, D:], shift2=mc,
-                              mod_bs=NM, mode=0, eps=1e-6, out_split=fmt)
+            hoisted = qkv0 is not None and i_blk == 0 and blk.attn.foreign_processor is None
+            if hoisted:
+                hip.layernorm_mod(ws.h, ws.nh, B=B, rows=Nx, D=D, ldx=D, x_bs=SD, ldy=D, y_bs=SD, scale=mx[:, D:], shift=mx, mod_bs=NM, mode=0, eps=1e-6,
+                                  out_split=fmt)
+            else:
+                hip.layernorm_mod(ws.h, ws.nh, B=B, rows=S, D=D, ldx=D, x_bs=SD, ldy=D, y_bs=SD, scale=mx[:, D:], shift=mx, split_row=Nx, scale2=mc[:, D:], shift2=mc,
+                                  mod_bs=NM, mode=0, eps=1e-6, out_split=fmt)
             if blk.attn.foreign_processor is not None:
                 a, ca = self._call_processor(blk.attn, nh_x, nh_c, m_all, (pc, ps), (cc, cs))
                 a, ca = a.contiguous(), ca.contiguous()
                 hip.gate_residual(h_x, a, mx[:, 2 * D :], h_x, B=B, rows=Nx, D=D, ld_res=D, res_bs=SD, ld_y=D, y_bs=Nx * D, gate_bs=NM)
                 hip.gate_residual(h_c, ca, mc[:, 2 * D :], h_c, B=B, rows=Nc, D=D, ld_res=D, res_bs=SD, ld_y=D, y_bs=Nc * D, gate_bs=NM)
             else:
-                nd = run_qkv([
-                    G(nh_x, pa.wqkv, ws.qkv, M=Nx, N=3 * D, K=D, batch=B, a_bs=SD, c_bs=S * 3 * D, bias=pa.bqkv, flags=AS),
-                    G(nh_c, pa.wqkv_c, ws.qkv[:, Nx:], M=Nc, N=3 * D, K=D, batch=B, a_bs=SD, c_bs=S * 3 * D, bias=pa.bqkv_c, flags=AS),
-                ], [self._qkv_epi(blk.attn.norm_q, blk.attn.norm_k, pk), self._qkv_epi(blk.attn.norm_added_q, blk.attn.norm_added_k, None)])
-                self._attention(ws, B, 0, Nx, Nc, ws.att, D, SD, (blk.attn.norm_q, blk.attn.norm_k, pc, ps),
-                                (blk.attn.norm_added_q, blk.attn.norm_added_k, None, None), out_split=fmt, key_bias=kb_all, normed=nd)
+                probs = [G(nh_x, pa.wqkv, ws.qkv, M=Nx, N=3 * D, K=D, batch=B, a_bs=SD, c_bs=S * 3 * D, bias=pa.bqkv, flags=AS)]
+                epis = [self._qkv_epi(blk.attn.norm_q, blk.attn.norm_k, pk)]
+                seg_c = None
+                if hoisted:
+                    ws.qkv[:, Nx:].copy_(qkv0[idx * B : (idx + 1) * B])
+                else:
+                    probs.append(G(nh_c, pa.wqkv_c, ws.qkv[:, Nx:], M=Nc, N=3 * D, K=D, batch=B, a_bs=SD, c_bs=S * 3 * D, bias=pa.bqkv_c, flags=AS))
+                    epis.append(self._qkv_epi(blk.attn.norm_added_q, blk.attn.norm_added_k, None))
+                    seg_c = (blk.attn.norm_added_q, blk.attn.norm_added_k, None, None)
+                nd = run_qkv(probs, epis)
+                self._attention(ws, B, 0, Nx, Nc, ws.att, D, SD, (blk.attn.norm_q, blk.attn.norm_k, pc, ps), seg_c, out_split=fmt, key_bias=kb_all,
+                                normed=nd)
                 o, oc = blk.attn.to_out[0], blk.attn.to_add_out
                 run([
                     G(ws.att, o.weight, h_x, M=Nx, N=D, K=D, batch=B, a_bs=SD, c_bs=SD, bias=o.bias, gate=mx[:, 2 * D :], gate_bs=NM, R=h_x, ldr=D, r_bs=SD, flags=AS),
diff --git a/ladcast_amd/pipelines/edm_sampler.py b/ladcast_amd/pipelines/edm_sampler.py
--- a/ladcast_amd/pipelines/edm_sampler.py
+++ b/ladcast_amd/pipelines/edm_sampler.py
@@ -59,7 +59,8 @@
         plan_id = net.plan_identity()
         key = (tuple(shape), tuple(known.shape), num_inference_steps, tuple(float(v) for v in t_steps.tolist()),
                None if te is None else (te.data_ptr(), tuple(te.shape)), str(device), plan_id, batched,
-               bool(getattr(net, "skip_unread_rows", False)))
+               bool(getattr(net, "skip_unread_rows", False)),
+               bool(getattr(net, "share_level_invariant", False)))
         prepare = net.prepare_conditioning if batched else None
         key = ("edm_chunk",) + key
         cache = net._graphs
diff --git a/ladcast_amd/pipelines/pipeline_AR.py b/ladcast_amd/pipelines/pipeline_AR.py
--- a/ladcast_amd/pipelines/pipeline_AR.py
+++ b/ladcast_amd/pipelines/pipeline_AR.py
@@ -91,7 +91,8 @@
         te = net.time_elapsed_embedding(timestamps)
         key = (tuple(image.shape), tuple(known.shape), num_inference_steps, sch.graph_signature(),
                tuple(sorted((k, str(v)) for k, v in self.scheduler_step_kwargs.items())), None if te is None else (te.data_ptr(), tuple(te.shape)), str(dev), net.plan_identity(),
-               bool(getattr(net, "batch_conditioning", False)), bool(getattr(net, "skip_unread_rows", False)))
+               bool(getattr(net, "batch_conditioning", False)), bool(getattr(net, "skip_unread_rows", False)),
+               bool(getattr(net, "share_level_invariant", False)))
         key = ("pipeline_loop",) + key
         cache = net._graphs
         ent = cache.get(key)
```

New measurement: 3.252 (median of 6 runs). About the same (+0.9%).
